# shroglck/open-pi-zero

Hardware: AMD Instinct MI355X
Metric: train samples/sec at gbsz 1024 (bf16 fwd+bwd+clip+AdamW) (higher is better)
Workload: dtype bf16; 1 GPU; Pi0 bridge training step: 256 img + 20 text + 1 proprio + 4 action tokens; model=pi0 (SigLIP-So400m/14 + Gemma-2B + 0.3B action expert), global_batch=1024, micro_batch=256, grad_accum=4, seq_len=281, parallelism=dp1

## Files before the change

include/pz_abi.h:

```cpp
#ifndef PZ_ABI_H
#define PZ_ABI_H

#include <stdint.h>

#ifdef __cplusplus
extern "C" {
#endif

#define PZ_ABI_VERSION 22

enum {
  PZ_OK = 0,
  PZ_ERR_INVALID_ARG = 1,
  PZ_ERR_LAUNCH = 2,
  PZ_ERR_UNSUPPORTED = 3,
};

enum {
  PZ_EPI_NONE = 0,
  PZ_EPI_GELU = 1,
  PZ_EPI_GEGLU = 2,
  PZ_EPI_SILU = 3,
  PZ_EPI_DGELU = 4,
  PZ_EPI_DSILU = 5,
// ... 13 lines not shown
  const void* bias;
  const void* resid; int64_t ld_resid;
  void* aux; int64_t ld_aux;
  int64_t geglu_inter;
  void* workspace; int64_t ws_bytes;
  const void* norm_w; float norm_eps;
  int32_t fp8_mode; const float* a_row_scale;
  const void* A2; int64_t lda2;
  const void* B2; int64_t ldb2;
  int64_t K2;
} pz_gemm_args;
int pz_gemm(const pz_gemm_args* args, void* stream);
#define PZ_ABSMAX_PARTS 1024
int pz_fp8_quant_vt(const void* v, int64_t ldv, int64_t v_bstride, int64_t Z, int64_t nk, void* vt, float* vs,
                    int64_t ldt, void* stream);
int pz_fp8_quant_attn(const void* q, int64_t nqr, const void* k, int64_t nkr, const void* v, int64_t ldv,
                      int64_t v_bstride, int64_t Z, int64_t nk, void* qc, float* qs, void* kc, float* ks, void* vt,
                      float* vs, int64_t ldt, void* stream);
int pz_rmsnorm_fwd_f8(const void* x, int64_t ldx, const void* w, void* q, int64_t ldq, float* qscale, int64_t R,
                      int64_t D, float eps, void* stream);
int pz_layernorm_fwd_f8(const void* x, int64_t ldx, const void* w, const void* b, void* q, int64_t ldq, float* qscale,
                        int64_t R, int64_t D, float eps, void* stream);
int pz_fp8_quant_rows(const void* x, int64_t ldx, void* q, int64_t ldq, float* row_scale, int64_t R, int64_t D,
                      void* stream);
int pz_fp8_quant_tensor(const void* x, int64_t n, void* q, float inv_scale, void* stream);
int pz_fp8_absmax(const void* x, int64_t n, float* parts, void* stream);
const char* pz_gemm_kernel_name(const pz_gemm_args* args);

typedef struct pz_small_gemm_args {
  int64_t M, N, K;
  const void* A; int64_t sAm, sAk;
  const void* B; int64_t sBk, sBn;
  void* C; int64_t ldc;
  const void* bias;
  float alpha;
  int32_t beta;
} pz_small_gemm_args;
int pz_gemm_small(const pz_small_gemm_args* args, void* stream);

int pz_rmsnorm_fwd(const void* x, int64_t ldx, const void* w, void* y, int64_t ldy, float* rstd,
                   int64_t R, int64_t D, float eps, void* stream);
int pz_rmsnorm_bwd(const void* dy, int64_t lddy, const void* x, int64_t ldx, const void* w,
                   const float* rstd, const void* dres, void* dx, int64_t lddx, float* dw_part,
                   int64_t R, int64_t D, void* stream);
int pz_layernorm_fwd(const void* x, int64_t ldx, const void* w, const void* b, void* y, int64_t ldy,
                     float* mean, float* rstd, int64_t R, int64_t D, float eps, void* stream);
int pz_layernorm_bwd(const void* dy, int64_t lddy, const void* x, int64_t ldx, const void* w,
                     const float* mean, const float* rstd, const void* dres, void* dx, int64_t lddx,
                     float* dw_part, float* db_part, int64_t R, int64_t D, float* dx_part, void* stream);
int64_t pz_norm_rows_per_part(void);
int pz_reduce_parts(const float* part, int64_t P, int64_t D, void* out, int32_t beta, void* stream);
typedef struct pz_reduce_seg {
  const float* part; int64_t P, D; void* out; int32_t beta;
} pz_reduce_seg;
int pz_reduce_parts_multi(const pz_reduce_seg* segs, int32_t nseg, void* stream);
int pz_act_bwd_colsum(const void* dh, int64_t lddh, const void* pre, int64_t ldpre, void* dpre, int64_t M, int64_t N,
                      int32_t act, float* ws, int64_t ws_rows, void* dbias, int32_t beta, void* stream);
int pz_colsum(const void* X, int64_t ld, int64_t M, int64_t N, void* out, int32_t beta, float* ws,
              void* stream);
int pz_batch_sum(const void* X, int64_t B, int64_t stride, int64_t n, void* out, int32_t beta, void* stream);

int pz_rope_table(float* cs, int64_t max_pos, int64_t head_dim, float theta, void* stream);
int pz_qkv_rope_split(const void* qkv, const int64_t* pos, const float* cs, void* q_out, void* k_out,
                      void* v_out, int64_t B, int64_t T, int64_t nh, int64_t nkv, int64_t hd,
                      int64_t Lq, int64_t qoff, int64_t Lk, int64_t koff, void* stream);
typedef struct pz_qkv_rope_args {
  const void* x; int64_t ldx;
  const void* W; int64_t ldw;
  int64_t M, N, K;
  const void* norm_w; float norm_eps;
  const int64_t* pos; const float* cs;
  void* q_out; void* k_out; void* v_out;
  int64_t T, nh, hd, Lq, qoff, Lk, koff;
  int32_t w_fp8; float w_scale;
  const void* x2; int64_t ldx2;
  const void* W2; int64_t ldw2;
  int64_t K2;
} pz_qkv_rope_args;
int pz_gemv_qkv_rope(const pz_qkv_rope_args* a, void* stream);
int pz_gemm_qkv_rope(const pz_qkv_rope_args* a, void* stream);
int pz_qkv_rope_split_bwd(const void* dq, const void* dk, const void* dv, const int64_t* pos,
                          const float* cs, void* dqkv, int64_t B, int64_t T, int64_t nh, int64_t nkv,
                          int64_t hd, int64_t Lq, int64_t qoff, int64_t Lk, int64_t koff, void* stream);

typedef struct pz_softmax_args {
  const float* S; int64_t lds;
  void* P; int64_t ldp;
  void* tcap;
  int64_t R, N;
  float scale, cap;
  int32_t mask_mode;
  int64_t rows_per_batch, heads, qoff;
  const int32_t* cnt; int64_t prefix, cond;
  const float* mask; int64_t ldm, mask_bstride;
} pz_softmax_args;
int pz_attn_softmax(const pz_softmax_args* a, void* stream);
int pz_attn_softmax_bwd(const void* P, const float* dP, int64_t lddp, const void* tcap, void* dS,
                        int64_t ldp, int64_t R, int64_t N, float scale, float cap, void* stream);

typedef struct pz_flash_args {
  int64_t Z, H, nq, nk, head_dim;
  const void* q; int64_t ldq, q_bstride, q_hstride;
  const void* k; int64_t ldk, k_bstride, k_hstride;
  const void* v; int64_t ldv, v_bstride, v_hstride;
  int32_t n_groups;
  int64_t g_row0[3];
  void* g_o[3];
  int64_t g_bstride[3], g_ld[3];
  int64_t o_hstride;
  float* lse;
  float scale, cap;
  int32_t mask_mode;
  const int32_t* cnt; int64_t prefix, cond, rows_per_token;
  const void* g_do[3];
  float* delta;
  void* dq; void* dk; void* dv;
  float* ws; int64_t ws_bytes;
  int64_t mask_row0;
} pz_flash_args;
int pz_flash_fwd(const pz_flash_args* a, void* stream);
int pz_flash_fwd_f8(const pz_flash_args* a, const void* qc, const float* qs, const void* kc, const float* ks,
                    int64_t krows, const void* vtc, const float* vs, int64_t ldvt, void* stream);
int pz_flash_fwd_probs(const pz_flash_args* a, void* P, void* tcap, int64_t ldp, void* stream);
int pz_flash_bwd_ds(const pz_flash_args* a, const void* P, const void* tcap, void* dS, int64_t ldp, void* stream);
int pz_flash_bwd_prep(const pz_flash_args* a, void* stream);
int pz_flash_bwd(const pz_flash_args* a, void* stream);

typedef struct pz_decode_attn_args {
  const void* q; int64_t ldq, Lq, qoff;
  const void* k; const void* v; int64_t k_bstride, v_bstride;
  void* o; int64_t ldo;
  int64_t B, nh, T, nk, head_dim;
  float scale, cap;
  const int32_t* cnt; int64_t prefix, cond, qtok0;
  float* ws; int64_t ws_bytes;
} pz_decode_attn_args;
int64_t pz_decode_attn_ws_bytes(int64_t B, int64_t rows, int64_t nk);
int pz_decode_attn(const pz_decode_attn_args* a, void* stream);

int pz_patchify(const void* pix, void* cols, int64_t B, int64_t H, int64_t W, int64_t ps, int64_t ldc,
                void* stream);
int pz_embed_merge(const int64_t* ids, const void* table, int64_t vocab, const void* img, void* out,
                   int64_t B, int64_t P, int64_t D, int64_t n_img, int64_t image_token, int64_t pad_token,
                   float emb_scale, float img_scale, void* stream);
int pz_embed_merge_bwd(const int64_t* ids, const void* dout, void* dimg, int64_t B, int64_t P,
                       int64_t D, int64_t n_img, int64_t image_token, float img_scale, void* stream);

int pz_time_embed(const float* t, void* out, int64_t B, int64_t D, float max_period, int32_t mode,
                  void* stream);
int pz_time_embed_rows(const float* t, void* out, int64_t ldo, int64_t B, int64_t H, int64_t D, float max_period,
                       int32_t mode, void* stream);
int pz_concat_time(const void* temb, const void* e1, void* out, int64_t B, int64_t H, int64_t D,
                   void* stream);
int pz_split_time_grad(const void* dcat, void* de1, int64_t rows, int64_t D, void* stream);
int pz_flow_psi(const float* x0, const float* x1, const float* t, void* psi, int64_t B, int64_t HA,
                float sig_min, void* stream);
int pz_flow_loss(const void* v, int64_t ldv, int64_t v_bstride, const float* x0, const float* x1, float* loss,
                 void* dv, const float* grad_scale, int64_t B, int64_t H, int64_t A, float sig_min, void* stream);
int pz_action_in(const float* action, int64_t A, const void* w1, const void* b1, const float* t, void* cat,
                 int64_t ldc, int64_t B, int64_t H, int64_t D, float max_period, int32_t mode, void* stream);
int pz_action_out(const void* x, int64_t ldx, const void* norm_w, float eps, const void* wd, const void* bd, int64_t D,
                  int64_t A, float* action, float* t, int64_t B, int64_t H, float dt, void* stream);
int pz_euler_step(float* action, const void* v, int64_t ldv, int64_t v_bstride, float* t, int64_t B, int64_t H,
                  int64_t A, float dt, void* stream);
int pz_clamp(float* x, int64_t n, float lo, float hi, void* stream);

int pz_geglu_bwd(const void* dh, int64_t lddh, const void* gu, int64_t ldgu, void* dgu, void* h_out,
                 int64_t ldh, int64_t M, int64_t I, void* stream);
int pz_act_bwd(const void* dh, int64_t lddh, const void* pre, int64_t ldpre, void* dpre, void* h_out,
               int64_t ldh, int64_t M, int64_t N, int32_t act ,
               void* stream);

int pz_adamw(void* p, const void* g, float* m, float* v, int64_t n, float lr, float beta1,
             float beta2, float eps, float wd, float bc1, float bc2, const float* gscale, void* stream);
#define PZ_SUMSQ_PARTS 2048
int pz_sumsq(const void* g, int64_t n, float* parts, void* stream);
int pz_clip_coef(const float* parts, int64_t nparts, float* coef, float* norm_out, float max_norm,
                 void* stream);

typedef struct pz_adamw8_args {
  void* p; const void* g;
  uint8_t* s1; uint8_t* s2;
  float* absmax1; float* absmax2;
  float* m32; float* v32;
  const int64_t* seg;
  int64_t nseg, nblocks;
  const float* qmap1; const float* qmap2;
  float beta1, beta2, omb1, omb2, step, epsc, decay;
  const float* gscale;
} pz_adamw8_args;
int pz_adamw8bit(const pz_adamw8_args* a, void* stream);

int pz_adamw8bit_r(const pz_adamw8_args* a, void* comp, int32_t mode, uint64_t rng_key, int64_t rng_base,
                   void* stream);
int pz_adamw_r(void* p, void* comp, const void* g, float* m, float* v, int64_t n, float lr, float beta1, float beta2,
               float eps, float wd, float bc1, float bc2, const float* gscale, int32_t mode, uint64_t rng_key,
               int64_t rng_base, void* stream);

int pz_fill_uniform(void* x, int32_t out_fp32, int64_t n, uint64_t seed, float off, float scale,
                    void* stream);
int pz_copy_rows(const void* src, int64_t sld, int64_t sbs, void* dst, int64_t dld, int64_t dbs, int64_t B,
                 int64_t rows, int64_t D, float scale, int32_t beta, void* stream);
int pz_cast_f32_bf16(const float* x, void* y, int64_t n, void* stream);
int pz_cast_bf16_f32(const void* x, float* y, int64_t n, void* stream);

int pz_adaln_fwd(const void* x, int64_t ldx, const void* y, int64_t ldy, const float* gate_pre,
                 const void* gate_bias, void* xm, int64_t ldxm, const float* gamma_pre, const void* gamma_bias,
                 const float* beta, void* h, int64_t ldh, float* rstd, int64_t ldmod, int64_t R, int64_t D,
                 int64_t rows_per_sample, float eps, void* stream);
int pz_adaln_norm_bwd(const void* dh, int64_t lddh, const void* x, int64_t ldx, const float* rstd,
                      const float* gamma_pre, const void* gamma_bias, const void* dres, void* dx, int64_t lddx,
                      float* dgamma_pre, float* dbeta, int64_t ldmod, int64_t R, int64_t D, int64_t rows_per_sample,
                      void* stream);
int pz_adaln_gate_bwd(const void* dout, int64_t lddo, const void* y, int64_t ldy, const float* gate_pre,
                      const void* gate_bias, void* dy, int64_t lddy, float* dgate_pre, int64_t ldmod, int64_t R,
                      int64_t D, int64_t rows_per_sample, void* stream);

int64_t pz_lora_wgrad_ws_bytes(int64_t M, int64_t D, int64_t R);
int pz_lora_wgrad(const void* Q, int64_t ldq, const void* P, int64_t ldp, void* out, int64_t ld_out, int64_t M,
                  int64_t D, int64_t R, int32_t transposed, float alpha, int32_t beta, void* ws, int64_t ws_bytes,
                  void* stream);

int pz_avg_lerp(void* avg, const void* p, int64_t n, float w, void* stream);
int pz_avg_swap(void* a, void* b, int64_t n, void* stream);

#define PZ_OBS_MAX_TAPS 64
#define PZ_OBS_MAX_EXTENT 16384
enum { PZ_OBS_NORM_BOUND = 0, PZ_OBS_NORM_GAUSSIAN = 1 };
int64_t pz_image_resize_scratch_bytes(int64_t n, int64_t H_in, int64_t S);
int pz_image_resize_norm(const void* frames, int32_t channels_last, int64_t n, int64_t H_in, int64_t W_in, int64_t S,
                         const void* h_first, const void* h_count, const void* h_w, int64_t h_taps,
                         const void* v_first, const void* v_count, const void* v_w, int64_t v_taps, const void* lut,
                         void* scratch, int64_t scratch_bytes, void* out, void* stream);
int pz_proprio_normalize(const void* x, void* y, int64_t rows, int64_t D, const void* a, const void* b, int32_t mode,
                         void* stream);
int pz_action_denormalize(const void* x, void* y, int64_t rows, int64_t D, int64_t n_pass, const void* a,
                          const void* b, int32_t mode, void* stream);

int pz_debug_poison_lds(uint32_t word, void* stream);
int pz_debug_spin(int64_t wgs, int64_t ticks, void* stream);

const char* pz_last_error(void);
int pz_abi_version(void);

#ifdef __cplusplus
}
#endif
#endif
```

open-pi-zero_amd/csrc/pz_attn.hip:

```cpp
#include "pz_common.h"

namespace {

__global__ void rope_table_kernel(float* cs, int64_t max_pos, int hd, float theta) {
  const int half = hd / 2;
  const int64_t idx = (int64_t)blockIdx.x * blockDim.x + threadIdx.x;
  if (idx >= (max_pos + 1) * half) return;
  const int64_t pos = idx / half;
  const int i = (int)(idx % half);
  const float expo = (float)(2 * i) / (float)hd;
  const float inv = 1.0f / powf(theta, expo);
  const float f = (float)pos * inv;
  cs[2 * idx] = cosf(f);
  cs[2 * idx + 1] = sinf(f);
}

__global__ void qkv_rope_split_kernel(const bf16_t* __restrict__ qkv, const int64_t* __restrict__ pos,
                                      const float* __restrict__ cs, bf16_t* q_out, bf16_t* k_out,
                                      bf16_t* v_out, int64_t T, int nh, int nkv, int hd, int64_t Lq,
                                      int64_t qoff, int64_t Lk, int64_t koff) {
  const int64_t t = blockIdx.x, b = blockIdx.y;
  const int64_t tok = b * T + t;
  const int half = hd / 2;
  const int width = (nh + 2 * nkv) * hd;
  const bf16_t* src = qkv + tok * width;
  const float* c = cs + pos[tok] * hd;
  if (q_out) {
    bf16_t* dq = q_out + (b * Lq + qoff + t) * (int64_t)(nh * hd);
    for (int e = threadIdx.x; e < nh * half; e += blockDim.x) {
      const int h = e / half, i = e % half;
      const float x1 = bf2f(src[h * hd + i]), x2 = bf2f(src[h * hd + i + half]);
      const float co = c[2 * i], si = c[2 * i + 1];
      float o1, o2;
      rope_pair(x1, x2, co, si, o1, o2);
      dq[h * hd + i] = f2bf(o1);
      dq[h * hd + i + half] = f2bf(o2);
    }
  }
  bf16_t* dk = k_out + (b * Lk + koff + t) * (int64_t)(nkv * hd);
  bf16_t* dv = v_out + (b * Lk + koff + t) * (int64_t)(nkv * hd);
  const bf16_t* sk = src + nh * hd;
  const bf16_t* sv = src + (nh + nkv) * hd;
  for (int e = threadIdx.x; e < nkv * half; e += blockDim.x) {
    const int h = e / half, i = e % half;
    const float x1 = bf2f(sk[h * hd + i]), x2 = bf2f(sk[h * hd + i + half]);
    const float co = c[2 * i], si = c[2 * i + 1];
    float o1, o2;
    rope_pair(x1, x2, co, si, o1, o2);
    dk[h * hd + i] = f2bf(o1);
    dk[h * hd + i + half] = f2bf(o2);
  }
  for (int e = threadIdx.x; e < nkv * hd; e += blockDim.x) dv[e] = sv[e];
}

__global__ void qkv_rope_split_bwd_kernel(const bf16_t* __restrict__ dq, const bf16_t* __restrict__ dk,
                                          const bf16_t* __restrict__ dv, const int64_t* __restrict__ pos,
                                          const float* __restrict__ cs, bf16_t* dqkv, int64_t T, int nh,
                                          int nkv, int hd, int64_t Lq, int64_t qoff, int64_t Lk,
                                          int64_t koff) {
  const int64_t t = blockIdx.x, b = blockIdx.y;
  const int64_t tok = b * T + t;
  const int half = hd / 2;
  const int width = (nh + 2 * nkv) * hd;
  bf16_t* dst = dqkv + tok * width;
  const float* c = cs + pos[tok] * hd;
  const bf16_t* sq = dq ? dq + (b * Lq + qoff + t) * (int64_t)(nh * hd) : nullptr;
  for (int e = threadIdx.x; e < nh * half; e += blockDim.x) {
    const int h = e / half, i = e % half;
    float o1 = 0.f, o2 = 0.f;
    if (sq) {
      const float y1 = bf2f(sq[h * hd + i]), y2 = bf2f(sq[h * hd + i + half]);
      const float co = c[2 * i], si = c[2 * i + 1];
      o1 = y1 * co + y2 * si;
      o2 = y2 * co - y1 * si;
    }
    dst[h * hd + i] = f2bf(o1);
    dst[h * hd + i + half] = f2bf(o2);
  }
  const bf16_t* sk = dk + (b * Lk + koff + t) * (int64_t)(nkv * hd);
  const bf16_t* sv = dv + (b * Lk + koff + t) * (int64_t)(nkv * hd);
  bf16_t* ok = dst + nh * hd;
  bf16_t* ov = dst + (nh + nkv) * hd;
  for (int e = threadIdx.x; e < nkv * half; e += blockDim.x) {
    const int h = e / half, i = e % half;
    const float y1 = bf2f(sk[h * hd + i]), y2 = bf2f(sk[h * hd + i + half]);
    const float co = c[2 * i], si = c[2 * i + 1];
    ok[h * hd + i] = f2bf(y1 * co + y2 * si);
    ok[h * hd + i + half] = f2bf(y2 * co - y1 * si);
  }
  for (int e = threadIdx.x; e < nkv * hd; e += blockDim.x) ov[e] = sv[e];
}

__device__ __forceinline__ bool block_allowed(int64_t i, int64_t j, int64_t cnt, int64_t P, int64_t C) {
  if (i < P) return i < cnt && j < cnt;
  if (i < P + C) return j < cnt || (j >= P && j < P + C);
  return j < cnt || j >= P;
}

template <int MAXE>
__global__ void __launch_bounds__(256) softmax_kernel(pz_softmax_args a) {
  const int lane = threadIdx.x & 63;
  const int64_t row = (int64_t)blockIdx.x * 4 + (threadIdx.x >> 6);
  if (row >= a.R) return;
  const float* s = a.S + row * a.lds;
  int64_t b = 0, qi = 0;
  if (a.mask_mode != 0) {
    b = row / a.rows_per_batch;
    qi = a.qoff + (row % a.rows_per_batch) / a.heads;
  }
  const int64_t cnt = a.mask_mode == 1 ? (int64_t)a.cnt[b] : 0;
  const float* mrow = a.mask_mode == 2 ? a.mask + b * a.mask_bstride + (qi - a.qoff) * a.ldm : nullptr;
  float x[MAXE];
  bool ok[MAXE];
  float mx = -INFINITY;
#pragma unroll
  for (int e = 0; e < MAXE; ++e) {
    const int64_t j = lane + 64 * e;
    ok[e] = false;
    x[e] = 0.f;
    if (j < a.N) {
      float v = s[j] * a.scale;
      if (a.cap > 0.f) v = a.cap * tanhf(v / a.cap);
      bool al = true;
      if (a.mask_mode == 1) al = block_allowed(qi, j, cnt, a.prefix, a.cond);
      else if (a.mask_mode == 2) {
        v += mrow[j];
        al = v > -INFINITY;
      }
      x[e] = v;
      ok[e] = al;
      if (al) mx = fmaxf(mx, v);
    }
  }
  mx = warp_max(mx);
  bf16_t* prow = (bf16_t*)a.P + row * a.ldp;
  bf16_t* trow = a.tcap ? (bf16_t*)a.tcap + row * a.ldp : nullptr;
  if (mx == -INFINITY) {
    const float u = 1.f / (float)a.N;
    for (int64_t j = lane; j < a.ldp; j += 64) {
      prow[j] = f2bf(j < a.N ? u : 0.f);
      if (trow) trow[j] = 0;
    }
    return;
  }
  float sum = 0.f;
#pragma unroll
  for (int e = 0; e < MAXE; ++e) {
    const float p = ok[e] ? __expf(x[e] - mx) : 0.f;
    x[e] = p;
    sum += p;
  }
  const float inv = 1.f / warp_sum(sum);
#pragma unroll
  for (int e = 0; e < MAXE; ++e) {
    const int64_t j = lane + 64 * e;
    if (j < a.N) {
      prow[j] = f2bf(x[e] * inv);
      if (trow) {
        float v = s[j] * a.scale;
        trow[j] = f2bf(a.cap > 0.f ? tanhf(v / a.cap) : 0.f);
      }
    }
  }
  for (int64_t j = a.N + lane; j < a.ldp; j += 64) {
    prow[j] = 0;
    if (trow) trow[j] = 0;
  }
}

__device__ __forceinline__ u32x2 pack4bf(const float (&v)[4]) { return u32x2{pack2bf(v[0], v[1]), pack2bf(v[2], v[3])}; }

template <int MAXV>
__global__ void __launch_bounds__(256) softmax4_kernel(pz_softmax_args a) {
// ... 115 lines not shown
      const float t[4] = {__uint_as_float(tw[0] << 16), __uint_as_float(tw[0] & 0xffff0000u),
                          __uint_as_float(tw[1] << 16), __uint_as_float(tw[1] & 0xffff0000u)};
#pragma unroll
      for (int i = 0; i < 4; ++i) {
        g[i] = j0 + i < N ? p[e][i] * (d[e][i] - dot) * scale : 0.f;
        if (cap > 0.f) g[i] *= (1.f - t[i] * t[i]);
      }
      *reinterpret_cast<u32x2*>(orow + j0) = pack4bf(g);
    }
  }
}

template <int MAXE>
__global__ void __launch_bounds__(256) softmax_bwd_kernel(const bf16_t* __restrict__ P,
                                                          const float* __restrict__ dP, int64_t lddp,
                                                          const bf16_t* __restrict__ tcap, bf16_t* dS,
                                                          int64_t ldp, int64_t R, int64_t N, float scale,
                                                          float cap) {
  const int lane = threadIdx.x & 63;
  const int64_t row = (int64_t)blockIdx.x * 4 + (threadIdx.x >> 6);
  if (row >= R) return;
  const bf16_t* prow = P + row * ldp;
  const float* drow = dP + row * lddp;
  float p[MAXE], d[MAXE];
  float dot = 0.f;
#pragma unroll
  for (int e = 0; e < MAXE; ++e) {
    const int64_t j = lane + 64 * e;
    p[e] = 0.f;
    d[e] = 0.f;
    if (j < N) {
      p[e] = bf2f(prow[j]);
      d[e] = drow[j];
      dot += p[e] * d[e];
    }
  }
  dot = warp_sum(dot);
  bf16_t* orow = dS + row * ldp;
#pragma unroll
  for (int e = 0; e < MAXE; ++e) {
    const int64_t j = lane + 64 * e;
    if (j < N) {
      float g = p[e] * (d[e] - dot) * scale;
      if (cap > 0.f) {
        const float t = bf2f(tcap[row * ldp + j]);
        g *= (1.f - t * t);
      }
      orow[j] = f2bf(g);
    }
  }
  for (int64_t j = N + lane; j < ldp; j += 64) orow[j] = 0;
}

}

extern "C" int pz_rope_table(float* cs, int64_t max_pos, int64_t head_dim, float theta, void* stream) {
  PZ_CHECK_ARG(cs && max_pos >= 0 && head_dim % 2 == 0, "rope_table: bad args");
  const int64_t n = (max_pos + 1) * (head_dim / 2);
  hipLaunchKernelGGL(rope_table_kernel, dim3((unsigned)((n + 255) / 256)), dim3(256), 0, (hipStream_t)stream, cs,
                     max_pos, (int)head_dim, theta);
  PZ_CHECK_LAUNCH();
  return PZ_OK;
}

extern "C" int pz_qkv_rope_split(const void* qkv, const int64_t* pos, const float* cs, void* q_out, void* k_out,
                                 void* v_out, int64_t B, int64_t T, int64_t nh, int64_t nkv, int64_t hd,
                                 int64_t Lq, int64_t qoff, int64_t Lk, int64_t koff, void* stream) {
  PZ_CHECK_ARG(qkv && pos && cs && k_out && v_out && B > 0 && T > 0 && hd % 2 == 0, "qkv_rope_split: bad args");
  PZ_CHECK_ARG(koff + T <= Lk && (!q_out || qoff + T <= Lq), "qkv_rope_split: token range");
  hipLaunchKernelGGL(qkv_rope_split_kernel, dim3((unsigned)T, (unsigned)B), dim3(256), 0, (hipStream_t)stream,
                     (const bf16_t*)qkv, pos, cs, (bf16_t*)q_out, (bf16_t*)k_out, (bf16_t*)v_out, T, (int)nh,
                     (int)nkv, (int)hd, Lq, qoff, Lk, koff);
  PZ_CHECK_LAUNCH();
  return PZ_OK;
}

extern "C" int pz_qkv_rope_split_bwd(const void* dq, const void* dk, const void* dv, const int64_t* pos,
                                     const float* cs, void* dqkv, int64_t B, int64_t T, int64_t nh, int64_t nkv,
                                     int64_t hd, int64_t Lq, int64_t qoff, int64_t Lk, int64_t koff, void* stream) {
  PZ_CHECK_ARG(dk && dv && pos && cs && dqkv && B > 0 && T > 0, "qkv_rope_split_bwd: bad args");
  hipLaunchKernelGGL(qkv_rope_split_bwd_kernel, dim3((unsigned)T, (unsigned)B), dim3(256), 0,
                     (hipStream_t)stream, (const bf16_t*)dq, (const bf16_t*)dk, (const bf16_t*)dv, pos, cs,
                     (bf16_t*)dqkv, T, (int)nh, (int)nkv, (int)hd, Lq, qoff, Lk, koff);
  PZ_CHECK_LAUNCH();
  return PZ_OK;
}

extern "C" int pz_attn_softmax(const pz_softmax_args* a, void* stream) {
  PZ_CHECK_ARG(a && a->S && a->P && a->R > 0 && a->N > 0 && a->ldp >= a->N && a->lds >= a->N,
               "attn_softmax: bad args");
  PZ_CHECK_ARG(a->N <= 1024, "attn_softmax: N=%lld > 1024 unsupported", (long long)a->N);
  if (a->mask_mode == 1) PZ_CHECK_ARG(a->cnt && a->rows_per_batch > 0 && a->heads > 0, "attn_softmax: block mask");
  if (a->mask_mode == 2) PZ_CHECK_ARG(a->mask && a->rows_per_batch > 0 && a->heads > 0, "attn_softmax: mask");
  dim3 grid((unsigned)((a->R + 3) / 4));
  hipStream_t st = (hipStream_t)stream;
  const bool vec = a->lds % 4 == 0 && a->ldp % 4 == 0 && PZ_ALIGNED(a->S, 16) && PZ_ALIGNED(a->P, 8) &&
                   (!a->tcap || PZ_ALIGNED(a->tcap, 8)) && a->R < (1LL << 31) && a->ldp <= 1024;
  if (vec) {
    if (a->ldp <= 512) hipLaunchKernelGGL(softmax4_kernel<2>, grid, dim3(256), 0, st, *a);
    else hipLaunchKernelGGL(softmax4_kernel<4>, grid, dim3(256), 0, st, *a);
    PZ_CHECK_LAUNCH();
    return PZ_OK;
  }
  if (a->N <= 256) hipLaunchKernelGGL(softmax_kernel<4>, grid, dim3(256), 0, st, *a);
  else if (a->N <= 512) hipLaunchKernelGGL(softmax_kernel<8>, grid, dim3(256), 0, st, *a);
  else hipLaunchKernelGGL(softmax_kernel<16>, grid, dim3(256), 0, st, *a);
  PZ_CHECK_LAUNCH();
  return PZ_OK;
}

extern "C" int pz_attn_softmax_bwd(const void* P, const float* dP, int64_t lddp, const void* tcap, void* dS,
                                   int64_t ldp, int64_t R, int64_t N, float scale, float cap, void* stream) {
  PZ_CHECK_ARG(P && dP && dS && R > 0 && N > 0 && N <= 1024 && (cap <= 0.f || tcap), "attn_softmax_bwd: bad args");
  dim3 grid((unsigned)((R + 3) / 4));
  hipStream_t st = (hipStream_t)stream;
  if (lddp % 4 == 0 && ldp % 4 == 0 && ldp <= 1024 && PZ_ALIGNED(dP, 16) && PZ_ALIGNED(P, 8) && PZ_ALIGNED(dS, 8) &&
      (cap <= 0.f || PZ_ALIGNED(tcap, 8))) {
    if (ldp <= 512)
      hipLaunchKernelGGL(softmax_bwd4_kernel<2>, grid, dim3(256), 0, st, (const bf16_t*)P, dP, lddp,
                         (const bf16_t*)tcap, (bf16_t*)dS, ldp, R, (int)N, scale, cap);
    else
      hipLaunchKernelGGL(softmax_bwd4_kernel<4>, grid, dim3(256), 0, st, (const bf16_t*)P, dP, lddp,
                         (const bf16_t*)tcap, (bf16_t*)dS, ldp, R, (int)N, scale, cap);
    PZ_CHECK_LAUNCH();
    return PZ_OK;
  }
  if (N <= 256)
    hipLaunchKernelGGL(softmax_bwd_kernel<4>, grid, dim3(256), 0, st, (const bf16_t*)P, dP, lddp,
                       (const bf16_t*)tcap, (bf16_t*)dS, ldp, R, N, scale, cap);
  else if (N <= 512)
    hipLaunchKernelGGL(softmax_bwd_kernel<8>, grid, dim3(256), 0, st, (const bf16_t*)P, dP, lddp,
                       (const bf16_t*)tcap, (bf16_t*)dS, ldp, R, N, scale, cap);
  else
    hipLaunchKernelGGL(softmax_bwd_kernel<16>, grid, dim3(256), 0, st, (const bf16_t*)P, dP, lddp,
                       (const bf16_t*)tcap, (bf16_t*)dS, ldp, R, N, scale, cap);
  PZ_CHECK_LAUNCH();
  return PZ_OK;
}
```

open-pi-zero_amd/csrc/pz_common.h:

```cpp
#pragma once

#include <hip/hip_runtime.h>
#include <stdint.h>
#include <stdlib.h>

#include "../../include/pz_abi.h"

typedef unsigned short bf16_t;
typedef __bf16 bf16x8 __attribute__((ext_vector_type(8)));
typedef float f32x4 __attribute__((ext_vector_type(4)));
typedef short s16x4 __attribute__((ext_vector_type(4)));
typedef short s16x8 __attribute__((ext_vector_type(8)));
typedef int i32x8 __attribute__((ext_vector_type(8)));
typedef unsigned int u32x4 __attribute__((ext_vector_type(4)));
typedef unsigned int u32x2 __attribute__((ext_vector_type(2)));

__device__ __forceinline__ float bf2f(bf16_t h) { return __uint_as_float(((unsigned)h) << 16); }
__device__ __forceinline__ bf16_t f2bf(float f) {
  __bf16 b = (__bf16)f;
  return __builtin_bit_cast(bf16_t, b);
}
typedef __bf16 bf16x2_t __attribute__((ext_vector_type(2)));
typedef float f32x2_t __attribute__((ext_vector_type(2)));
__device__ __forceinline__ unsigned pack2bf(float lo, float hi) {
  return __builtin_bit_cast(unsigned, __builtin_convertvector(f32x2_t{lo, hi}, bf16x2_t));
}

__device__ __forceinline__ uint64_t splitmix64(uint64_t z) {
  z += 0x9E3779B97F4A7C15ull;
  z = (z ^ (z >> 30)) * 0xBF58476D1CE4E5B9ull;
  z = (z ^ (z >> 27)) * 0x94D049BB133111EBull;
  return z ^ (z >> 31);
}

__device__ __forceinline__ float warp_sum(float v) {
#pragma unroll
  for (int o = 32; o > 0; o >>= 1) v += __shfl_xor(v, o, 64);
  return v;
}
__device__ __forceinline__ float warp_max(float v) {
#pragma unroll
  for (int o = 32; o > 0; o >>= 1) v = fmaxf(v, __shfl_xor(v, o, 64));
  return v;
}

template <int NW>
__device__ __forceinline__ float block_sum(float v, float* red) {
  v = warp_sum(v);
  const int w = threadIdx.x >> 6, l = threadIdx.x & 63;
  if (NW == 1) return v;
  if (l == 0) red[w] = v;
  __syncthreads();
  float t = 0.f;
#pragma unroll
  for (int i = 0; i < NW; ++i) t += red[i];
  __syncthreads();
  return t;
}

__device__ __forceinline__ float fast_rcp(float x) { return __builtin_amdgcn_rcpf(x); }
__device__ __forceinline__ float fast_exp(float u) { return __builtin_amdgcn_exp2f(u * 1.4426950408889634f); }

__device__ __forceinline__ float tanh_fast(float u) { return 1.f - 2.f * fast_rcp(fast_exp(2.f * u) + 1.f); }

__device__ __forceinline__ float gelu_tanh(float x) {
  constexpr float c0 = -2.f * 0.7978845608028654f * 1.4426950408889634f, c1 = c0 * 0.044715f;
  const float e = __builtin_amdgcn_exp2f(x * __builtin_fmaf(c1, x * x, c0));
  return x * fast_rcp(1.f + e);
}
__device__ __forceinline__ void gelu_tanh_both(float x, float& gl, float& gr) {
  constexpr float c0 = -2.f * 0.7978845608028654f * 1.4426950408889634f, c1 = c0 * 0.044715f;
  constexpr float k0 = 0.7978845608028654f, k3 = 3.f * 0.044715f * 0.7978845608028654f;
  const float x2 = x * x;
  const float s = fast_rcp(1.f + __builtin_amdgcn_exp2f(x * __builtin_fmaf(c1, x2, c0)));
  gl = x * s;
  gr = __builtin_fmaf(2.f * x * s * (1.f - s), __builtin_fmaf(k3, x2, k0), s);
}
__device__ __forceinline__ float gelu_tanh_grad(float x) {
  float gl, gr;
  gelu_tanh_both(x, gl, gr);
  return gr;
}

__device__ __forceinline__ float silu(float x) { return x * fast_rcp(1.f + fast_exp(-x)); }
__device__ __forceinline__ float silu_grad(float x) {
  const float s = fast_rcp(1.f + fast_exp(-x));
  return s * (1.f + x * (1.f - s));
}

bool pz_gemv_supported(const pz_gemm_args* a);
int pz_gemv_launch(const pz_gemm_args* a, hipStream_t st);

void pz_set_error(const char* fmt, ...);
#define PZ_CHECK_ARG(cond, ...)          \
  do {                                   \
    if (!(cond)) {                       \
      pz_set_error(__VA_ARGS__);         \
      return PZ_ERR_INVALID_ARG;         \
    }                                    \
  } while (0)
#define PZ_CHECK_LAUNCH()                                                   \
  do {                                                                      \
    hipError_t e_ = hipGetLastError();                                      \
    if (e_ != hipSuccess) {                                                 \
      pz_set_error("%s: launch failed: %s", __func__, hipGetErrorString(e_)); \
      return PZ_ERR_LAUNCH;                                                 \
    }                                                                       \
  } while (0)
#define PZ_ALIGNED(p, n) ((((uintptr_t)(p)) % (n)) == 0)

__device__ __forceinline__ void rope_pair(float x1, float x2, float co, float si, float& o1, float& o2) {
#pragma clang fp contract(off)
  o1 = x1 * co - x2 * si;
  o2 = x2 * co + x1 * si;
}
```

open-pi-zero_amd/csrc/pz_flash.hip:

```cpp
#include "pz_common.h"

#include <type_traits>

namespace {

constexpr int FA_KB = 64;
constexpr int FA_NW = 4;
constexpr int FA_QS = 32;

template <int HD>
struct FaDims {
  static constexpr int HDK = (HD + 31) / 32 * 32;
  static constexpr int HDV = (HD + 15) / 16 * 16;
  static constexpr int NKS = HDK / 32;
  static constexpr int NDB = HDV / 16;
  static constexpr int ROW = HD == 256 ? 272 : (HD == 72 ? 112 : HDK + 16);
  static constexpr int FNW = HD == 256 ? 8 : 4;
  static constexpr int FNQB = HD == 256 ? 1 : 2;
};

__device__ __forceinline__ bool fa_allowed(int64_t i, int64_t j, int64_t cnt, int64_t P, int64_t C) {
  if (i < P) return i < cnt && j < cnt;
  if (i < P + C) return j < cnt || (j >= P && j < P + C);
  return j < cnt || j >= P;
// ... 2104 lines not shown
    const bf16x8 dt = fs_cat(td[db][0], td[db][1]), qt = fs_cat(tq[db][0], tq[db][1]); \
    dv[db][0] = mfma(dt, pb0, dv[db][0]);                                        \
    dv[db][1] = mfma(dt, pb1, dv[db][1]);                                        \
    dk[db][0] = mfma(qt, sb0, dk[db][0]);                                        \
    dk[db][1] = mfma(qt, sb1, dk[db][1]);                                        \
  }
      FS_TR(0, 0); FS_TR(0, 1); FS_TR(1, 0); FS_TR(1, 1);
      asm volatile("s_waitcnt lgkmcnt(0)"
                   : "+v"(td[0][0]), "+v"(td[0][1]), "+v"(td[1][0]), "+v"(td[1][1]), "+v"(tq[0][0]), "+v"(tq[0][1]),
                     "+v"(tq[1][0]), "+v"(tq[1][1]));
      FS_TR(2, 0); FS_TR(2, 1); FS_TR(3, 0); FS_TR(3, 1);
      FS_MM(0) FS_MM(1)
      asm volatile("s_waitcnt lgkmcnt(0)"
                   : "+v"(td[2][0]), "+v"(td[2][1]), "+v"(td[3][0]), "+v"(td[3][1]), "+v"(tq[2][0]), "+v"(tq[2][1]),
                     "+v"(tq[3][0]), "+v"(tq[3][1]));
      FS_TR(4, 0); FS_TR(4, 1);
      FS_MM(2) FS_MM(3)
      asm volatile("s_waitcnt lgkmcnt(0)" : "+v"(td[4][0]), "+v"(td[4][1]), "+v"(tq[4][0]), "+v"(tq[4][1]));
      FS_MM(4)
#undef FS_MM
#undef FS_TR
    };
#pragma unroll 1
    for (int qs = 0; qs < FS_N / FA_QS - 1; ++qs) step(qs, false);
    step(FS_N / FA_QS - 1, true);
    FS_WAIT_VM(0);
#pragma unroll
    for (int kb2 = 0; kb2 < 2; ++kb2) {
      const int key = wave * 32 + kb2 * 16 + (lane & 15);
      bf16_t* dK = (bf16_t*)a.dk + b * a.k_bstride + h * a.k_hstride + (int64_t)key * a.ldk;
      bf16_t* dV = (bf16_t*)a.dv + b * a.v_bstride + h * a.v_hstride + (int64_t)key * a.ldv;
#pragma unroll
      for (int db = 0; db < 5; ++db) {
        const int d = db * 16 + 4 * g;
        if (d < 72) {
          *reinterpret_cast<u32x2*>(dK + d) = u32x2{pack2bf(dk[db][kb2][0] * a.scale, dk[db][kb2][1] * a.scale),
                                                    pack2bf(dk[db][kb2][2] * a.scale, dk[db][kb2][3] * a.scale)};
          *reinterpret_cast<u32x2*>(dV + d) =
              u32x2{pack2bf(dv[db][kb2][0], dv[db][kb2][1]), pack2bf(dv[db][kb2][2], dv[db][kb2][3])};
        }
      }
    }
    if (un < units && w0) tix.publish(tk, fa_smem + ((t + 1) & 1) * 2 * FS_IMG + FS_SLOT1);
    FS_BARRIER();
    u = un;
  }
}

constexpr int JD_SLOT = 64 * 512, JD_SMEM = 4 * JD_SLOT;

struct JdDma {
  int wave, lane;
  bool trs;
  __device__ __forceinline__ JdDma(int wave_, int lane_, bool trs_) : wave(wave_), lane(lane_), trs(trs_) {}
  __device__ __forceinline__ void issue(const bf16_t* X, int64_t ld, int kb, int nk, char* slot, int) const {
    int ln = lane;
    asm volatile("" : "+v"(ln));
#pragma unroll
    for (int s = 0; s < 4; ++s) {
      const int r = 2 * (wave * 4 + s) + (ln >> 5), pch = ln & 31;
      const int coff = 8 * (pch ^ (trs ? 2 * (r & 7) : (r & 15)));
      int key = kb * 64 + r;
      key = key < nk ? key : nk - 1;
      fs_glds16(X + (int64_t)key * ld + coff, slot + (wave * 4 + s) * 1024);
    }
  }
};

template <int K2, int DG>
__device__ __forceinline__ void jd_pv_group(f32x4 (&o)[16], const unsigned (&vs)[8], const bf16x8& pk) {
  s16x4 tv[4][2];
#define JD_TR(u, hf) tv[u][hf] = fs_tr<(K2 * 32 + 16 * (hf)) * 512 + ((DG * 4 + (u)) & 8) * 32>(vs[(DG * 4 + (u)) & 7])
  JD_TR(0, 0); JD_TR(0, 1); JD_TR(1, 0); JD_TR(1, 1); JD_TR(2, 0); JD_TR(2, 1); JD_TR(3, 0); JD_TR(3, 1);
#undef JD_TR
  asm volatile("s_waitcnt lgkmcnt(0)"
               : "+v"(tv[0][0]), "+v"(tv[0][1]), "+v"(tv[1][0]), "+v"(tv[1][1]), "+v"(tv[2][0]), "+v"(tv[2][1]),
                 "+v"(tv[3][0]), "+v"(tv[3][1]));
#pragma unroll
  for (int u = 0; u < 4; ++u) o[DG * 4 + u] = mfma(fs_cat(tv[u][0], tv[u][1]), pk, o[DG * 4 + u]);
}

template <bool CAP>
__global__ void __launch_bounds__(JP_NW * 64, 1) flash_fwd_probs_dma_kernel(pz_flash_args a, bf16_t* P, bf16_t* TC,
                                                                         int64_t ldp) {
  extern __shared__ __attribute__((aligned(16))) char fa_smem[];
  constexpr int RPW = JP_NW * 16;
  const int lane = threadIdx.x & 63, wave = threadIdx.x >> 6, g = lane >> 4, l15 = lane & 15;
  int64_t zh;
  int qblk;
  fa_unit_block((int)((a.nq + RPW - 1) / RPW), (int)(a.Z * a.H), zh, qblk);
  const int64_t b = zh / a.H, h = zh % a.H;
  const int64_t r = (int64_t)qblk * RPW + wave * 16 + l15;
  const bool live = r < a.nq;
  const bf16_t* Q = (const bf16_t*)a.q + b * a.q_bstride + h * a.q_hstride;
  const bf16_t* K = (const bf16_t*)a.k + b * a.k_bstride + h * a.k_hstride;
  const bf16_t* V = (const bf16_t*)a.v + b * a.v_bstride + h * a.v_hstride;
  const FaMask mk(a, b);
  const FaFast ff(a);
  const int nk = (int)a.nk;
  const JdDma dmk(wave, lane, false), dmv(wave, lane, true);
  bf16x8 qf[8];
  {
    const bf16_t* qrow = Q + (live ? r : 0) * a.ldq + 8 * g;
#define JD_QLD(ks) asm volatile("global_load_dwordx4 %0, %1, off offset:%2" : "=v"(qf[ks]) : "v"(qrow), "i"((ks) * 64) : "memory")
    JD_QLD(0); JD_QLD(1); JD_QLD(2); JD_QLD(3); JD_QLD(4); JD_QLD(5); JD_QLD(6); JD_QLD(7);
#undef JD_QLD
  }
  auto issue = [&](int s) {
    char* slot = fa_smem + (s % 4) * JD_SLOT;
    if (s < 5) dmk.issue(K, a.ldk, s, nk, slot, wave);
    else dmv.issue(V, a.ldv, s - 5, nk, slot, wave);
  };
  issue(0);
  issue(1);
  issue(2);
  const int t = mk.token((int)r);
  const bool dead = mk.dead(t);
  const int rb = fa_row_bits(mk, t), full_keys = fa_full_keys(mk);
  const bool clean = __ballot(dead || !live) == 0ull;
  f32x4 sc[JP_MAXKB][4];
  u32x2 tcv[JP_MAXKB][4];
  float mx = -INFINITY;
  auto logits_blk = [&](int kb) {
    auto logits = [&](auto FAST) {
#pragma unroll
      for (int i = 0; i < 4; ++i) {
        float tv[4];
#pragma unroll
        for (int e = 0; e < 4; ++e) {
          const float sv = sc[kb][i][e];
          float th = 0.f, x2;
          if constexpr (CAP) {
            th = fmaf(-2.f, __builtin_amdgcn_rcpf(__builtin_amdgcn_exp2f(sv * ff.k2) + 1.f), 1.f);
            x2 = th * ff.crow_live;
          } else {
            x2 = sv * ff.crow_live;
          }
          if constexpr (!decltype(FAST)::value) {
            const int j = kb * FA_KB + i * 16 + 4 * g + e;
            const bool ok = j < nk && (j < full_keys || ((rb >> fa_key_class(mk, j)) & 1));
            x2 = ok ? x2 : -INFINITY;
            th = (dead || j >= nk) ? 0.f : th;
          }
          sc[kb][i][e] = x2;
          mx = fmaxf(mx, x2);
          tv[e] = th;
        }
        tcv[kb][i] = u32x2{pack2bf(tv[0], tv[1]), pack2bf(tv[2], tv[3])};
      }
    };
    if (clean && (kb + 1) * 64 <= full_keys) logits(std::true_type{});
    else logits(std::false_type{});
  };
#pragma unroll
  for (int kb = 0; kb < JP_MAXKB; ++kb) {
    FS_WAIT_VM(8);
    FS_BARRIER();
    if (kb == 0)
      asm volatile("" : "+v"(qf[0]), "+v"(qf[1]), "+v"(qf[2]), "+v"(qf[3]), "+v"(qf[4]), "+v"(qf[5]), "+v"(qf[6]),
                   "+v"(qf[7]));
    issue(kb + 3);
    const char* slot = fa_smem + (kb % 4) * JD_SLOT + l15 * 512;
#pragma unroll
    for (int i = 0; i < 4; ++i) sc[kb][i] = f32x4{0.f, 0.f, 0.f, 0.f};
#pragma unroll
    for (int ks = 0; ks < 8; ++ks) {
      const char* kp = slot + 16 * ((4 * ks + g) ^ l15);
#pragma unroll
      for (int i = 0; i < 4; ++i) sc[kb][i] = mfma(*reinterpret_cast<const bf16x8*>(kp + i * 8192), qf[ks], sc[kb][i]);
    }
    if (kb >= 1) logits_blk(kb - 1);
  }
  logits_blk(JP_MAXKB - 1);
  FS_WAIT_VM(4);
  bf16_t* prow = P + (b * a.nq + (live ? r : 0)) * ldp;
  if (TC) {
    bf16_t* trow = TC + (b * a.nq + (live ? r : 0)) * ldp;
#pragma unroll
    for (int kb = 0; kb < JP_MAXKB; ++kb)
#pragma unroll
      for (int i = 0; i < 4; ++i) {
        const int j0 = kb * FA_KB + i * 16 + 4 * g;
        if (clean && (kb + 1) * 64 <= full_keys) *reinterpret_cast<u32x2*>(trow + j0) = tcv[kb][i];
        else if (live && j0 < ldp) *reinterpret_cast<u32x2*>(trow + j0) = tcv[kb][i];
      }
  }
  mx = fs_max4(mx);
  float sum = 0.f;
#pragma unroll
  for (int kb = 0; kb < JP_MAXKB; ++kb)
#pragma unroll
    for (int i = 0; i < 4; ++i)
#pragma unroll
      for (int e = 0; e < 4; ++e) {
        const float pv = __builtin_amdgcn_exp2f(sc[kb][i][e] - mx);
        sc[kb][i][e] = pv;
        sum += pv;
      }
  sum = fs_sum4(sum);
  const float inv = 1.f / sum, uni = 1.f / (float)nk;
  bf16x8 pf[JP_MAXKB][2];
#pragma unroll
  for (int kb = 0; kb < JP_MAXKB; ++kb) {
    unsigned pk[4][2];
    auto probs = [&](auto FAST) {
#pragma unroll
      for (int i = 0; i < 4; ++i) {
        if constexpr (decltype(FAST)::value) {
          pk[i][0] = pack2bf(sc[kb][i][0] * inv, sc[kb][i][1] * inv);
          pk[i][1] = pack2bf(sc[kb][i][2] * inv, sc[kb][i][3] * inv);
        } else {
          float pv[4];
#pragma unroll
          for (int e = 0; e < 4; ++e) {
            const int j = kb * FA_KB + i * 16 + 4 * g + e;
            pv[e] = dead ? (j < nk ? uni : 0.f) : sc[kb][i][e] * inv;
          }
          pk[i][0] = pack2bf(pv[0], pv[1]);
          pk[i][1] = pack2bf(pv[2], pv[3]);
        }
        const int j0 = kb * FA_KB + i * 16 + 4 * g;
        if (decltype(FAST)::value || (live && j0 < ldp)) *reinterpret_cast<u32x2*>(prow + j0) = u32x2{pk[i][0], pk[i][1]};
      }
    };
    if (clean && (kb + 1) * 64 <= full_keys) probs(std::true_type{});
    else probs(std::false_type{});
    pf[kb][0] = __builtin_bit_cast(bf16x8, u32x4{pk[0][0], pk[0][1], pk[1][0], pk[1][1]});
    pf[kb][1] = __builtin_bit_cast(bf16x8, u32x4{pk[2][0], pk[2][1], pk[3][0], pk[3][1]});
  }
  f32x4 o[16];
#pragma unroll
  for (int db = 0; db < 16; ++db) o[db] = f32x4{0.f, 0.f, 0.f, 0.f};
  const int q4 = l15 >> 2, p4 = lane & 3, w = 4 * (g & 1) + q4;
  unsigned va[8];
#pragma unroll
  for (int d7 = 0; d7 < 8; ++d7) va[d7] = fs_lds_addr(fa_smem + (4 * g + q4) * 512 + 32 * (d7 ^ w) + 8 * p4);
#pragma unroll
  for (int kb = 0; kb < JP_MAXKB; ++kb) {
    const int s = 5 + kb;
    if (s == 7) FS_WAIT_VM(8);
    if (s == 8) FS_WAIT_VM(4);
    if (s == 9) FS_WAIT_VM(0);
    FS_BARRIER();
    if (s + 3 <= 9) issue(s + 3);
    const unsigned sb = (unsigned)((s % 4) * JD_SLOT);
    unsigned vs[8];
#pragma unroll
    for (int d7 = 0; d7 < 8; ++d7) vs[d7] = va[d7] + sb;
    jd_pv_group<0, 0>(o, vs, pf[kb][0]);
    jd_pv_group<0, 1>(o, vs, pf[kb][0]);
    jd_pv_group<0, 2>(o, vs, pf[kb][0]);
    jd_pv_group<0, 3>(o, vs, pf[kb][0]);
    jd_pv_group<1, 0>(o, vs, pf[kb][1]);
    jd_pv_group<1, 1>(o, vs, pf[kb][1]);
    jd_pv_group<1, 2>(o, vs, pf[kb][1]);
    jd_pv_group<1, 3>(o, vs, pf[kb][1]);
  }
  if (!live) return;
  const FaRow fr{&a};
  const int gi = fr.grp(r);
  bf16_t* O = (bf16_t*)a.g_o[gi] + fr.off(b, h, r, gi);
#pragma unroll
  for (int db = 0; db < 16; ++db) {
    const int d = db * 16 + 4 * g;
    *reinterpret_cast<u32x2*>(O + d) = u32x2{pack2bf(o[db][0], o[db][1]), pack2bf(o[db][2], o[db][3])};
  }
}

__global__ void __launch_bounds__(JP_NW * 64, 1) flash_bwd_ds_dma_kernel(pz_flash_args a, const bf16_t* P,
                                                                      const bf16_t* TC, bf16_t* dS, int64_t ldp) {
  extern __shared__ __attribute__((aligned(16))) char fa_smem[];
  constexpr int RPW = JP_NW * 16;
  const int lane = threadIdx.x & 63, wave = threadIdx.x >> 6, g = lane >> 4, l15 = lane & 15;
  int64_t zh;
  int qblk;
  fa_unit_block((int)((a.nq + RPW - 1) / RPW), (int)(a.Z * a.H), zh, qblk);
  const int64_t b = zh / a.H, h = zh % a.H;
  const int64_t r = (int64_t)qblk * RPW + wave * 16 + l15;
  const bool live = r < a.nq;
  const bool want_dq = a.dq != nullptr;
  const bf16_t* V = (const bf16_t*)a.v + b * a.v_bstride + h * a.v_hstride;
  const bf16_t* K = want_dq ? (const bf16_t*)a.k + b * a.k_bstride + h * a.k_hstride : V;
  const int64_t ldk = want_dq ? a.ldk : a.ldv;
  const int nk = (int)a.nk;
  const JdDma dmv(wave, lane, false), dmk(wave, lane, true);
  auto issue = [&](int s) {
    char* slot = fa_smem + (s % 4) * JD_SLOT;
    if (s < 5) dmv.issue(V, a.ldv, s, nk, slot, wave);
    else dmk.issue(K, ldk, s - 5, nk, slot, wave);
  };
  bf16x8 df[8];
  bool has_do;
  {
    const FaRow fr{&a};
    const int gi = live ? fr.grp(r) : 0;
    has_do = live && a.g_do[gi];
    const bf16_t* dOr = has_do ? (const bf16_t*)a.g_do[gi] + fr.off(b, h, r, gi) + 8 * g : V;
#define JD_DLD(ks) asm volatile("global_load_dwordx4 %0, %1, off offset:%2" : "=v"(df[ks]) : "v"(dOr), "i"((ks) * 64) : "memory")
    JD_DLD(0); JD_DLD(1); JD_DLD(2); JD_DLD(3); JD_DLD(4); JD_DLD(5); JD_DLD(6); JD_DLD(7);
#undef JD_DLD
  }
  issue(0);
  issue(1);
  issue(2);
  const bf16_t* prow = P + (b * a.nq + (live ? r : 0)) * ldp;
  const bf16_t* trow = TC ? TC + (b * a.nq + (live ? r : 0)) * ldp : prow;
  const bool clean = __ballot(!live) == 0ull;
  f32x4 dp[JP_MAXKB][4];
  u32x2 pw[JP_MAXKB][4], tw[JP_MAXKB][4];
#pragma unroll
  for (int kb = 0; kb < JP_MAXKB; ++kb) {
    FS_WAIT_VM(8);
    FS_BARRIER();
    if (kb == 0) {
      asm volatile("" : "+v"(df[0]), "+v"(df[1]), "+v"(df[2]), "+v"(df[3]), "+v"(df[4]), "+v"(df[5]), "+v"(df[6]),
                   "+v"(df[7]));
      if (!has_do) {
#pragma unroll
        for (int ks = 0; ks < 8; ++ks) df[ks] = bf16x8{};
      }
    }
    issue(kb + 3);
    const char* slot = fa_smem + (kb % 4) * JD_SLOT + l15 * 512;
#pragma unroll
    for (int i = 0; i < 4; ++i) dp[kb][i] = f32x4{0.f, 0.f, 0.f, 0.f};
#pragma unroll
    for (int ks = 0; ks < 8; ++ks) {
      const char* vp = slot + 16 * ((4 * ks + g) ^ l15);
#pragma unroll
      for (int i = 0; i < 4; ++i) dp[kb][i] = mfma(*reinterpret_cast<const bf16x8*>(vp + i * 8192), df[ks], dp[kb][i]);
    }
  }
  int gl = g;
  asm volatile("" : "+v"(gl));
#pragma unroll
  for (int k2 = 0; k2 < JP_MAXKB; ++k2)
#pragma unroll
    for (int i = 0; i < 4; ++i) {
      const int j0 = k2 * FA_KB + i * 16 + 4 * gl;
      const int jc = j0 < ldp ? j0 : 0;
      asm volatile("global_load_dwordx2 %0, %1, off" : "=v"(pw[k2][i]) : "v"(prow + jc) : "memory");
    }
#pragma unroll
  for (int k2 = 0; k2 < JP_MAXKB; ++k2)
#pragma unroll
    for (int i = 0; i < 4; ++i) {
      const int j0 = k2 * FA_KB + i * 16 + 4 * gl;
      const int jc = j0 < ldp ? j0 : 0;
      asm volatile("global_load_dwordx2 %0, %1, off" : "=v"(tw[k2][i]) : "v"(trow + jc) : "memory");
    }
  FS_WAIT_VM(20);
  bf16_t* orow = dS + (b * a.nq + (live ? r : 0)) * ldp;
  const bool cap = a.cap > 0.f;
  float dot = 0.f;
#pragma unroll
  for (int kb = 0; kb < JP_MAXKB; ++kb)
#pragma unroll
    for (int i = 0; i < 4; ++i) {
      asm volatile("" : "+v"(pw[kb][i]));
      const int j0 = kb * FA_KB + i * 16 + 4 * g;
      if (!(live && j0 < nk)) pw[kb][i] = u32x2{0u, 0u};
      const float p0 = __uint_as_float(pw[kb][i][0] << 16), p1 = __uint_as_float(pw[kb][i][0] & 0xffff0000u);
      const float p2 = __uint_as_float(pw[kb][i][1] << 16), p3 = __uint_as_float(pw[kb][i][1] & 0xffff0000u);
      dot += p0 * dp[kb][i][0] + p1 * dp[kb][i][1] + p2 * dp[kb][i][2] + p3 * dp[kb][i][3];
    }
  dot += __shfl_xor(dot, 16, 64);
  dot += __shfl_xor(dot, 32, 64);
  FS_WAIT_VM(0);
#pragma unroll
  for (int kb = 0; kb < JP_MAXKB; ++kb)
#pragma unroll
    for (int i = 0; i < 4; ++i) asm volatile("" : "+v"(tw[kb][i]));
  bf16x8 dsf[JP_MAXKB][2];
#pragma unroll
  for (int kb = 0; kb < JP_MAXKB; ++kb) {
    unsigned pk[4][2];
#pragma unroll
    for (int i = 0; i < 4; ++i) {
      const int j0 = kb * FA_KB + i * 16 + 4 * g;
      const u32x2 tv2 = (cap && live && j0 < nk) ? tw[kb][i] : u32x2{0u, 0u};
      const float pv[4] = {__uint_as_float(pw[kb][i][0] << 16), __uint_as_float(pw[kb][i][0] & 0xffff0000u),
                           __uint_as_float(pw[kb][i][1] << 16), __uint_as_float(pw[kb][i][1] & 0xffff0000u)};
      const float tv[4] = {__uint_as_float(tv2[0] << 16), __uint_as_float(tv2[0] & 0xffff0000u),
                           __uint_as_float(tv2[1] << 16), __uint_as_float(tv2[1] & 0xffff0000u)};
      float x[4];
#pragma unroll
      for (int e = 0; e < 4; ++e) {
        x[e] = pv[e] * (dp[kb][i][e] - dot) * a.scale;
        if (cap) x[e] *= fmaf(-tv[e], tv[e], 1.f);
      }
      pk[i][0] = pack2bf(x[0], x[1]);
      pk[i][1] = pack2bf(x[2], x[3]);
      if (clean ? j0 < ldp : (live && j0 < ldp)) *reinterpret_cast<u32x2*>(orow + j0) = u32x2{pk[i][0], pk[i][1]};
    }
    dsf[kb][0] = __builtin_bit_cast(bf16x8, u32x4{pk[0][0], pk[0][1], pk[1][0], pk[1][1]});
    dsf[kb][1] = __builtin_bit_cast(bf16x8, u32x4{pk[2][0], pk[2][1], pk[3][0], pk[3][1]});
  }
  f32x4 dq[16];
#pragma unroll
  for (int db = 0; db < 16; ++db) dq[db] = f32x4{0.f, 0.f, 0.f, 0.f};
  const int q4 = l15 >> 2, p4 = lane & 3, w = 4 * (g & 1) + q4;
  unsigned ka[8];
#pragma unroll
  for (int d7 = 0; d7 < 8; ++d7) ka[d7] = fs_lds_addr(fa_smem + (4 * g + q4) * 512 + 32 * (d7 ^ w) + 8 * p4);
#pragma unroll
  for (int kb = 0; kb < JP_MAXKB; ++kb) {
    const int s = 5 + kb;
    if (s == 8) FS_WAIT_VM(4);
    if (s == 9) FS_WAIT_VM(0);
    FS_BARRIER();
    if (s + 3 <= 9) issue(s + 3);
    if (want_dq) {
      const unsigned sb = (unsigned)((s % 4) * JD_SLOT);
      unsigned ks_[8];
#pragma unroll
      for (int d7 = 0; d7 < 8; ++d7) ks_[d7] = ka[d7] + sb;
      jd_pv_group<0, 0>(dq, ks_, dsf[kb][0]);
      jd_pv_group<0, 1>(dq, ks_, dsf[kb][0]);
      jd_pv_group<0, 2>(dq, ks_, dsf[kb][0]);
      jd_pv_group<0, 3>(dq, ks_, dsf[kb][0]);
      jd_pv_group<1, 0>(dq, ks_, dsf[kb][1]);
      jd_pv_group<1, 1>(dq, ks_, dsf[kb][1]);
      jd_pv_group<1, 2>(dq, ks_, dsf[kb][1]);
      jd_pv_group<1, 3>(dq, ks_, dsf[kb][1]);
    }
  }
  if (!live || !want_dq) return;
  bf16_t* dQ = (bf16_t*)a.dq + b * a.q_bstride + h * a.q_hstride + r * a.ldq;
#pragma unroll
  for (int db = 0; db < 16; ++db) {
    const int d = db * 16 + 4 * g;
    *reinterpret_cast<u32x2*>(dQ + d) = u32x2{pack2bf(dq[db][0], dq[db][1]), pack2bf(dq[db][2], dq[db][3])};
  }
}

constexpr int F8_KB = 128, F8_KT = F8_KB * 256, F8_VT = 256 * F8_KB;
constexpr int F8_SMEM = 2 * (F8_KT + F8_VT) + 2 * F8_KB * 4;

__device__ __forceinline__ int f8_kswz(int r) { return (r & 3) | ((r >> 5) << 2); }
__device__ __forceinline__ int f8_vswz(int d) { return (d & 6) | ((d >> 3) & 1); }
__device__ __forceinline__ i32x8 f8_cat(const u32x4& lo, const u32x4& hi) {
  return i32x8{(int)lo[0], (int)lo[1], (int)lo[2], (int)lo[3], (int)hi[0], (int)hi[1], (int)hi[2], (int)hi[3]};
}
__device__ __forceinline__ unsigned f8_enc4(float a, float b, float c, float d) {
  int v = __builtin_amdgcn_cvt_pk_fp8_f32(a, b, 0, false);
  v = __builtin_amdgcn_cvt_pk_fp8_f32(c, d, v, true);
  return (unsigned)v;
}

__global__ void __launch_bounds__(512) flash_fwd_f8_kernel(pz_flash_args a, const uint8_t* __restrict__ qc,
                                                          const float* __restrict__ qs, const uint8_t* __restrict__ kc,
                                                          const float* __restrict__ ks, int64_t krows,
                                                          const uint8_t* __restrict__ vtc,
                                                          const float* __restrict__ vs, int64_t ldvt) {
  extern __shared__ __attribute__((aligned(16))) char fa_smem[];
  auto Kt = [&](int bi) { return fa_smem + bi * F8_KT; };
  auto Vt = [&](int bi) { return fa_smem + 2 * F8_KT + bi * F8_VT; };
  auto Sk = [&](int bi) { return reinterpret_cast<float*>(fa_smem + 2 * (F8_KT + F8_VT)) + bi * F8_KB; };
  const int t = threadIdx.x, lane = t & 63, wave = t >> 6, g = lane >> 4, l15 = lane & 15;
  const int64_t b = blockIdx.y;
  const int64_t q0 = (int64_t)blockIdx.x * 128 + wave * 16;
  const int64_t r = q0 + l15;
  const FaMask mk(a, b);
  const int nkb = (int)((a.nk + F8_KB - 1) / F8_KB);
  const int per = (nkb + (int)gridDim.z - 1) / (int)gridDim.z;
  const int kb_begin = (int)blockIdx.z * per, kb_end = min(nkb, kb_begin + per);
  u32x4 sk_[4], sv_[4];
  float sks = 0.f;
  auto load = [&](int kb) {
#pragma unroll
    for (int j = 0; j < 4; ++j) {
      const int c = t + 512 * j;
      const int64_t kr = min((int64_t)kb * F8_KB + (c >> 4), krows - 1);
      sk_[j] = *reinterpret_cast<const u32x4*>(kc + (b * krows + kr) * 256 + (c & 15) * 16);
      sv_[j] = *reinterpret_cast<const u32x4*>(vtc + (b * 256 + (c >> 3)) * ldvt + (int64_t)kb * F8_KB + (c & 7) * 16);
    }
    if (t < F8_KB) sks = ks[b * krows + min((int64_t)kb * F8_KB + t, krows - 1)];
  };
  auto store = [&](int bi) {
#pragma unroll
    for (int j = 0; j < 4; ++j) {
      const int c = t + 512 * j;
      const int kr = c >> 4, d = c >> 3;
      *reinterpret_cast<u32x4*>(Kt(bi) + kr * 256 + (((c & 15) ^ f8_kswz(kr)) << 4)) = sk_[j];
      *reinterpret_cast<u32x4*>(Vt(bi) + d * 128 + (((c & 7) ^ f8_vswz(d)) << 4)) = sv_[j];
    }
    if (t < F8_KB) Sk(bi)[t] = sks;
  };
  i32x8 qf[2];
  float sq = 0.f;
  {
    const bool ok = r < a.nq;
    const uint8_t* qr = qc + (b * a.nq + (ok ? r : 0)) * 256 + 32 * g;
#pragma unroll
    for (int k2 = 0; k2 < 2; ++k2) {
      const u32x4 lo = ok ? *reinterpret_cast<const u32x4*>(qr + 128 * k2) : u32x4{0u, 0u, 0u, 0u};
      const u32x4 hi = ok ? *reinterpret_cast<const u32x4*>(qr + 128 * k2 + 16) : u32x4{0u, 0u, 0u, 0u};
      qf[k2] = f8_cat(lo, hi);
    }
    if (ok) sq = qs[b * a.nq + r];
  }
  const int tq = mk.token((int)r);
  f32x4 o[16];
#pragma unroll
  for (int db = 0; db < 16; ++db) o[db] = f32x4{0.f, 0.f, 0.f, 0.f};
  float m = -INFINITY, l = 0.f;
  if (kb_begin < kb_end) {
    load(kb_begin);
    store(0);
  }
  __syncthreads();
// ... 167 lines not shown
               (long long)a->head_dim);
  PZ_CHECK_ARG(a->n_groups >= 1 && a->n_groups <= 3 && a->g_row0[0] == 0, "flash_fwd: output groups");
  for (int i = 0; i < a->n_groups; ++i) PZ_CHECK_ARG(a->g_o[i] && a->g_ld[i] % 4 == 0, "flash_fwd: group %d", i);
  PZ_CHECK_ARG(PZ_ALIGNED(a->q, 16) && PZ_ALIGNED(a->k, 16) && PZ_ALIGNED(a->v, 16) && a->ldq % 8 == 0 &&
                   a->ldk % 8 == 0 && a->ldv % 8 == 0 && a->q_hstride % 8 == 0 && a->k_hstride % 8 == 0 &&
                   a->v_hstride % 8 == 0 && a->q_bstride % 8 == 0 && a->k_bstride % 8 == 0 &&
                   a->v_bstride % 8 == 0 && a->o_hstride % 4 == 0,
               "flash_fwd: operands need 16-byte aligned rows");
  if (a->mask_mode == 1) PZ_CHECK_ARG(a->cnt && a->rows_per_token > 0, "flash_fwd: block mask needs cnt");
  PZ_CHECK_ARG(a->nq + a->mask_row0 < (1 << 22) && a->nk < (1 << 22) && a->mask_row0 >= 0, "flash_fwd: nq/nk too large");
  PZ_CHECK_ARG(a->Z * a->H < 65536, "flash_fwd: too many units");
  const int64_t qblk = (a->nq + 127) / 128, units = qblk * a->Z * a->H;
  const int64_t nkb = (a->nk + FA_KB - 1) / FA_KB;
  int64_t sp = 1;
  if (a->ws && units < 128 && nkb > 1 && a->head_dim % 4 == 0) {
    sp = (256 + units - 1) / units;
    sp = sp < nkb ? sp : nkb;
    sp = sp < 16 ? sp : 16;
    while (sp > 1 && sp * a->Z * a->H * a->nq * (a->head_dim + 2) * 4 > a->ws_bytes) --sp;
    const int64_t per = (nkb + sp - 1) / sp;
    sp = (nkb + per - 1) / per;
  }
  dim3 grid((unsigned)qblk, (unsigned)(a->Z * a->H), (unsigned)sp);
  hipStream_t st = (hipStream_t)stream;
  if (sp == 1 && fa_resident(a) && fa_unit(a)) {
    static bool attr = false;
    static bool attr2 = false;
    static bool attr3 = false;
    const dim3 gu((unsigned)(a->Z * a->H));
    if (fa_sig(a)) {
      const int G = fa_sig_grid(a);
      (void)attr3;
      {
        static bool attr4 = false;
        fa_smem_attr(flash_fwd_sig_kernel<1>, FS_SMEM, attr4);
        hipLaunchKernelGGL(flash_fwd_sig_kernel<1>, dim3((unsigned)G), dim3(16 * 64), FS_SMEM, st, *a, G);
      }
    } else if (fa_plain(a)) {
      fa_smem_attr(flash_fwd_unit_kernel<72, true>, FR_SMEM_KQ, attr);
      hipLaunchKernelGGL((flash_fwd_unit_kernel<72, true>), gu, dim3(FU_NW * 64), FR_SMEM_KQ, st, *a);
    } else {
      fa_smem_attr(flash_fwd_unit_kernel<72, false>, FR_SMEM_KQ, attr2);
      hipLaunchKernelGGL((flash_fwd_unit_kernel<72, false>), gu, dim3(FU_NW * 64), FR_SMEM_KQ, st, *a);
    }
    PZ_CHECK_LAUNCH();
    return PZ_OK;
  }
  if (sp == 1 && fa_resident(a)) {
    static bool attr = false;
    fa_smem_attr(flash_fwd_res_kernel<72>, FR_SMEM_KQ, attr);
    hipLaunchKernelGGL(flash_fwd_res_kernel<72>, dim3((unsigned)((a->nq + FR_NW * 16 - 1) / (FR_NW * 16) * a->Z * a->H)),
                       dim3(FR_NW * 64), FR_SMEM_KQ, st, *a);
    PZ_CHECK_LAUNCH();
    return PZ_OK;
  }
  FA_DISPATCH(a->head_dim, flash_fwd_kernel, grid, dim3((a->head_dim == 256 ? 8 : 4) * 64), 0, st, *a);
  PZ_CHECK_LAUNCH();
  if (sp > 1) {
    const int64_t n = a->Z * a->H * a->nq * (a->head_dim / 4);
    FA_DISPATCH(a->head_dim, flash_fwd_combine_kernel, dim3((unsigned)((n + 255) / 256)), dim3(256), 0, st, *a,
                (int)sp);
    PZ_CHECK_LAUNCH();
  }
  return PZ_OK;
}


extern "C" int pz_flash_fwd_probs(const pz_flash_args* a, void* P, void* tcap, int64_t ldp, void* stream) {
  PZ_CHECK_ARG(a && a->q && a->k && a->v && P && a->Z > 0 && a->H > 0 && a->nq > 0 && a->nk > 0,
               "flash_fwd_probs: bad args");
  PZ_CHECK_ARG(a->head_dim == 256, "flash_fwd_probs: head_dim %lld (256 only)", (long long)a->head_dim);
  PZ_CHECK_ARG(a->nk <= JP_MAXKB * FA_KB && ldp >= a->nk && ldp % 4 == 0, "flash_fwd_probs: nk %lld / ldp %lld",
               (long long)a->nk, (long long)ldp);
  PZ_CHECK_ARG(a->mask_mode == 0 || (a->mask_mode == 1 && a->cnt && a->rows_per_token > 0),
               "flash_fwd_probs: mask mode %d", a->mask_mode);
  PZ_CHECK_ARG(a->n_groups >= 1 && a->n_groups <= 3 && a->g_row0[0] == 0, "flash_fwd_probs: output groups");
  for (int i = 0; i < a->n_groups; ++i) PZ_CHECK_ARG(a->g_o[i] && a->g_ld[i] % 4 == 0, "flash_fwd_probs: group %d", i);
  PZ_CHECK_ARG(PZ_ALIGNED(a->q, 16) && PZ_ALIGNED(a->k, 16) && PZ_ALIGNED(a->v, 16) && PZ_ALIGNED(P, 8) &&
                   (!tcap || PZ_ALIGNED(tcap, 8)) && a->ldq % 8 == 0 && a->ldk % 8 == 0 && a->ldv % 8 == 0 &&
                   a->q_bstride % 8 == 0 && a->k_bstride % 8 == 0 && a->v_bstride % 8 == 0,
               "flash_fwd_probs: operands need 16-byte aligned rows");
  PZ_CHECK_ARG(a->nq + a->mask_row0 < (1 << 22) && a->Z * a->H < 65536, "flash_fwd_probs: nq / units too large");
  const int64_t units = a->Z * a->H, nqb = (a->nq + JP_NW * 16 - 1) / (JP_NW * 16);
  {
    static bool attr0 = false, attr1 = false;
    if (a->cap > 0.f) {
      fa_smem_attr(flash_fwd_probs_dma_kernel<true>, JD_SMEM, attr1);
      hipLaunchKernelGGL(flash_fwd_probs_dma_kernel<true>, dim3((unsigned)(nqb * units)), dim3(JP_NW * 64), JD_SMEM,
                         (hipStream_t)stream, *a, (bf16_t*)P, (bf16_t*)tcap, ldp);
    } else {
      fa_smem_attr(flash_fwd_probs_dma_kernel<false>, JD_SMEM, attr0);
      hipLaunchKernelGGL(flash_fwd_probs_dma_kernel<false>, dim3((unsigned)(nqb * units)), dim3(JP_NW * 64), JD_SMEM,
                         (hipStream_t)stream, *a, (bf16_t*)P, (bf16_t*)tcap, ldp);
    }
    PZ_CHECK_LAUNCH();
    return PZ_OK;
  }
}

extern "C" int pz_flash_bwd_ds(const pz_flash_args* a, const void* P, const void* tcap, void* dS, int64_t ldp,
                               void* stream) {
  PZ_CHECK_ARG(a && a->v && P && dS && a->Z > 0 && a->H > 0 && a->nq > 0 && a->nk > 0, "flash_bwd_ds: bad args");
  PZ_CHECK_ARG(a->head_dim == 256, "flash_bwd_ds: head_dim %lld (256 only)", (long long)a->head_dim);
  PZ_CHECK_ARG(a->nk <= JP_MAXKB * FA_KB && ldp >= a->nk && ldp % 4 == 0, "flash_bwd_ds: nk %lld / ldp %lld",
               (long long)a->nk, (long long)ldp);
  PZ_CHECK_ARG(a->cap <= 0.f || tcap, "flash_bwd_ds: soft-cap needs tcap");
  PZ_CHECK_ARG(a->n_groups >= 1 && a->n_groups <= 3 && a->g_row0[0] == 0, "flash_bwd_ds: output groups");
  for (int i = 0; i < a->n_groups; ++i) PZ_CHECK_ARG(!a->g_do[i] || a->g_ld[i] % 8 == 0, "flash_bwd_ds: dO group %d", i);
  PZ_CHECK_ARG(PZ_ALIGNED(a->v, 16) && a->ldv % 8 == 0 && a->v_bstride % 8 == 0 && PZ_ALIGNED(P, 8) &&
                   PZ_ALIGNED(dS, 8) && (!tcap || PZ_ALIGNED(tcap, 8)),
               "flash_bwd_ds: alignment");
  if (a->dq)
    PZ_CHECK_ARG(a->k && PZ_ALIGNED(a->k, 16) && a->ldk % 8 == 0 && a->k_bstride % 8 == 0 && PZ_ALIGNED(a->dq, 8) &&
                     a->ldq % 4 == 0 && a->q_bstride % 4 == 0,
                 "flash_bwd_ds: dQ needs K (16-byte rows) and an 8-byte aligned dQ");
  PZ_CHECK_ARG(a->Z * a->H < 65536, "flash_bwd_ds: too many units");
  const int64_t units = a->Z * a->H, nqb = (a->nq + JP_NW * 16 - 1) / (JP_NW * 16);
  static bool attr = false;
  fa_smem_attr(flash_bwd_ds_dma_kernel, JD_SMEM, attr);
  hipLaunchKernelGGL(flash_bwd_ds_dma_kernel, dim3((unsigned)(nqb * units)), dim3(JP_NW * 64), JD_SMEM,
                     (hipStream_t)stream, *a, (const bf16_t*)P, (const bf16_t*)tcap, (bf16_t*)dS, ldp);
  PZ_CHECK_LAUNCH();
  return PZ_OK;
}

extern "C" int pz_flash_bwd_prep(const pz_flash_args* a, void* stream) {
  PZ_CHECK_ARG(a && a->delta && a->n_groups >= 1 && a->n_groups <= 3, "flash_bwd_prep: bad args");
  for (int i = 0; i < a->n_groups; ++i) PZ_CHECK_ARG(a->g_o[i] && a->g_do[i], "flash_bwd_prep: group %d", i);
  const int64_t rows = a->Z * a->H * a->nq;
  PZ_CHECK_ARG(fa_hd_ok(a->head_dim), "flash_bwd_prep: head_dim");
  FA_DISPATCH(a->head_dim, flash_bwd_prep_kernel, dim3((unsigned)((rows + 3) / 4)), dim3(256), 0, (hipStream_t)stream,
              *a);
  PZ_CHECK_LAUNCH();
  return PZ_OK;
}

extern "C" int pz_flash_bwd(const pz_flash_args* a, void* stream) {
  PZ_CHECK_ARG(a && a->lse && a->delta && a->dq && a->dk && a->dv, "flash_bwd: bad args");
  PZ_CHECK_ARG(fa_hd_ok(a->head_dim), "flash_bwd: head_dim");
  PZ_CHECK_ARG(PZ_ALIGNED(a->dq, 16) && PZ_ALIGNED(a->dk, 16) && PZ_ALIGNED(a->dv, 16), "flash_bwd: alignment");
  for (int i = 0; i < a->n_groups; ++i) PZ_CHECK_ARG(a->g_do[i] && a->g_ld[i] % 8 == 0, "flash_bwd: dO group %d", i);
  hipStream_t st = (hipStream_t)stream;
  const int64_t nkb = (a->nk + FA_KB - 1) / FA_KB;
  int64_t splits = 1;
  if (a->ws && a->head_dim % 4 == 0) {
    splits = (1024 + nkb * a->Z * a->H - 1) / (nkb * a->Z * a->H);
    splits = splits < 8 ? splits : 8;
    while (splits > 1 && splits * 2 * a->Z * a->H * a->nk * a->head_dim * 4 > a->ws_bytes) --splits;
  }
  if (fa_resident(a) && fa_unit(a)) {
    static bool aq = false, akv = false, aq2 = false, akv2 = false, aq3 = false, akv3 = false;
    const dim3 gu((unsigned)(a->Z * a->H));
    if (fa_sig(a)) {
      const int G = fa_sig_grid(a);
      fa_smem_attr(flash_bwd_kv_sig_kernel, FS_SMEM, akv3);
      (void)aq3;
      {
        static bool aq4 = false;
        fa_smem_attr(flash_bwd_q_sig_kernel<true>, FS_SMEM, aq4);
        hipLaunchKernelGGL(flash_bwd_q_sig_kernel<true>, dim3((unsigned)G), dim3(FS_NW * 64), FS_SMEM, st, *a, G);
      }
      PZ_CHECK_LAUNCH();
      hipLaunchKernelGGL(flash_bwd_kv_sig_kernel, dim3((unsigned)G), dim3(FS_NW * 64), FS_SMEM, st, *a, G);
    } else if (fa_plain(a)) {
      fa_smem_attr(flash_bwd_q_unit_kernel<72, true>, FR_SMEM_KQ, aq);
      fa_smem_attr(flash_bwd_kv_unit_kernel<72, true>, FU_SMEM_KV, akv);
      hipLaunchKernelGGL((flash_bwd_q_unit_kernel<72, true>), gu, dim3(FU_NW * 64), FR_SMEM_KQ, st, *a);
      PZ_CHECK_LAUNCH();
      hipLaunchKernelGGL((flash_bwd_kv_unit_kernel<72, true>), gu, dim3(FU_NW * 64), FU_SMEM_KV, st, *a);
    } else {
      fa_smem_attr(flash_bwd_q_unit_kernel<72, false>, FR_SMEM_KQ, aq2);
      fa_smem_attr(flash_bwd_kv_unit_kernel<72, false>, FU_SMEM_KV, akv2);
      hipLaunchKernelGGL((flash_bwd_q_unit_kernel<72, false>), gu, dim3(FU_NW * 64), FR_SMEM_KQ, st, *a);
      PZ_CHECK_LAUNCH();
      hipLaunchKernelGGL((flash_bwd_kv_unit_kernel<72, false>), gu, dim3(FU_NW * 64), FU_SMEM_KV, st, *a);
    }
    PZ_CHECK_LAUNCH();
    return PZ_OK;
  }
  if (fa_resident(a)) {
    static bool aq = false, akv = false;
    fa_smem_attr(flash_bwd_q_res_kernel<72>, FR_SMEM_KQ, aq);
    fa_smem_attr(flash_bwd_kv_res_kernel<72>, FR_SMEM_KV, akv);
    hipLaunchKernelGGL(flash_bwd_q_res_kernel<72>, dim3((unsigned)((a->nq + FR_NW * 16 - 1) / (FR_NW * 16) * a->Z * a->H)),
                       dim3(FR_NW * 64), FR_SMEM_KQ, st, *a);
    PZ_CHECK_LAUNCH();
    hipLaunchKernelGGL(flash_bwd_kv_res_kernel<72>, dim3((unsigned)(nkb * a->Z * a->H)), dim3(FR_NW * 64),
                       FR_SMEM_KV, st, *a);
    PZ_CHECK_LAUNCH();
    return PZ_OK;
  }
  const int fm = fa_fast_bwd(a);
  {
    const int64_t units = a->Z * a->H, nqb = (a->nq + JQ_NW * 32 - 1) / (JQ_NW * 32);
    const dim3 gq2((unsigned)(nqb * units));
    if (fm == 2) {
      FA_DISPATCH(a->head_dim, FA_T2(flash_bwd_q2_kernel, true), gq2, dim3(JQ_NW * 64), 0, st, *a);
    } else {
      FA_DISPATCH(a->head_dim, FA_T2(flash_bwd_q2_kernel, false), gq2, dim3(JQ_NW * 64), 0, st, *a);
    }
  }
  PZ_CHECK_LAUNCH();
  const dim3 gkv1((unsigned)(nkb * a->Z * a->H * splits));
  if (fm == 2) {
    FA_DISPATCH(a->head_dim, FA_T2(flash_bwd_kv_kernel, 2), gkv1, dim3(FA_NW * 64), 0, st, *a, (int)splits);
  } else {
// ... 50 lines not shown
```

open-pi-zero_amd/csrc/pz_gemm.hip:

```cpp
#include <stdarg.h>
#include <stdio.h>
#include <stdlib.h>
#include <string.h>

#include <type_traits>

#include "pz_gemm_epi.h"

namespace {

constexpr int BM = 128, BN = 128, BK = 64, NT = 256;
constexpr int TILE_BYTES = 128 * 64 * 2;


__device__ __forceinline__ i32x8 cat_f8(const bf16x8& lo, const bf16x8& hi) {
  const u32x4 a = __builtin_bit_cast(u32x4, lo), b = __builtin_bit_cast(u32x4, hi);
  return i32x8{(int)a[0], (int)a[1], (int)a[2], (int)a[3], (int)b[0], (int)b[1], (int)b[2], (int)b[3]};
}

__device__ __forceinline__ int sw_tr(int k) { return ((k & 3) | (((k >> 3) & 1) << 2)) << 2; }

template <bool KC>
__device__ __forceinline__ void g2r(u32x4 (&r)[4], const bf16_t* __restrict__ base, int64_t ld,
                                    int64_t row0, int64_t R, int64_t k0, int64_t K,
// ... 560 lines not shown
          float gl_, gr_;
          gelu_tanh_both(x0[e], gl_, gr_);
          dg[e] = v[e] * x1[e] * gr_;
          du[e] = v[e] * gl_;
        }
        st16(Cp, pack8v(dg));
        st16(Cp + p.geglu_I, pack8v(du));
      } else if (FM == FM_DACT) {
#pragma unroll
        for (int e = 0; e < 8; ++e) v[e] *= gelu ? gelu_tanh_grad(x0[e]) : silu_grad(x0[e]);
        st16(Cp, pack8v(v));
      } else {
        if (act) {
          if (p.aux) st16(p.aux + (m0 + row) * p.ld_aux + n0 + col, iv[i]);
#pragma unroll
          for (int e = 0; e < 8; ++e) v[e] = gelu ? gelu_tanh(v[e]) : silu(v[e]);
        }
#pragma unroll
        for (int e = 0; e < 8; ++e) v[e] += x1[e] + x0[e];
        st16(Cp, pack8v(v));
      }
    }
  }
}

__device__ __forceinline__ void epi8p_rope(const GemmP& p, int64_t m0, int64_t n0, int wr, int wc, int lane,
                                           const f32x4 (&acc)[8][4], char* smem) {
  const int g4 = 4 * (lane >> 4), rl = lane & 15;
  char* img = smem + (wc >> 1) * 65536;
#pragma unroll
  for (int rb = 0; rb < 8; ++rb)
#pragma unroll
    for (int cb = 0; cb < 4; ++cb) {
      float v[4];
#pragma unroll
      for (int r = 0; r < 4; ++r) v[r] = acc[rb][cb][r] * p.alpha;
      img_put(img, wr * 128 + rb * 16 + rl, (wc & 1) * 64 + cb * 16 + g4, u32x2{pack2bf(v[0], v[1]), pack2bf(v[2], v[3])});
    }
  lds_sync();
  const int64_t h = n0 >> 8;
#pragma unroll 2
  for (int it = 0; it < 8; ++it) {
    const int c = threadIdx.x + it * NT2, row = c >> 4, ch = c & 15;
    const int64_t m = m0 + row;
    if (m >= p.M) continue;
    const int off = (ch ^ (row & 15)) << 4;
    const u32x4 w1 = *reinterpret_cast<const u32x4*>(smem + row * 256 + off);
    const u32x4 w2 = *reinterpret_cast<const u32x4*>(smem + 65536 + row * 256 + off);
    const int64_t b = m / p.rT, t = m - b * p.rT;
    if (h == p.rnh + 1) {
      bf16_t* dv = p.rv + (b * p.rLk + p.rkoff + t) * 256 + ch * 8;
      *reinterpret_cast<u32x4*>(dv) = w1;
      *reinterpret_cast<u32x4*>(dv + 128) = w2;
      continue;
    }
    float x1[8], x2[8], o1[8], o2[8];
    unpack8(w1, x1);
    unpack8(w2, x2);
    const float4* cs = reinterpret_cast<const float4*>(p.rcs + p.rpos[m] * 256 + 16 * ch);
#pragma unroll
    for (int q = 0; q < 4; ++q) {
      const float4 c2 = cs[q];
      const float co0 = c2.x, si0 = c2.y, co1 = c2.z, si1 = c2.w;
      rope_pair(x1[2 * q], x2[2 * q], co0, si0, o1[2 * q], o2[2 * q]);
      rope_pair(x1[2 * q + 1], x2[2 * q + 1], co1, si1, o1[2 * q + 1], o2[2 * q + 1]);
    }
    bf16_t* d = h < p.rnh ? p.rq + (b * p.rLq + p.rqoff + t) * (p.rnh * 256) + h * 256 + ch * 8
                          : p.rk + (b * p.rLk + p.rkoff + t) * 256 + ch * 8;
    *reinterpret_cast<u32x4*>(d) = pack8v(o1);
    *reinterpret_cast<u32x4*>(d + 128) = pack8v(o2);
  }
}

template <bool GEGLU>
__device__ __forceinline__ void epilogue8p(const GemmP& p, int64_t cofs, int64_t rofs, int64_t m0, int64_t n0,
                                           int wr, int wc, int lane, const f32x4 (&acc)[8][4], char* smem) {
  if (!GEGLU && p.rcs) {
    epi8p_rope(p, m0, n0, wr, wc, lane, acc, smem);
    return;
  }
  const int g4 = 4 * (lane >> 4), rl = lane & 15;
  if (GEGLU) {
    if (m0 + BT <= p.M && n0 + BT / 2 <= p.geglu_I && p.aux) {
#pragma unroll
      for (int rb = 0; rb < 8; ++rb) {
        const int64_t m = m0 + wr * 128 + rb * 16 + rl;
        bf16_t* Ur = p.aux + m * p.ld_aux + p.geglu_I + n0 + wc * 32 + g4;
#pragma unroll
        for (int j = 0; j < 2; ++j) {
          float gg[4], hh[4], uu[4];
#pragma unroll
          for (int r = 0; r < 4; ++r) {
            gg[r] = acc[rb][j][r] * p.alpha;
            uu[r] = acc[rb][2 + j][r] * p.alpha;
            hh[r] = gelu_tanh(gg[r]) * uu[r];
          }
          const int row = wr * 128 + rb * 16 + rl, col = wc * 32 + j * 16 + g4;
          img_put(smem, row, col, u32x2{pack2bf(hh[0], hh[1]), pack2bf(hh[2], hh[3])});
          img_put(smem + 65536, row, col, u32x2{pack2bf(gg[0], gg[1]), pack2bf(gg[2], gg[3])});
          *reinterpret_cast<u32x2*>(Ur + j * 16) = pk4(uu);
        }
      }
      lds_sync();
      img_flush(smem, reinterpret_cast<bf16_t*>(p.C) + cofs + m0 * p.ldc + n0, p.ldc);
      img_flush(smem + 65536, p.aux + m0 * p.ld_aux + n0, p.ld_aux);
      return;
    }
#pragma unroll
    for (int rb = 0; rb < 8; ++rb) {
      const int64_t m = m0 + wr * 128 + rb * 16 + rl;
#pragma unroll
      for (int j = 0; j < 2; ++j) store_geglu4(p, cofs, m, n0 + wc * 32 + j * 16 + g4, acc[rb][j], acc[rb][2 + j]);
    }
    return;
  }
  const int64_t m = m0 + wr * 128 + (lane & 15), nb = n0 + wc * 64 + 4 * (lane >> 4);
  if (m0 + BT <= p.M && n0 + BT <= p.N) {
    switch (fast_mode(p)) {
      case FM_STORE: {
        float bias[4][4];
#pragma unroll
        for (int cb = 0; cb < 4; ++cb) {
          if (p.bias) {
            unpack4(*reinterpret_cast<const u32x2*>(p.bias + nb + cb * 16), bias[cb]);
          } else {
#pragma unroll
            for (int r = 0; r < 4; ++r) bias[cb][r] = 0.f;
          }
        }
        char* img = smem + (wc >> 1) * 65536;
#pragma unroll
        for (int rb = 0; rb < 8; ++rb)
#pragma unroll
          for (int cb = 0; cb < 4; ++cb) {
            float v[4];
#pragma unroll
            for (int r = 0; r < 4; ++r) v[r] = acc[rb][cb][r] * p.alpha + bias[cb][r];
            img_put(img, wr * 128 + rb * 16 + rl, (wc & 1) * 64 + cb * 16 + g4, u32x2{pack2bf(v[0], v[1]), pack2bf(v[2], v[3])});
          }
        lds_sync();
        bf16_t* C = reinterpret_cast<bf16_t*>(p.C) + cofs + m0 * p.ldc + n0;
        img_flush(smem, C, p.ldc);
        img_flush(smem + 65536, C + 128, p.ldc);
        break;
      }
      case FM_F32: epi8p_fast<FM_F32>(p, cofs, rofs, m, nb, acc); break;
      case FM_DACT: epi8p_staged<FM_DACT>(p, cofs, rofs, m0, n0, wr, wc, lane, acc, smem); break;
      case FM_DGEGLU: epi8p_staged<FM_DGEGLU>(p, cofs, rofs, m0, n0, wr, wc, lane, acc, smem); break;
      default: epi8p_staged<FM_BF16>(p, cofs, rofs, m0, n0, wr, wc, lane, acc, smem); break;
    }
    return;
  }
  f32x4* park = reinterpret_cast<f32x4*>(smem) + (wr * 4 + wc) * 1024 + lane;
#pragma unroll
  for (int half = 0; half < 2; ++half) {
#pragma unroll
    for (int g = 0; g < 16; ++g) park[g * 64] = acc[half * 4 + (g >> 2)][g & 3];
#pragma unroll 1
    for (int g = 0; g < 16; ++g)
      store_out4_rt(p, cofs, rofs, m + (half * 4 + (g >> 2)) * 16, nb + (g & 3) * 16, park[g * 64]);
  }
}

template <bool AKC, bool BKC, bool GEGLU, bool KTAIL, bool F8, bool EXT = false>
__device__ __forceinline__ void gemm8p_body(const GemmP& p) {
  static_assert(!EXT || (KTAIL && !F8), "rank extension: bf16, tail-capable instantiation");
  static_assert(AKC, "a k-strided A takes gemm8k_kernel (use_khalf)");
  extern __shared__ __attribute__((aligned(16))) char smem[];
  const int nk1 = (int)((p.K + 63) / 64);
  const int nk_all = EXT ? nk1 + (int)((p.K2 + 63) / 64) : nk1;
  int lid = blockIdx.x, piece = -1, kt0 = 0, nk = nk_all;
  if (p.tail_s && lid >= p.dp_tiles) {
    const int u = lid - p.dp_tiles;
    piece = u;
    lid = p.dp_tiles + u / p.tail_s;
    kt0 = (u % p.tail_s) * p.tail_kt;
    nk = min(nk_all - kt0, p.tail_kt);
  }
  int tm, tn;
  tile_coords(lid, p.tiles_m * p.tiles_n, p.tiles_m, p.tiles_n, tm, tn, p.group);
  const int64_t m0 = (int64_t)tm * BT;
  const int64_t n0 = GEGLU ? (int64_t)tn * (BT / 2) : (int64_t)tn * BT;
  const int t = threadIdx.x, lane = t & 63;
// ... 556 lines not shown
      float* Cp = reinterpret_cast<float*>(p.C) + cofs + mm * p.ldc + nn;
      *Cp = p.beta ? *Cp + x : x;
    } else {
      bf16_t* Cp = reinterpret_cast<bf16_t*>(p.C) + cofs + mm * p.ldc + nn;
      *Cp = f2bf(p.beta ? bf2f(*Cp) + x : x);
    }
  }
}

__global__ void gemm_small_kernel(pz_small_gemm_args a) {
  const int64_t idx = (int64_t)blockIdx.x * blockDim.x + threadIdx.x;
  if (idx >= a.M * a.N) return;
  const int64_t m = idx / a.N, n = idx % a.N;
  const bf16_t* A = (const bf16_t*)a.A;
  const bf16_t* B = (const bf16_t*)a.B;
  float s = 0.f;
  for (int64_t k = 0; k < a.K; ++k)
    s += bf2f(A[m * a.sAm + k * a.sAk]) * bf2f(B[k * a.sBk + n * a.sBn]);
  s *= a.alpha;
  if (a.bias) s += bf2f(((const bf16_t*)a.bias)[n]);
  bf16_t* C = (bf16_t*)a.C + m * a.ldc + n;
  if (a.beta) s += bf2f(*C);
  *C = f2bf(s);
}

constexpr int SMALL_NMAX = 8;
__global__ void __launch_bounds__(256) gemm_small_rowwave_kernel(pz_small_gemm_args a) {
  const int lane = threadIdx.x & 63;
  const int64_t m = (int64_t)blockIdx.x * 4 + (threadIdx.x >> 6);
  if (m >= a.M) return;
  const bf16_t* A = (const bf16_t*)a.A + m * a.sAm;
  const bf16_t* B = (const bf16_t*)a.B;
  float s[SMALL_NMAX];
#pragma unroll
  for (int n = 0; n < SMALL_NMAX; ++n) s[n] = 0.f;
  for (int64_t k = 8 * lane; k < a.K; k += 512) {
    const u32x4 xa = *reinterpret_cast<const u32x4*>(A + k);
    float x[8];
#pragma unroll
    for (int e = 0; e < 4; ++e) {
      x[2 * e] = bf2f(xa[e] & 0xffff);
      x[2 * e + 1] = bf2f(xa[e] >> 16);
    }
#pragma unroll
    for (int n = 0; n < SMALL_NMAX; ++n) {
      if (n >= a.N) break;
      const u32x4 wb = *reinterpret_cast<const u32x4*>(B + n * a.sBn + k);
#pragma unroll
      for (int e = 0; e < 4; ++e) s[n] += x[2 * e] * bf2f(wb[e] & 0xffff) + x[2 * e + 1] * bf2f(wb[e] >> 16);
    }
  }
#pragma unroll
  for (int n = 0; n < SMALL_NMAX; ++n) {
#pragma unroll
    for (int off = 32; off > 0; off >>= 1) s[n] += __shfl_xor(s[n], off);
  }
  if (lane < a.N) {
    float v = 0.f;
#pragma unroll
    for (int n = 0; n < SMALL_NMAX; ++n)
      if (n == lane) v = s[n];
    v *= a.alpha;
    if (a.bias) v += bf2f(((const bf16_t*)a.bias)[lane]);
    bf16_t* C = (bf16_t*)a.C + m * a.ldc + lane;
    if (a.beta) v += bf2f(*C);
    *C = f2bf(v);
  }
}

}


static thread_local char g_err[512];
void pz_set_error(const char* fmt, ...) {
  va_list ap;
  va_start(ap, fmt);
  vsnprintf(g_err, sizeof(g_err), fmt, ap);
  va_end(ap);
}

extern "C" const char* pz_last_error(void) { return g_err; }

extern "C" int pz_abi_version(void) { return PZ_ABI_VERSION; }

template <bool AKC, bool BKC, int WM, int TAG = 0>
static int launch_tile(const GemmP& p, int64_t batch, hipStream_t st) {
  const int smem = 4 * TILE_BYTES;
  auto kern = gemm_kernel<AKC, BKC, WM, TAG>;
  static bool attr_set = false;
  if (!attr_set) {
    hipFuncSetAttribute((const void*)kern, hipFuncAttributeMaxDynamicSharedMemorySize, smem);
    attr_set = true;
  }
  static int xb = -1;
  if (xb < 0) {
    const char* e = getenv("PZ_GEMM_BATCH_XCD");
    xb = !(e && e[0] == '0');
  }
  if (xb && p.ksplit == 0 && batch >= 8 && batch % 8 == 0 && (int64_t)p.tiles_m * p.tiles_n * batch < (1LL << 31)) {
    GemmP q = p;
    q.batch_xcd = (int)batch;
    hipLaunchKernelGGL(kern, dim3((unsigned)(p.tiles_m * p.tiles_n * batch)), dim3(NT), smem, st, q);
    PZ_CHECK_LAUNCH();
    return PZ_OK;
  }
  dim3 grid(p.tiles_m * p.tiles_n, (unsigned)batch);
  hipLaunchKernelGGL(kern, grid, dim3(NT), smem, st, p);
  PZ_CHECK_LAUNCH();
  return PZ_OK;
}

template <bool AKC, bool BKC, int WM>
static int launch_tile_x(const GemmP& p, hipStream_t st) {
  const int smem = 4 * TILE_BYTES;
  auto kern = gemm_x_kernel<AKC, BKC, WM>;
  static bool attr_set = false;
  if (!attr_set) {
    hipFuncSetAttribute((const void*)kern, hipFuncAttributeMaxDynamicSharedMemorySize, smem);
    attr_set = true;
  }
  hipLaunchKernelGGL(kern, dim3(p.tiles_m * p.tiles_n, 1), dim3(NT), smem, st, p);
  PZ_CHECK_LAUNCH();
  return PZ_OK;
}

static bool use_khalf(bool akc, bool bkc, int64_t m, int64_t n, int64_t k);

namespace {
static bool sk64_two_launch() {
  const char* e = getenv("PZ_SK64_FUSED");
  return e && e[0] == '0';
}

enum PathKind { PATH_SKINNY, PATH_256, PATH_TILE, PATH_SPLIT, PATH_GEMV, PATH_SKINNY64, PATH_ROWS, PATH_TALL };
struct Plan {
  PathKind kind;
  bool akc, bkc, geglu;
  int wm, tag, skinny_w, skinny_nc, skinny_mb, splits;
  int64_t ksplit, ldw, tiles_m, tiles_n;
  int dp_tiles, tail_s, tail_kt;
  int rows_w, rows_tnb, rows_tmb;
  int rows_f8;
  int tall_mi;
};

int device_cus() {
  static int cache[64] = {0};
  int dev = 0;
  if (hipGetDevice(&dev) != hipSuccess || dev < 0 || dev >= 64) return 256;
  if (!cache[dev]) {
    int n = 0;
    if (hipDeviceGetAttribute(&n, hipDeviceAttributeMultiprocessorCount, dev) != hipSuccess || n <= 0) n = 256;
    cache[dev] = n;
  }
  return cache[dev];
}

void plan_tail(Plan& pl, const pz_gemm_args* a) {
  if (a->batch != 1 || !a->workspace || !PZ_ALIGNED(a->workspace, 16)) return;
  const char* e = getenv("PZ_GEMM_TAIL");
  if (e && e[0] == '0') return;
  const int64_t G = device_cus();
  const int64_t T = pl.tiles_m * pl.tiles_n;
  const int64_t q = T / G, r = T % G;
  const int64_t nk = (a->K + 63) / 64;
  if (r == 0 || (q > 0 && 2 * r >= G) || q > 8) return;
// ... 407 lines not shown
               "pz_gemm: batch strides must keep 16-byte alignment");
  if (a->a_kcontig) PZ_CHECK_ARG(a->K % 8 == 0, "pz_gemm: k-contiguous A needs K %% 8 == 0");
  else PZ_CHECK_ARG(a->M % 8 == 0, "pz_gemm: k-strided A needs M %% 8 == 0");
  if (a->b_kcontig) PZ_CHECK_ARG(a->K % 8 == 0, "pz_gemm: k-contiguous B needs K %% 8 == 0");
  else PZ_CHECK_ARG(a->N % 8 == 0, "pz_gemm: k-strided B needs N %% 8 == 0");
  const bool geglu = a->epilogue == PZ_EPI_GEGLU;
  if (geglu) {
    PZ_CHECK_ARG(a->b_kcontig && a->geglu_inter > 0 && a->N == 2 * a->geglu_inter && a->batch == 1 &&
                     !a->beta_accum && !a->resid && !a->bias && !a->c_fp32 && a->geglu_inter % 4 == 0,
                 "pz_gemm: GEGLU needs k-contiguous B = [gate; up] (N = 2I), no batch/bias/resid");
  }
  if (a->epilogue == PZ_EPI_GELU || a->epilogue == PZ_EPI_SILU)
    PZ_CHECK_ARG(a->batch == 1, "pz_gemm: activation epilogue is unbatched");
  PZ_CHECK_ARG(a->epilogue >= PZ_EPI_NONE && a->epilogue <= PZ_EPI_DGEGLU, "pz_gemm: unknown epilogue %d",
               (int)a->epilogue);
  PZ_CHECK_ARG(!(a->c_fp32 && a->beta_accum && a->resid), "pz_gemm: fp32 beta accumulation takes no resid");
  if (a->epilogue >= PZ_EPI_DGELU) {
    PZ_CHECK_ARG(a->batch == 1 && a->aux && !a->bias && !a->resid && !a->beta_accum && !a->c_fp32,
                 "pz_gemm: backward epilogues read aux, write bf16 C, unbatched, no bias/resid/beta");
    if (a->epilogue == PZ_EPI_DGEGLU)
      PZ_CHECK_ARG(a->geglu_inter == a->N && a->ldc >= 2 * a->N && a->ld_aux >= 2 * a->N,
                   "pz_gemm: DGEGLU needs N == geglu_inter and [*, 2I] aux / C rows");
  }
  if (a->aux) PZ_CHECK_ARG(a->ld_aux % 4 == 0 && PZ_ALIGNED(a->aux, 8), "pz_gemm: aux alignment");
  PZ_CHECK_ARG(a->ws_bytes >= 0, "pz_gemm: negative ws_bytes");
  PZ_CHECK_ARG(a->fp8_mode >= 0 && a->fp8_mode <= 2, "pz_gemm: fp8_mode %d", (int)a->fp8_mode);
  PZ_CHECK_ARG(a->K2 >= 0, "pz_gemm: negative K2");
  if (a->K2 > 0) {
    if (a->fp8_mode != 0) {
      pz_set_error("pz_gemm: the rank extension (K2 > 0) takes bf16 operands only");
      return PZ_ERR_UNSUPPORTED;
    }
    PZ_CHECK_ARG(a->K2 % 8 == 0 && a->K2 >= 8 && a->K2 <= 384, "pz_gemm: K2 = %lld must be a multiple of 8 in [8, 384]",
                 (long long)a->K2);
    PZ_CHECK_ARG(a->A2 && a->B2 && PZ_ALIGNED(a->A2, 16) && PZ_ALIGNED(a->B2, 16) && a->lda2 % 8 == 0 &&
                     a->ldb2 % 8 == 0,
                 "pz_gemm: A2 / B2 must be 16-byte aligned with lda2 / ldb2 %% 8 == 0");
    PZ_CHECK_ARG(a->batch == 1 && !a->norm_w, "pz_gemm: the rank extension is unbatched and takes no fused norm");
  }
  pz_gemm_args a8;
  if (a->fp8_mode == 1) {
    PZ_CHECK_ARG(a->a_kcontig && a->b_kcontig && a->batch == 1 && !a->norm_w && a->epilogue <= PZ_EPI_SILU &&
                     a->K % 16 == 0 && a->lda % 16 == 0 && a->ldb % 16 == 0,
                 "pz_gemm: fp8 W8A8 needs k-contiguous A [M][K] and B [N][K] codes, batch 1, K / lda / ldb "
                 "%% 16 == 0, a forward epilogue and no fused norm");
    a8 = *a;
    a8.K = a->K / 2;
    a8.lda = a->lda / 2;
    a8.ldb = a->ldb / 2;
    a = &a8;
  }
  if (a->fp8_mode == 2) {
    PZ_CHECK_ARG(a->a_kcontig && a->b_kcontig && a->batch == 1 && a->K % 64 == 0 && !a->c_fp32 &&
                     a->epilogue < PZ_EPI_DGELU && a->ldb % 16 == 0,
                 "pz_gemm: fp8 weights with bf16 rows (W8A16) need k-contiguous A and B, batch 1, "
                 "K %% 64 == 0, ldb %% 16 == 0, bf16 C and a forward epilogue");
    PZ_CHECK_ARG(a->M <= 64 || make_plan(a).kind == PATH_ROWS,
                 "pz_gemm: W8A16 above 64 rows needs a row-slab shape (M <= 1024, K <= 2048, <= 4096 columns)");
  }

  GemmP p;
  memset(&p, 0, sizeof(p));
  p.A = (const bf16_t*)a->A;
  p.B = (const bf16_t*)a->B;
  p.C = a->C;
  p.bias = (const bf16_t*)a->bias;
  p.resid = (const bf16_t*)a->resid;
  p.aux = (bf16_t*)a->aux;
  p.M = a->M; p.N = a->N; p.K = a->K;
  p.lda = a->lda; p.ldb = a->ldb; p.ldc = a->ldc;
  p.ld_resid = a->ld_resid; p.ld_aux = a->ld_aux; p.geglu_I = a->geglu_inter;
  p.batch_inner = a->batch_inner;
  p.sAo = a->sA_outer; p.sAi = a->sA_inner;
  p.sBo = a->sB_outer; p.sBi = a->sB_inner;
  p.sCo = a->sC_outer; p.sCi = a->sC_inner;
  p.sRo = a->sR_outer; p.sRi = a->sR_inner;
  p.epi = a->epilogue;
  p.c_fp32 = a->c_fp32;
  p.beta = a->beta_accum;
  p.alpha = a->alpha;
  p.nw = (const bf16_t*)a->norm_w;
  p.neps = a->norm_eps;
  p.rs = a->fp8_mode == 1 ? a->a_row_scale : nullptr;
  if (a->K2 > 0) {
    p.A2 = (const bf16_t*)a->A2;
    p.B2 = (const bf16_t*)a->B2;
    p.lda2 = a->lda2; p.ldb2 = a->ldb2; p.K2 = a->K2;
  }
  hipStream_t st = (hipStream_t)stream;

  const Plan pl = make_plan(a);
  {
    const char* e = getenv("PZ_GEMM_GROUP");
    if (e && atoi(e) >= 1 && atoi(e) <= 64) p.group = atoi(e);
    else p.group = (a->K >= 16384 && pl.tiles_n <= 8) || a->epilogue == PZ_EPI_DGEGLU ? 2 : 8;
  }
  if (pl.kind == PATH_GEMV) return pz_gemv_launch(a, st);
  if (a->norm_w)
    PZ_CHECK_ARG((pl.kind == PATH_SKINNY || pl.kind == PATH_SKINNY64) && PZ_ALIGNED(a->norm_w, 16),
                 "pz_gemm: fused RMSNorm needs the few-row paths (M <= 64, k-contiguous A/B, K %% 32 == 0 "
                 "(M <= 16) or K %% 64 == 0) and a 16-byte aligned weight");
  if (pl.kind == PATH_SKINNY64) {
    p.tiles_n = (int)pl.tiles_n;
    if (pl.ksplit > 0) {
      p.ws = (float*)a->workspace;
      p.ksplit = pl.ksplit;
      p.ldw = pl.ldw;
      p.sk_tk = sk64_fits(pl, a) ? 0 : -1;
    }
    return pz_sk64_launch(p, pl.skinny_w, pl.skinny_mb, a->fp8_mode == 2, pl.tiles_n, st);
  }
  if (a->fp8_mode == 1 && pl.kind == PATH_ROWS) {
    p.tiles_m = (int)pl.tiles_m;
    p.tiles_n = (int)pl.tiles_n;
    PZ_CHECK_ARG(PZ_ALIGNED(a->A, 16) && PZ_ALIGNED(a->B, 16), "pz_gemm: W8A8 rows need 16-byte aligned codes");
    return pz_rows_launch(p, pl.rows_w, pl.rows_tnb, false, 2, st);
  }
  if (a->fp8_mode == 1) {
    p.tiles_m = (int)pl.tiles_m;
    p.tiles_n = (int)pl.tiles_n;
    PZ_CHECK_ARG(pl.tiles_m * pl.tiles_n < (1LL << 31), "pz_gemm: grid too large");
    if (pl.tail_s) {
      p.ws = (float*)a->workspace;
      p.dp_tiles = pl.dp_tiles;
      p.tail_s = pl.tail_s;
      p.tail_kt = pl.tail_kt;
    }
    return geglu ? launch8p_f8<true>(p, st) : launch8p_f8<false>(p, st);
  }
  if (pl.kind == PATH_SKINNY) {
    PZ_CHECK_ARG(a->batch < 65536, "pz_gemm: batch too large");
    if (pl.skinny_w == 16) return launch_skinny<16>(p, pl.skinny_nc, pl.tiles_n, a->batch, st);
    if (pl.skinny_w == 8) return launch_skinny<8>(p, pl.skinny_nc, pl.tiles_n, a->batch, st);
    return launch_skinny<4>(p, pl.skinny_nc, pl.tiles_n, a->batch, st);
  }
  p.tiles_m = (int)pl.tiles_m;
  p.tiles_n = (int)pl.tiles_n;
  PZ_CHECK_ARG(pl.tiles_m * pl.tiles_n < (1LL << 31) && a->batch < 65536, "pz_gemm: grid too large");
  if (pl.kind == PATH_ROWS)
    return pz_rows_launch(p, pl.rows_w, pl.rows_tnb, pl.geglu, pl.rows_f8, st);
  if (pl.kind == PATH_TALL) {
    if (pl.splits > 1) {
      p.ws = (float*)a->workspace;
      p.ksplit = pl.ksplit;
      p.ldw = pl.ldw;
    }
    return pz_tall_launch(p, pl.tall_mi, pl.splits > 1 ? pl.splits : 1, st);
  }
  if (a->K2 > 0) {
    if (pl.kind == PATH_256) {
      if (geglu) return launch8p_x<true, true>(p, st);
      return a->b_kcontig ? launch8p_x<true, false>(p, st) : launch8p_x<false, false>(p, st);
    }
    if (geglu) return a->a_kcontig ? launch_tile_x<true, true, 4>(p, st) : launch_tile_x<false, true, 4>(p, st);
    if (a->a_kcontig && a->b_kcontig) return launch_tile_x<true, true, 2>(p, st);
    if (a->a_kcontig && !a->b_kcontig) return launch_tile_x<true, false, 2>(p, st);
    if (!a->a_kcontig && a->b_kcontig) return launch_tile_x<false, true, 2>(p, st);
    return launch_tile_x<false, false, 2>(p, st);
  }
  if (pl.kind == PATH_256) {
    if (pl.tail_s) {
      p.ws = (float*)a->workspace;
      p.dp_tiles = pl.dp_tiles;
      p.tail_s = pl.tail_s;
      p.tail_kt = pl.tail_kt;
    }
// ... 125 lines not shown
```

open-pi-zero_amd/csrc/pz_gemm_epi.h:

```cpp
#pragma once

#include <type_traits>

#include "pz_common.h"

struct GemmP {
  const bf16_t* A;
  const bf16_t* B;
  void* C;
  const bf16_t* bias;
  const bf16_t* resid;
  bf16_t* aux;
  int64_t M, N, K, lda, ldb, ldc, ld_resid, ld_aux, geglu_I;
  int64_t batch_inner, sAo, sAi, sBo, sBi, sCo, sCi, sRo, sRi;
  int tiles_m, tiles_n, epi, c_fp32, beta;
  float alpha;
  float* ws;
  int64_t ksplit, ldw;
  int sk_tk;
  int batch_xcd;
  int dp_tiles, tail_s, tail_kt;
  const bf16_t* nw;
  float neps;
  const float* rs;
  const int64_t* rpos;
  const float* rcs;
  bf16_t *rq, *rk, *rv;
  int64_t rT, rnh, rLq, rqoff, rLk, rkoff;
  int group;
  const bf16_t* A2;
  const bf16_t* B2;
  int64_t lda2, ldb2, K2;
};

namespace {

__device__ __forceinline__ void tile_coords(int bid, int nwg, int tiles_m, int tiles_n, int& tm, int& tn,
                                            int GROUP = 8) {
  const int xcd = bid & 7, local = bid >> 3;
  const int q = nwg >> 3, r = nwg & 7;
  const int wg = (xcd < r ? xcd * (q + 1) : r * (q + 1) + (xcd - r) * q) + local;
  GROUP = GROUP >= 1 ? GROUP : 8;
  const int per_group = GROUP * tiles_n;
  const int g = wg / per_group;
  const int first_m = g * GROUP;
  const int gsize = min(tiles_m - first_m, GROUP);
  const int in = wg - g * per_group;
  tm = first_m + in % gsize;
  tn = in / gsize;
}

struct Side {
  u32x4 w;
};

__device__ __forceinline__ u32x2 ld4bf(const bf16_t* X, bool full, int64_t n, int64_t N) {
  if (full) return *reinterpret_cast<const u32x2*>(X);
  unsigned h[4];
#pragma unroll
  for (int r = 0; r < 4; ++r) h[r] = n + r < N ? (unsigned)X[r] : 0u;
  return u32x2{h[0] | (h[1] << 16), h[2] | (h[3] << 16)};
}
__device__ __forceinline__ void unpack4(u32x2 w, float (&o)[4]) {
  o[0] = __uint_as_float(w[0] << 16); o[1] = __uint_as_float(w[0] & 0xffff0000u);
  o[2] = __uint_as_float(w[1] << 16); o[3] = __uint_as_float(w[1] & 0xffff0000u);
}
__device__ __forceinline__ void store4(bf16_t* X, bool full, int64_t n, int64_t N, const float (&v)[4]) {
  if (full) {
    *reinterpret_cast<u32x2*>(X) = u32x2{pack2bf(v[0], v[1]), pack2bf(v[2], v[3])};
  } else {
#pragma unroll
    for (int r = 0; r < 4; ++r)
      if (n + r < N) X[r] = f2bf(v[r]);
  }
}

__device__ __forceinline__ u32x2 epi_load_bias(const GemmP& p, int64_t n) {
  if (!p.bias || n >= p.N) return u32x2{0u, 0u};
  return ld4bf(p.bias + n, n + 4 <= p.N, n, p.N);
}

enum EpiMode { EM_BF16 = 0, EM_F32 = 1, EM_DACT = 2, EM_DGEGLU = 3 };

template <int EM>
__device__ __forceinline__ void epi_load4(const GemmP& p, int64_t cofs, int64_t rofs, int64_t m, int64_t n,
                                          Side& s) {
  s.w = u32x4{0u, 0u, 0u, 0u};
  if (m >= p.M || n >= p.N) return;
  const bool full = n + 4 <= p.N;
  if constexpr (EM == EM_DGEGLU) {
    const bf16_t* X = p.aux + m * p.ld_aux + n;
    const u32x2 g = ld4bf(X, full, n, p.N), u = ld4bf(X + p.geglu_I, full, n, p.N);
    s.w = u32x4{g[0], g[1], u[0], u[1]};
  } else if constexpr (EM == EM_DACT) {
    const u32x2 x = ld4bf(p.aux + m * p.ld_aux + n, full, n, p.N);
    s.w = u32x4{x[0], x[1], 0u, 0u};
  } else if constexpr (EM == EM_F32) {
    if (p.beta) {
      const float* Cp = reinterpret_cast<const float*>(p.C) + cofs + m * p.ldc + n;
      if (full) {
        s.w = *reinterpret_cast<const u32x4*>(Cp);
      } else {
#pragma unroll
        for (int r = 0; r < 4; ++r) s.w[r] = n + r < p.N ? __float_as_uint(Cp[r]) : 0u;
      }
    } else if (p.resid) {
      const u32x2 x = ld4bf(p.resid + rofs + m * p.ld_resid + n, full, n, p.N);
      s.w = u32x4{0u, 0u, x[0], x[1]};
    }
  } else {
    u32x2 x0{0u, 0u}, x1{0u, 0u};
    if (p.resid) x1 = ld4bf(p.resid + rofs + m * p.ld_resid + n, full, n, p.N);
    if (p.beta) x0 = ld4bf(reinterpret_cast<const bf16_t*>(p.C) + cofs + m * p.ldc + n, full, n, p.N);
    s.w = u32x4{x0[0], x0[1], x1[0], x1[1]};
  }
// ... 198 lines not shown
```

open-pi-zero_amd/pizero_native/_lib.py:

```python

from __future__ import annotations

import ctypes as C
import os

_HERE = os.path.dirname(os.path.dirname(os.path.abspath(__file__)))
LIB_PATH = os.path.join(_HERE, "libpizero_hip.so")
if os.environ.get("PZ_LIB_PATH"):
    LIB_PATH = os.path.join(_HERE, os.path.basename(os.environ["PZ_LIB_PATH"]))
    import sys as _sys

    print(f"[pizero_native] PZ_LIB_PATH override: loading {LIB_PATH} instead of the default libpizero_hip.so",
          file=_sys.stderr, flush=True)

ABI_VERSION = 22
PZ_EPI_NONE, PZ_EPI_GELU, PZ_EPI_GEGLU, PZ_EPI_SILU = 0, 1, 2, 3
PZ_EPI_DGELU, PZ_EPI_DSILU, PZ_EPI_DGEGLU = 4, 5, 6
PZ_SUMSQ_PARTS = 2048
PZ_OBS_MAX_TAPS, PZ_OBS_MAX_EXTENT = 64, 16384
PZ_OBS_NORM_BOUND, PZ_OBS_NORM_GAUSSIAN = 0, 1

i64, i32, f32, vp = C.c_int64, C.c_int32, C.c_float, C.c_void_p
fp = C.POINTER(C.c_float)

# ... 35 lines not shown
        ("mask", vp), ("ldm", i64), ("mask_bstride", i64),
    ]


class FlashArgs(C.Structure):
    _fields_ = [
        ("Z", i64), ("H", i64), ("nq", i64), ("nk", i64), ("head_dim", i64),
        ("q", vp), ("ldq", i64), ("q_bstride", i64), ("q_hstride", i64),
        ("k", vp), ("ldk", i64), ("k_bstride", i64), ("k_hstride", i64),
        ("v", vp), ("ldv", i64), ("v_bstride", i64), ("v_hstride", i64),
        ("n_groups", i32),
        ("g_row0", i64 * 3), ("g_o", vp * 3), ("g_bstride", i64 * 3), ("g_ld", i64 * 3),
        ("o_hstride", i64),
        ("lse", vp),
        ("scale", f32), ("cap", f32),
        ("mask_mode", i32),
        ("cnt", vp), ("prefix", i64), ("cond", i64), ("rows_per_token", i64),
        ("g_do", vp * 3),
        ("delta", vp),
        ("dq", vp), ("dk", vp), ("dv", vp),
        ("ws", vp), ("ws_bytes", i64),
        ("mask_row0", i64),
    ]


class AdamW8Args(C.Structure):
    _fields_ = [
        ("p", vp), ("g", vp), ("s1", vp), ("s2", vp), ("absmax1", vp), ("absmax2", vp),
        ("m32", vp), ("v32", vp), ("seg", vp), ("nseg", i64), ("nblocks", i64),
        ("qmap1", vp), ("qmap2", vp),
        ("beta1", f32), ("beta2", f32), ("omb1", f32), ("omb2", f32), ("step", f32), ("epsc", f32),
        ("decay", f32), ("gscale", vp),
    ]


class QkvRopeArgs(C.Structure):
    _fields_ = [
        ("x", vp), ("ldx", i64), ("W", vp), ("ldw", i64), ("M", i64), ("N", i64), ("K", i64),
        ("norm_w", vp), ("norm_eps", f32), ("pos", vp), ("cs", vp), ("q_out", vp), ("k_out", vp), ("v_out", vp),
        ("T", i64), ("nh", i64), ("hd", i64), ("Lq", i64), ("qoff", i64), ("Lk", i64), ("koff", i64),
        ("w_fp8", i32), ("w_scale", f32),
        ("x2", vp), ("ldx2", i64), ("W2", vp), ("ldw2", i64), ("K2", i64),
    ]


class ReduceSeg(C.Structure):
    _fields_ = [("part", vp), ("P", i64), ("D", i64), ("out", vp), ("beta", i32)]


class DecodeAttnArgs(C.Structure):
    _fields_ = [
        ("q", vp), ("ldq", i64), ("Lq", i64), ("qoff", i64), ("k", vp), ("v", vp), ("k_bstride", i64),
        ("v_bstride", i64), ("o", vp), ("ldo", i64), ("B", i64), ("nh", i64), ("T", i64), ("nk", i64),
        ("head_dim", i64), ("scale", f32), ("cap", f32), ("cnt", vp), ("prefix", i64), ("cond", i64),
        ("qtok0", i64), ("ws", vp), ("ws_bytes", i64),
    ]


SIGNATURES = {
    "pz_gemm": [C.POINTER(GemmArgs), vp],
    "pz_fp8_quant_rows": [vp, i64, vp, i64, vp, i64, i64, vp],
    "pz_fp8_quant_tensor": [vp, i64, vp, f32, vp],
    "pz_fp8_quant_vt": [vp, i64, i64, i64, i64, vp, vp, i64, vp],
    "pz_rmsnorm_fwd_f8": [vp, i64, vp, vp, i64, vp, i64, i64, f32, vp],
    "pz_layernorm_fwd_f8": [vp, i64, vp, vp, vp, i64, vp, i64, i64, f32, vp],
    "pz_fp8_quant_attn": [vp, i64, vp, i64, vp, i64, i64, i64, i64, vp, vp, vp, vp, vp, vp, i64, vp],
    "pz_flash_fwd_f8": [C.POINTER(FlashArgs), vp, vp, vp, vp, i64, vp, vp, i64, vp],
    "pz_fp8_absmax": [vp, i64, vp, vp],
    "pz_gemm_kernel_name": [C.POINTER(GemmArgs)],
    "pz_gemm_small": [C.POINTER(SmallGemmArgs), vp],
    "pz_rmsnorm_fwd": [vp, i64, vp, vp, i64, vp, i64, i64, f32, vp],
    "pz_rmsnorm_bwd": [vp, i64, vp, i64, vp, vp, vp, vp, i64, vp, i64, i64, vp],
    "pz_layernorm_fwd": [vp, i64, vp, vp, vp, i64, vp, vp, i64, i64, f32, vp],
    "pz_layernorm_bwd": [vp, i64, vp, i64, vp, vp, vp, vp, vp, i64, vp, vp, i64, i64, vp, vp],
    "pz_act_bwd_colsum": [vp, i64, vp, i64, vp, i64, i64, i32, vp, i64, vp, i32, vp],
    "pz_reduce_parts_multi": [vp, i32, vp],
    "pz_norm_rows_per_part": [],
    "pz_reduce_parts": [vp, i64, i64, vp, i32, vp],
    "pz_colsum": [vp, i64, i64, i64, vp, i32, vp, vp],
    "pz_batch_sum": [vp, i64, i64, i64, vp, i32, vp],
    "pz_rope_table": [vp, i64, i64, f32, vp],
    "pz_qkv_rope_split": [vp, vp, vp, vp, vp, vp, i64, i64, i64, i64, i64, i64, i64, i64, i64, vp],
    "pz_qkv_rope_split_bwd": [vp, vp, vp, vp, vp, vp, i64, i64, i64, i64, i64, i64, i64, i64, i64, vp],
    "pz_gemv_qkv_rope": [C.POINTER(QkvRopeArgs), vp],
    "pz_gemm_qkv_rope": [C.POINTER(QkvRopeArgs), vp],
    "pz_decode_attn": [C.POINTER(DecodeAttnArgs), vp],
    "pz_decode_attn_ws_bytes": [i64, i64, i64],
    "pz_attn_softmax": [C.POINTER(SoftmaxArgs), vp],
    "pz_attn_softmax_bwd": [vp, vp, i64, vp, vp, i64, i64, i64, f32, f32, vp],
    "pz_flash_fwd": [C.POINTER(FlashArgs), vp],
    "pz_flash_fwd_probs": [C.POINTER(FlashArgs), vp, vp, i64, vp],
    "pz_flash_bwd_ds": [C.POINTER(FlashArgs), vp, vp, vp, i64, vp],
    "pz_flash_bwd_prep": [C.POINTER(FlashArgs), vp],
    "pz_flash_bwd": [C.POINTER(FlashArgs), vp],
    "pz_patchify": [vp, vp, i64, i64, i64, i64, i64, vp],
    "pz_embed_merge": [vp, vp, i64, vp, vp, i64, i64, i64, i64, i64, i64, f32, f32, vp],
    "pz_embed_merge_bwd": [vp, vp, vp, i64, i64, i64, i64, i64, f32, vp],
    "pz_time_embed": [vp, vp, i64, i64, f32, i32, vp],
    "pz_concat_time": [vp, vp, vp, i64, i64, i64, vp],
    "pz_split_time_grad": [vp, vp, i64, i64, vp],
    "pz_flow_psi": [vp, vp, vp, vp, i64, i64, f32, vp],
    "pz_flow_loss": [vp, i64, i64, vp, vp, vp, vp, vp, i64, i64, i64, f32, vp],
    "pz_euler_step": [vp, vp, i64, i64, vp, i64, i64, i64, f32, vp],
    "pz_action_in": [vp, i64, vp, vp, vp, vp, i64, i64, i64, i64, f32, i32, vp],
    "pz_action_out": [vp, i64, vp, f32, vp, vp, i64, i64, vp, vp, i64, i64, f32, vp],
    "pz_copy_rows": [vp, i64, i64, vp, i64, i64, i64, i64, i64, f32, i32, vp],
    "pz_time_embed_rows": [vp, vp, i64, i64, i64, i64, f32, i32, vp],
    "pz_clamp": [vp, i64, f32, f32, vp],
    "pz_geglu_bwd": [vp, i64, vp, i64, vp, vp, i64, i64, i64, vp],
    "pz_act_bwd": [vp, i64, vp, i64, vp, vp, i64, i64, i64, i32, vp],
    "pz_adamw": [vp, vp, vp, vp, i64, f32, f32, f32, f32, f32, f32, f32, vp, vp],
    "pz_adamw8bit": [C.POINTER(AdamW8Args), vp],
    "pz_adamw8bit_r": [C.POINTER(AdamW8Args), vp, i32, C.c_uint64, i64, vp],
    "pz_adamw_r": [vp, vp, vp, vp, vp, i64, f32, f32, f32, f32, f32, f32, f32, vp, i32, C.c_uint64, i64, vp],
    "pz_sumsq": [vp, i64, vp, vp],
    "pz_clip_coef": [vp, i64, vp, vp, f32, vp],
    "pz_fill_uniform": [vp, i32, i64, C.c_uint64, f32, f32, vp],
    "pz_cast_f32_bf16": [vp, vp, i64, vp],
    "pz_cast_bf16_f32": [vp, vp, i64, vp],
    "pz_adaln_fwd": [vp, i64, vp, i64, vp, vp, vp, i64, vp, vp, vp, vp, i64, vp, i64, i64, i64, i64, f32, vp],
    "pz_adaln_norm_bwd": [vp, i64, vp, i64, vp, vp, vp, vp, vp, i64, vp, vp, i64, i64, i64, i64, vp],
    "pz_adaln_gate_bwd": [vp, i64, vp, i64, vp, vp, vp, i64, vp, i64, i64, i64, i64, vp],
    "pz_lora_wgrad_ws_bytes": [i64, i64, i64],
    "pz_lora_wgrad": [vp, i64, vp, i64, vp, i64, i64, i64, i64, i32, f32, i32, vp, i64, vp],
    "pz_avg_lerp": [vp, vp, i64, f32, vp],
    "pz_avg_swap": [vp, vp, i64, vp],
    "pz_image_resize_scratch_bytes": [i64, i64, i64],
    "pz_image_resize_norm": [vp, i32, i64, i64, i64, i64, vp, vp, vp, i64, vp, vp, vp, i64, vp, vp, i64, vp, vp],
    "pz_proprio_normalize": [vp, vp, i64, i64, vp, vp, i32, vp],
    "pz_action_denormalize": [vp, vp, i64, i64, i64, vp, vp, i32, vp],
    "pz_debug_poison_lds": [C.c_uint32, vp],
    "pz_debug_spin": [i64, i64, vp],
    "pz_last_error": [],
    "pz_abi_version": [],
}
_RESTYPE = {"pz_last_error": C.c_char_p, "pz_gemm_kernel_name": C.c_char_p, "pz_norm_rows_per_part": i64,
            "pz_decode_attn_ws_bytes": i64, "pz_lora_wgrad_ws_bytes": i64, "pz_image_resize_scratch_bytes": i64}

_lib = None


class NativeError(RuntimeError):
    pass


def lib():
    global _lib
    if _lib is None:
        if not os.path.exists(LIB_PATH):
            raise NativeError(
                f"{LIB_PATH} not found: build it with `python open-pi-zero_amd/build_native.py` "
                "(or __graft_entry__.build()); the Pi0 path has no CPU/eager fallback")
        L = C.CDLL(LIB_PATH)
        for name, argt in SIGNATURES.items():
            fn = getattr(L, name)
            fn.argtypes = argt
            fn.restype = _RESTYPE.get(name, C.c_int)
        if L.pz_abi_version() != ABI_VERSION:
            raise NativeError(f"{LIB_PATH}: ABI version {L.pz_abi_version()} != {ABI_VERSION}; rebuild it")
        _lib = L
    return _lib


_NO_LAUNCH = {"pz_last_error", "pz_abi_version", "pz_gemm_kernel_name", "pz_norm_rows_per_part",
              "pz_decode_attn_ws_bytes", "pz_lora_wgrad_ws_bytes", "pz_debug_poison_lds",
              "pz_image_resize_scratch_bytes"}
_POISON_LDS = [0xFFFFFFFF if os.environ.get("PZ_POISON_LDS", "0") == "1" else None]


_RECENT = [[] if os.environ.get("PZ_CHECK_FINITE", "0") == "1" else None]


def recent_launches(clear=True):
    r = _RECENT[0] or []
    if clear and _RECENT[0] is not None:
        _RECENT[0] = []
    return r


def set_poison_lds(word):
    _POISON_LDS[0] = None if word is None else int(word) & 0xFFFFFFFF


def call(name, *args):
    if _POISON_LDS[0] is not None and name not in _NO_LAUNCH:
        rc = lib().pz_debug_poison_lds(_POISON_LDS[0], args[-1])
        if rc != 0:
            raise NativeError(f"pz_debug_poison_lds failed (rc={rc}): {lib().pz_last_error().decode(errors='replace')}")
    if _RECENT[0] is not None:
        _RECENT[0].append(name)
    rc = getattr(lib(), name)(*args)
    if rc != 0:
        msg = lib().pz_last_error().decode(errors="replace")
        raise NativeError(f"{name} failed (rc={rc}): {msg}")
    return rc
```

open-pi-zero_amd/pizero_native/engine.py:

```python

from __future__ import annotations

import contextlib
import functools
import math
import os
import weakref
from dataclasses import dataclass

import torch

from . import ops
from .ops import PZ_EPI_DGEGLU, PZ_EPI_GEGLU, PZ_EPI_GELU, PZ_EPI_NONE, PZ_EPI_SILU

BF16 = torch.bfloat16
F32 = torch.float32


def _cfg(cfg, key, default=None):
    from src.utils.config import cfg_get

    return cfg_get(cfg, key, default)


# ... 181 lines not shown
        sl = eng.ar.slots
        self.r = sl[self.a[0]].shape[0]
        self.S = len(wnames)
        self.outs = [sl[n].shape[0] for n in self.b]
        self._b2 = None
        self._b2_ver = None

    def A(self):
        return self.eng.ar.span(self.a[0], self.a[-1])

    def B2(self):
        ar = self.eng.ar
        if self.S == 1:
            return ar.view(self.b[0])
        ver = self.eng.weights_version()
        if self._b2 is None or self._b2_ver != ver or self._b2.device != ar.data.device:
            if self._b2 is None or self._b2.device != ar.data.device:
                self._b2 = torch.zeros(sum(self.outs), self.S * self.r, device=ar.data.device, dtype=ar.data.dtype)
            r0 = 0
            for i, (n, o) in enumerate(zip(self.b, self.outs)):
                self._b2[r0:r0 + o, i * self.r:(i + 1) * self.r].copy_(ar.view(n))
                r0 += o
            self._b2_ver = ver
        return self._b2

    def fwd(self, x):
        u = torch.empty(x.shape[0], self.S * self.r, device=x.device, dtype=x.dtype)
        ops.linear(x, self.A(), u)
        return u, self.B2()

    def bwd(self, dy):
        v = torch.empty(dy.shape[0], self.S * self.r, device=dy.device, dtype=dy.dtype)
        ops.linear_dgrad(dy, self.B2(), v)
        return v, self.A()

    def grads(self, x, u, dy, v, beta):
        from src.model.lora import LORA_SCALING

        eng, r, c0 = self.eng, self.r, 0
        for i, o in enumerate(self.outs):
            if eng.rg(self.a[i]):
                ops.lora_wgrad(x, v[:, i * r:(i + 1) * r], eng.gw(self.a[i]), alpha=LORA_SCALING, beta=beta)
            if eng.rg(self.b[i]):
                ops.lora_wgrad(dy[:, c0:c0 + o], u[:, i * r:(i + 1) * r], eng.gw(self.b[i]), transposed=True,
                               alpha=LORA_SCALING, beta=beta)
            c0 += o


def _merged_weights(fn):

    @functools.wraps(fn)
    def wrap(self, *a, **k):
        if not self.m.has_lora:
            return fn(self, *a, **k)
        if not torch.cuda.is_current_stream_capturing():
            self.lora_refresh()
        prev, self._infer = self._infer, True
        try:
            return fn(self, *a, **k)
        finally:
            self._infer = prev

    return wrap


class Group:

    def __init__(self, name, prefix, mixtures, T, joint_off, hidden, inter, theta, skip_last, pos_key):
        self.name, self.prefix, self.mixtures = name, prefix, mixtures
        self.T, self.off, self.hid, self.inter, self.theta = T, joint_off, hidden, inter, theta
        self.skip_last = skip_last
        self.pos_key = pos_key


class Engine:
    def __init__(self, model):
        self.m = model
        self.d = Dims.from_cfg(model.cfg)
        self._tables = {}
        self._ws = {}
        self._jkv_holder = None
        self.joint_flash = False
        self.joint_probs = True
        self.infer_flash = True
        self.fuse_qkv_rope = self.d.hd == 256
        self.expert_stream = True
        self.expert_stream_fwd = False
        self.sig_pitch = (self.d.vI + 63) // 64 * 64
        self._side = {}
        self.check_finite = os.environ.get("PZ_CHECK_FINITE", "0") == "1"
        self.f8 = None
        self.f8_version = None
        self._lora_sites = {}
        self._lora_w = frozenset(n[: -len("lora_A")] + "weight" for n in self.ar.slots if n.endswith(".lora_A"))
        self._merged = None
        self._merged_ver = None
        self._infer = False
        if self.d.nkv != 1:
            raise NotImplementedError("joint attention kernel path assumes MQA (num_key_value_heads=1, bridge.yaml:176)")

    def ada_slots(self, prefix):
        key = ("ada_slots", prefix)
        sl = self._tables.get(key)
        if sl is None:
            from src.model.vla.pizero import adaln_slots

            sl = self._tables[key] = adaln_slots(prefix, self.d.nL, self.d.ada)
        return sl

    def _chk(self, where, **tensors):
        if not self.check_finite:
            return
        check_finite(where, **tensors)

    @property
    def ar(self):
        return self.m._arena

    def w(self, name):
        return self.ar.view(name, self._merged if self._infer and name in self._lora_w else None)

    def span(self, first, last):
        return self.ar.span(first, last, self._merged if self._infer and first in self._lora_w else None)

    def lora(self, *wnames):
        if wnames[0] not in self._lora_w:
            return None
        st = self._lora_sites.get(wnames)
        if st is None:
            st = self._lora_sites[wnames] = LoraSite(self, wnames)
        return st

    def lora_refresh(self):
        if not self._lora_w:
            return False
        ver = self.weights_version()
        if self._merged is not None and self._merged_ver == ver and self._merged.device == self.ar.data.device:
            return False
        from src.model.lora import LORA_SCALING

        if self._merged is None or self._merged.device != self.ar.data.device:
            self._merged = torch.empty_like(self.ar.data)
        for wn in sorted(self._lora_w):
            W = self.ar.view(wn)
            A = self.ar.view(wn[: -len("weight")] + "lora_A")
            Bm = self.ar.view(wn[: -len("weight")] + "lora_B")
            out, inn = W.shape
            ops.gemm(out, inn, A.shape[0], Bm, A.shape[0], True, A, inn, False, self.ar.view(wn, self._merged), inn,
                     alpha=LORA_SCALING, resid=W, ld_resid=inn)
        self._merged_ver = ver
        return True

    def gw(self, name):
        return self.ar.grad_view(name)

    def rg(self, name):
        return self.m._requires_grad(name)

    def qkv_w(self, p):
        return self.span(p + "self_attn.q_proj.weight", p + "self_attn.v_proj.weight")

    def gu_w(self, p):
        return self.span(p + "mlp.gate_proj.weight", p + "mlp.up_proj.weight")

    @_merged_weights
    def prepare_fp8(self):
# ... 628 lines not shown
                                 sA=(L * nh * Lp, 0), sB=(Lp * hd, 0), sC=(g.T * nh * hd, 0))
                st["O"] = Os
            if side is not None:
                side.wait_stream(main)
                for t in Os.values():
                    t.record_stream(side)
            for g in groups:
                gs = st["g"][g.name]
                if last and g.skip_last:
                    X[g.name] = None
                    gs["skip"] = True
                    continue
                with self._on(side, g):
                    if ada and g.name in ada:
                        self._post_attn_ada(ada[g.name], g, l, X, gs, Os, dev)
                    else:
                        self._post_attn_train(g, l, X, gs, Os, dev)
            layers.append(st)
            self._chk(f"joint fwd layer {l}", Q=Qj, K=Kj, V=Vj, O=Os, P=st.get("P"), tc=st.get("tc"), X=X)
        if side is not None:
            main.wait_stream(side)
            for t in X.values():
                if t is not None:
                    t.record_stream(main)
            for st in layers:
                for g in groups:
                    if g.name != "vlm":
                        for t in st["g"][g.name].values():
                            if isinstance(t, torch.Tensor):
                                t.record_stream(main)
        save["joint"] = layers
        return X

    def _mlp_oproj_backward(self, g, gs, p, dX, dO, dXm, beta, rpp, nh, hd, dev, A=None, l=None):
        dx = dres = dX[g.name]
        M = dx.shape[0]
        part = None if A is not None else torch.empty((M + rpp - 1) // rpp, g.hid, device=dev, dtype=F32)
        if A is not None and A.zero:
            dx = ops.adaln_gate_bwd(dres, gs["yd"], A.mod, A.biased(l, "final_z"), torch.empty_like(dres), A.dmod, g.T)
            gs["yd"] = None
        gu = gs["gu"]
        s_o = self.lora(p + "self_attn.o_proj.weight")
        s_gu = self.lora(p + "mlp.gate_proj.weight", p + "mlp.up_proj.weight")
        s_dn = self.lora(p + "mlp.down_proj.weight")
        lo = None
        if s_dn is not None:
            lo = s_dn.bwd(dx)
            s_dn.grads(gs["hm"], gs["u_dn"], dx, lo[0], beta)
        ops.linear_dgrad(dx, self.w(p + "mlp.down_proj.weight"), gu, epi=PZ_EPI_DGEGLU, aux=gu, lora=lo)
        if self.rg(p + "mlp.down_proj.weight"):
            ops.linear_wgrad(dx, gs["hm"], self.gw(p + "mlp.down_proj.weight"), beta=beta)
        gs["hm"] = None
        if self.rg(p + "mlp.gate_proj.weight") and self.rg(p + "mlp.up_proj.weight"):
            ops.linear_wgrad(gu, gs["h2"], self.ar.grad_span(p + "mlp.gate_proj.weight", p + "mlp.up_proj.weight"),
                             beta=beta)
        dh2 = torch.empty(M, g.hid, device=dev, dtype=BF16)
        lo = None
        if s_gu is not None:
            lo = s_gu.bwd(gu)
            s_gu.grads(gs["h2"], gs["u_gu"], gu, lo[0], beta)
        ops.linear_dgrad(gu, self.gu_w(p), dh2, lora=lo)
        dxm = torch.empty_like(dx)
        if A is not None:
            A.norm_bwd(dh2, gs["xm"], gs["r2"], l, "post_", g.T, dxm, dres=dres)
        else:
            ops.rmsnorm_bwd(dh2, gs["xm"], self.w(p + "post_attention_layernorm.weight"), gs["r2"], dxm, dres=dx,
                            dw_part=part)
            self._norm_grads(p + "post_attention_layernorm.", part, None, beta)
        dyo = dxm
        if A is not None and A.zero:
            dyo = ops.adaln_gate_bwd(dxm, gs["yo"], A.mod, A.biased(l, "post_z"), torch.empty_like(dxm), A.dmod, g.T)
            gs["yo"] = None
        if self.rg(p + "self_attn.o_proj.weight"):
            ops.linear_wgrad(dyo, gs["O"], self.gw(p + "self_attn.o_proj.weight"), beta=beta)
        o = torch.empty(M, nh * hd, device=dev, dtype=BF16)
        lo = None
        if s_o is not None:
            lo = s_o.bwd(dyo)
            s_o.grads(gs["O"], gs["u_o"], dyo, lo[0], beta)
        ops.linear_dgrad(dyo, self.w(p + "self_attn.o_proj.weight"), o, lora=lo)
        dO[g.name] = o
        dXm[g.name] = dxm

    def _qkv_backward(self, g, gs, p, dQ, dK, dV, dX, dXm, pos, B, L, Lp, beta, rpp, nh, hd, dev, A=None, l=None):
        x = gs["x"]
        M = x.shape[0]
        W = (nh + 2) * hd
        dqkv = torch.empty(M, W, device=dev, dtype=BF16)
        ops.qkv_rope_split_bwd(None if gs.get("skip") else dQ, dK, dV, pos[g.pos_key], self.rope(g.theta), dqkv,
                               B, g.T, nh, 1, hd, L, g.off, Lp, g.off)
        names = [p + f"self_attn.{k}_proj.weight" for k in "qkv"]
        rgs = [self.rg(n) for n in names]
        site = self.lora(*names)
        lo = None
        if site is not None:
            lo = site.bwd(dqkv)
            site.grads(gs["h"], gs["u_qkv"], dqkv, lo[0], beta)
        if gs.get("skip") and site is None:
            if rgs[0] and not beta:
                self.gw(names[0]).zero_()
            for n, rgk, c0, c1 in zip(names[1:], rgs[1:], (nh * hd, (nh + 1) * hd), ((nh + 1) * hd, W)):
                if rgk:
                    ops.linear_wgrad(dqkv[:, c0:c1], gs["h"], self.gw(n), beta=beta)
            dh = torch.empty(M, g.hid, device=dev, dtype=BF16)
            ops.linear_dgrad(dqkv[:, nh * hd:], self.span(names[1], names[2]), dh)
        else:
            if all(rgs):
                ops.linear_wgrad(dqkv, gs["h"], self.ar.grad_span(names[0], names[2]), beta=beta)
            elif rgs[0] and rgs[1]:
                ops.linear_wgrad(dqkv[:, : (nh + 1) * hd], gs["h"], self.ar.grad_span(names[0], names[1]),
                                 beta=beta)
            else:
                for n, rgk, c0, c1 in zip(names, rgs, (0, nh * hd, (nh + 1) * hd), (nh * hd, (nh + 1) * hd, W)):
                    if rgk:
                        ops.linear_wgrad(dqkv[:, c0:c1], gs["h"], self.gw(n), beta=beta)
            dh = torch.empty(M, g.hid, device=dev, dtype=BF16)
            ops.linear_dgrad(dqkv, self.qkv_w(p), dh, lora=lo)
        dxn = torch.empty(M, g.hid, device=dev, dtype=BF16)
        if A is not None:
            A.norm_bwd(dh, x, gs["r"], l, "in_", g.T, dxn, dres=dXm.get(g.name))
        else:
            part = torch.empty((M + rpp - 1) // rpp, g.hid, device=dev, dtype=F32)
            ops.rmsnorm_bwd(dh, x, self.w(p + "input_layernorm.weight"), gs["r"], dxn, dres=dXm.get(g.name),
                            dw_part=part)
            self._norm_grads(p + "input_layernorm.", part, None, beta)
        dX[g.name] = dxn

    def _joint_layers_backward(self, groups, dX, pos, cnt, B, sv, beta):
        d = self.d
        L, Lp, nh, hd = d.L, d.Lp, d.nh, d.hd
        dev = next(v for v in dX.values() if v is not None).device
        delta = dP = dS = None
        rpp = ops.rows_per_part()
        main = torch.cuda.current_stream(dev)
        side = None
        if self.expert_stream and len(groups) > 1 and dev.type == "cuda":
            side = self._side_stream(dev)
            side.wait_stream(main)
            for st in sv["joint"]:
                for g in groups:
                    if g.name != "vlm":
                        for t in st["g"][g.name].values():
                            if isinstance(t, torch.Tensor):
                                t.record_stream(side)
            for t in dX.values():
                if t is not None:
                    t.record_stream(side)
            for A in (sv.get("ada") or {}).values():
                A.mod.record_stream(side)
                A.dmod.record_stream(side)
        ada = sv.get("ada") or {}
        for l in reversed(range(d.nL)):
            st = sv["joint"][l]
            dQ = torch.empty(B, L, nh * hd, device=dev, dtype=BF16)
            dK = torch.empty(B, Lp, hd, device=dev, dtype=BF16)
            dV = torch.empty(B, Lp, hd, device=dev, dtype=BF16)
            dO = {}
            dXm = {}
            any_skip = False
            for g in groups:
                gs = st["g"][g.name]
                p = f"{g.prefix}{l}."
                if gs.get("skip"):
                    any_skip = True
                    continue
                with self._on(side, g):
                    self._mlp_oproj_backward(g, gs, p, dX, dO, dXm, beta, rpp, nh, hd, dev, ada.get(g.name), l)
                if side is not None and g.name != "vlm":
                    dO[g.name].record_stream(main)
            if side is not None:
                main.wait_stream(side)
            if "lse" in st:
                for g in groups:
                    if g.name not in dO:
                        dO[g.name] = torch.zeros(B * g.T, nh * hd, device=dev, dtype=BF16)
                if delta is None:
                    delta = torch.empty(B, L * nh, device=dev, dtype=F32)
                ops.flash_bwd(self._joint_flash(groups, st["Q"], st["K"], st["V"], st["O"], st["lse"], cnt, B, L,
                                                dO=dO, delta=delta, dq=dQ, dk=dK, dv=dV))
            else:
                Pm, tc, Qj, Kj, Vj = st["P"], st["tc"], st["Q"], st["K"], st["V"]
                dq_done = False
                if not isinstance(cnt, GeneralMask) and L <= 320 and hd == 256:
                    if dS is None:
                        dS = torch.empty(B, L * nh, Lp, device=dev, dtype=BF16)
                    ops.flash_bwd_ds(self._joint_flash(groups, Qj, Kj, Vj, st["O"], None, cnt, B, L, dO=dO,
                                                       dq=dQ), Pm, tc, dS, Lp)
                    dq_done = True
                else:
                    if dP is None:
                        dP = torch.empty(B, L * nh, Lp, device=dev, dtype=F32)
                    if dS is None:
                        dS = torch.empty(B, L * nh, Lp, device=dev, dtype=BF16)
                    if any_skip:
                        dP.zero_()
                    for g in groups:
                        if g.name not in dO:
                            continue
                        ops.gemm(g.T * nh, L, hd, dO[g.name], hd, True, Vj, hd, True, dP[:, g.off * nh:], Lp,
                                 batch=B, sA=(g.T * nh * hd, 0), sB=(Lp * hd, 0), sC=(L * nh * Lp, 0))
                    ops.attn_softmax_bwd(Pm, dP, Lp, tc, dS, Lp, B * L * nh, L, 1.0 / math.sqrt(hd), 50.0)
                if not dq_done:
                    ops.gemm(L * nh, hd, Lp, dS, Lp, True, Kj, hd, False, dQ, hd, batch=B, sA=(L * nh * Lp, 0),
                             sB=(Lp * hd, 0), sC=(L * nh * hd, 0))
                ops.gemm(Lp, hd, L * nh, dS, Lp, False, Qj, hd, False, dK, hd, batch=B, sA=(L * nh * Lp, 0),
                         sB=(L * nh * hd, 0), sC=(Lp * hd, 0))
                first = True
                for g in sorted(groups, key=lambda g: g.T):
                    if g.name not in dO:
                        continue
                    ops.gemm(Lp, hd, g.T * nh, Pm[:, g.off * nh:], Lp, False, dO[g.name], hd, False, dV, hd, batch=B,
                             sA=(L * nh * Lp, 0), sB=(g.T * nh * hd, 0), sC=(Lp * hd, 0), beta=not first)
                    first = False
                if first:
                    dV.zero_()
            if side is not None:
                side.wait_stream(main)
                for t in (dQ, dK, dV):
                    t.record_stream(side)
            for g in groups:
                with self._on(side, g):
                    self._qkv_backward(g, st["g"][g.name], f"{g.prefix}{l}.", dQ, dK, dV, dX, dXm, pos, B, L, Lp, beta,
                                       rpp, nh, hd, dev, ada.get(g.name), l)
            self._chk(f"joint bwd layer {l}", dO=dO, dS=dS, dQ=dQ, dK=dK, dV=dV, dX=dX)
            self._notify("joint", l, (side,) if side is not None else ())
        if side is not None:
            main.wait_stream(side)
            for t in dX.values():
                if t is not None:
                    t.record_stream(main)
        sv.pop("_jkv_token", None)
        return dX

    def train_forward(self, ids, pix, cnt, pos, proprios, actions, t, x0, save):
        d = self.d
        dev = pix.device
        B = ids.shape[0]
        tied = self.m._tied
        sv_v = {}
        img = self.siglip_forward(pix, sv_v)
        Xv = self.embed_prefix(ids, img)
        prop = proprios.reshape(B * d.C, d.Pd).to(BF16)
        pe = torch.empty(B * d.C, d.aH, device=dev, dtype=BF16)
        ops.small_linear(prop, self.w("proprio_encoder.weight"), pe, bias=self.w("proprio_encoder.bias"))
        psi = torch.empty(B * d.H, d.A, device=dev, dtype=BF16)
        ops.flow_psi(x0, actions, t, psi, d.sig_min)
        e3 = self.action_embed(psi, t, save)
        sa = math.sqrt(d.aH)
        if tied:
            Xe = torch.empty(B * (d.C + d.H), d.aH, device=dev, dtype=BF16)
            T = d.C + d.H
            ops.copy_rows(pe, d.aH, d.C * d.aH, Xe, d.aH, T * d.aH, B, d.C, d.aH, scale=sa)
            ops.copy_rows(e3, d.aH, d.H * d.aH, Xe[d.C:], d.aH, T * d.aH, B, d.H, d.aH, scale=sa)
            X = {"vlm": Xv, "expert": Xe}
        else:
            Xp = torch.empty(B * d.C, d.aH, device=dev, dtype=BF16)
            Xa = torch.empty(B * d.H, d.aH, device=dev, dtype=BF16)
            ops.copy_rows(pe, d.aH, 0, Xp, d.aH, 0, 1, B * d.C, d.aH, scale=sa)
            ops.copy_rows(e3, d.aH, 0, Xa, d.aH, 0, 1, B * d.H, d.aH, scale=sa)
            X = {"vlm": Xv, "proprio": Xp, "action": Xa}
        groups = self.groups(tied)
        if d.ada:
            cond = torch.empty(B, d.tH, device=dev, dtype=BF16)
            ops.time_embed(t, cond, d.tmax, ref_bf16=d.time_bf16)
            save["cond"] = cond
            save["ada"] = {g.name: Ada(self, g, cond) for g in groups if g.name != "vlm"}
        X = self._joint_layers_train(groups, X, pos, cnt, B, save)
        ag = "expert" if tied else "action"
        aoff = d.C if tied else 0
        Tg = d.C + d.H if tied else d.H
        Xl = X[ag]
        ya = torch.empty_like(Xl)
        ra = torch.empty(Xl.shape[0], device=dev, dtype=F32)
        if d.ada:
            save["ada"][ag].norm_fwd(Xl, "norm", "", Tg, ya, ra)
        else:
            ops.rmsnorm(Xl, self.w("joint_model.mixtures.action.norm.weight"), ya, ra, d.rms_eps)
        v = torch.empty(B * Tg, 8, device=dev, dtype=BF16)
        ops.small_linear(ya, self.w("action_decoder.weight"), v, bias=self.w("action_decoder.bias"))
        loss = torch.empty(1, device=dev, dtype=F32)
        ops.flow_loss(v[aoff:], 8, Tg * 8, x0, actions, loss, None, None, B, d.H, d.A, d.sig_min)
        save.update(sv_v=sv_v, ids=ids, cnt=cnt, pos=pos, B=B, prop=prop, pe=pe, tied=tied, Xl=Xl, ya=ya, ra=ra,
                    x0=x0, x1=actions, v=v, ag=ag, aoff=aoff, Tg=Tg, groups=groups)
        self._chk("train fwd head (action norm, decoder, flow loss)", embed=Xv, ya=ya, v=v, loss=loss)
        return loss

    def train_backward(self, sv, grad_loss, beta):
        d = self.d
        B = sv["B"]
        dev = sv["v"].device
        Tg, aoff = sv["Tg"], sv["aoff"]
        ws = self.colsum_ws(2 * d.aH)
        rpp = ops.rows_per_part()
        dv = torch.zeros(B * Tg, 8, device=dev, dtype=BF16)
        tmp = torch.empty(1, device=dev, dtype=F32)
        ops.flow_loss(sv["v"][aoff:], 8, Tg * 8, sv["x0"], sv["x1"], tmp, dv[aoff:], grad_loss, B, d.H, d.A, d.sig_min)
        R = B * Tg
        if self.rg("action_decoder.weight"):
            ops.small_gemm(d.A, d.aH, R, dv, 1, 8, sv["ya"], d.aH, 1, self.gw("action_decoder.weight"), d.aH, beta=beta)
        if self.rg("action_decoder.bias"):
            ops.colsum(dv[:, : d.A], self.gw("action_decoder.bias"), ws, beta=beta)
        dya = torch.empty(R, d.aH, device=dev, dtype=BF16)
        ops.small_gemm(R, d.aH, d.A, dv, 8, 1, self.w("action_decoder.weight"), d.aH, 1, dya, d.aH)
        dXl = torch.empty_like(dya)
        ada = sv.get("ada")
        if ada:
# ... 519 lines not shown
```

open-pi-zero_amd/pizero_native/ops.py:

```python

from __future__ import annotations

import ctypes as C

import torch

from ._lib import (
    PZ_EPI_DGEGLU,
    PZ_EPI_DGELU,
    PZ_EPI_DSILU,
    PZ_EPI_GEGLU,
    PZ_EPI_GELU,
    PZ_EPI_NONE,
    PZ_EPI_SILU,
    PZ_OBS_MAX_EXTENT,
    PZ_OBS_MAX_TAPS,
    PZ_OBS_NORM_BOUND,
    PZ_OBS_NORM_GAUSSIAN,
    PZ_SUMSQ_PARTS,
    AdamW8Args,
    QkvRopeArgs,
    DecodeAttnArgs,
    FlashArgs,
    GemmArgs,
# ... 427 lines not shown
    need = lib().pz_decode_attn_ws_bytes(B, T * nh, nk)
    ws = workspace(o.device)
    if ws.numel() * 4 < need:
        raise ValueError(f"decode_attn: {B} samples x {nk} keys need {need} B of workspace (> {ws.numel() * 4})")
    a.ws, a.ws_bytes = _p(ws), ws.numel() * 4
    call("pz_decode_attn", C.byref(a), _st())


def attn_softmax(S, lds, P, ldp, R, N, scale, cap=0.0, tcap=None, mask_mode=0, rows_per_batch=1, heads=1,
                 qoff=0, cnt=None, prefix=0, cond=0, mask=None, ldm=0, mask_bstride=0):
    a = SoftmaxArgs()
    a.S, a.lds, a.P, a.ldp, a.tcap = _p(S), lds, _p(P), ldp, _p(tcap)
    a.R, a.N, a.scale, a.cap, a.mask_mode = R, N, float(scale), float(cap), mask_mode
    a.rows_per_batch, a.heads, a.qoff = rows_per_batch, heads, qoff
    a.cnt, a.prefix, a.cond = _p(cnt), prefix, cond
    a.mask, a.ldm, a.mask_bstride = _p(mask), ldm, mask_bstride
    call("pz_attn_softmax", C.byref(a), _st())


def attn_softmax_bwd(P, dP, lddp, tcap, dS, ldp, R, N, scale, cap):
    call("pz_attn_softmax_bwd", _p(P), _p(dP), lddp, _p(tcap), _p(dS), ldp, R, N, float(scale), float(cap),
         _st())


def flash_args(Z, H, nq, nk, hd, q, q_strides, k, k_strides, v, v_strides, groups, o_hstride, lse, scale,
               cap=0.0, mask_mode=0, cnt=None, prefix=0, cond=0, rows_per_token=1, dgroups=None, delta=None,
               dq=None, dk=None, dv=None, mask_row0=0, key_split=False):
    a = FlashArgs()
    a.Z, a.H, a.nq, a.nk, a.head_dim = int(Z), int(H), int(nq), int(nk), int(hd)
    a.q, (a.ldq, a.q_bstride, a.q_hstride) = _p(q), tuple(int(x) for x in q_strides)
    a.k, (a.ldk, a.k_bstride, a.k_hstride) = _p(k), tuple(int(x) for x in k_strides)
    a.v, (a.ldv, a.v_bstride, a.v_hstride) = _p(v), tuple(int(x) for x in v_strides)
    a.n_groups = len(groups)
    for i, (r0, o, bs, ld) in enumerate(groups):
        a.g_row0[i], a.g_o[i], a.g_bstride[i], a.g_ld[i] = int(r0), _p(o), int(bs), int(ld)
        if dgroups is not None:
            a.g_do[i] = _p(dgroups[i])
    a.o_hstride = int(o_hstride)
    a.lse = _p(lse)
    a.scale, a.cap, a.mask_mode = float(scale), float(cap), int(mask_mode)
    a.cnt, a.prefix, a.cond, a.rows_per_token = _p(cnt), int(prefix), int(cond), int(rows_per_token)
    a.mask_row0 = int(mask_row0)
    a.delta, a.dq, a.dk, a.dv = _p(delta), _p(dq), _p(dk), _p(dv)
    if dq is not None or key_split:
        ws = flash_workspace(q.device)
        a.ws, a.ws_bytes = ws.data_ptr(), ws.numel() * ws.element_size()
    return a


_FLASH_WS_BYTES = 320 << 20
_FLASH_WS = {}


def flash_workspace(device):
    dev = torch.device(device)
    ws = _FLASH_WS.get(dev)
    if ws is None:
        ws = torch.empty(_FLASH_WS_BYTES // 4, dtype=torch.float32, device=dev)
        _FLASH_WS[dev] = ws
    return ws


def flash_fwd(a):
    call("pz_flash_fwd", C.byref(a), _st())


def fp8_quant_vt(v, Z, nk, vt, vs):
    call("pz_fp8_quant_vt", _p(v), v.stride(1), v.stride(0), Z, nk, _p(vt), _p(vs), vt.shape[2], _st())


def fp8_quant_attn(q, k, v, Z, nk, qc, qs, kc, ks, vt, vs):
    call("pz_fp8_quant_attn", _p(q), q.shape[0], _p(k), k.shape[0], _p(v), v.stride(1), v.stride(0), Z, nk, _p(qc),
         _p(qs), _p(kc), _p(ks), _p(vt), _p(vs), vt.shape[2], _st())


def flash_fwd_f8(a, qc, qs, kc, ks, krows, vt, vs):
    call("pz_flash_fwd_f8", C.byref(a), _p(qc), _p(qs), _p(kc), _p(ks), int(krows), _p(vt), _p(vs), vt.shape[2], _st())


def flash_bwd_ds(a, P, tcap, dS, ldp):
    call("pz_flash_bwd_ds", C.byref(a), _p(P), _p(tcap), _p(dS), int(ldp), _st())


def flash_fwd_probs(a, P, tcap, ldp):
    call("pz_flash_fwd_probs", C.byref(a), _p(P), _p(tcap), int(ldp), _st())


def flash_bwd(a):
    call("pz_flash_bwd", C.byref(a), _st())


def flash_bwd_prep(a):
    call("pz_flash_bwd_prep", C.byref(a), _st())


def siglip_flash_args(qkv, O, lse, B, nh, hd, N, dO=None, delta=None, dqkv=None):
    W = qkv.stride(0)
    H = nh * hd
    strides = (W, N * W, hd)
    return flash_args(B, nh, N, N, hd, qkv, strides, qkv[:, H:], strides, qkv[:, 2 * H:], strides,
                      [(0, O, N * O.stride(0), O.stride(0))], hd, lse, hd ** -0.5,
                      dgroups=None if dO is None else [dO], delta=delta,
                      dq=dqkv, dk=None if dqkv is None else dqkv[:, H:], dv=None if dqkv is None else dqkv[:, 2 * H:])


def patchify(pix, cols, ps):
    B, _, H, W = pix.shape
    call("pz_patchify", _p(pix), _p(cols), B, H, W, ps, cols.stride(0), _st())


def embed_merge(ids, table, img, out, n_img, image_token, pad_token, emb_scale, img_scale):
    B, P = ids.shape
    D = table.shape[1]
    call("pz_embed_merge", _p(ids), _p(table), table.shape[0], _p(img), _p(out), B, P, D, n_img, image_token,
         pad_token,
         float(emb_scale), float(img_scale), _st())


def embed_merge_bwd(ids, dout, dimg, n_img, image_token, img_scale):
    B, P = ids.shape
    D = dout.shape[-1]
    call("pz_embed_merge_bwd", _p(ids), _p(dout), _p(dimg), B, P, D, n_img, image_token, float(img_scale),
         _st())


def time_embed(t, out, max_period, ref_bf16=False):
    B, D = out.shape
    call("pz_time_embed", _p(t), _p(out), B, D, float(max_period), int(bool(ref_bf16)), _st())


def time_embed_rows(t, out, H, max_period, ref_bf16=False):
    rows, D = out.shape
    call("pz_time_embed_rows", _p(t), _p(out), out.stride(0), rows // H, H, D, float(max_period), int(bool(ref_bf16)),
         _st())


def concat_time(temb, e1, out, B, H, D):
    call("pz_concat_time", _p(temb), _p(e1), _p(out), B, H, D, _st())


def split_time_grad(dcat, de1, rows, D):
    call("pz_split_time_grad", _p(dcat), _p(de1), rows, D, _st())


def flow_psi(x0, x1, t, psi, sig_min):
    B = x0.shape[0]
    call("pz_flow_psi", _p(x0), _p(x1), _p(t), _p(psi), B, x0[0].numel(), float(sig_min), _st())


def flow_loss(v, ldv, vbs, x0, x1, loss, dv, grad_scale, B, H, A, sig_min):
    call("pz_flow_loss", _p(v), ldv, vbs, _p(x0), _p(x1), _p(loss), _p(dv), _p(grad_scale), B, H, A,
         float(sig_min), _st())


def action_in(action, W1, b1, t, cat, B, H, D, max_period, ref_bf16=False):
    A = action.shape[-1]
    call("pz_action_in", _p(action), A, _p(W1), _p(b1), _p(t), _p(cat), cat.stride(0), B, H, D, float(max_period),
         int(bool(ref_bf16)), _st())


def action_out(x, norm_w, eps, Wd, bd, action, t, B, H, dt):
    D = x.shape[1]
    call("pz_action_out", _p(x), x.stride(0), _p(norm_w), float(eps), _p(Wd), _p(bd), D, Wd.shape[0], _p(action),
         _p(t), B, H, float(dt), _st())


def euler_step(action, v, ldv, vbs, t, B, H, A, dt):
    call("pz_euler_step", _p(action), _p(v), ldv, vbs, _p(t), B, H, A, float(dt), _st())
# ... 219 lines not shown
```

Before: 277.2 samples/s.

## Fuse dQ RoPE-backward into flash dS kernel and widen attention stores

The joint-attention backward dS kernel now applies the inverse RoPE to dQ and writes it straight into each group's packed dqkv buffer. This removes the separate dQ tensor and its re-read in the split kernel, and a new vectorized kernel fills only the dK/dV part of dqkv. The probs, tcap, O and dQ stores in the flash kernels are widened to 16-byte writes using permlane16 swaps, with a debug switch to fall back to the old narrow stores. The cost is more code paths, and the fused path hardcodes hd=256 and assumes the expected alignment.

```diff
diff --git a/include/pz_abi.h b/include/pz_abi.h
--- a/include/pz_abi.h
+++ b/include/pz_abi.h
@@ -119,6 +119,8 @@
 int pz_qkv_rope_split_bwd(const void* dq, const void* dk, const void* dv, const int64_t* pos,
                           const float* cs, void* dqkv, int64_t B, int64_t T, int64_t nh, int64_t nkv,
                           int64_t hd, int64_t Lq, int64_t qoff, int64_t Lk, int64_t koff, void* stream);
+int pz_qkv_rope_split_bwd_kv(const void* dk, const void* dv, const int64_t* pos, const float* cs, void* dqkv, int64_t B,
+                             int64_t T, int64_t nh, int64_t nkv, int64_t hd, int64_t Lk, int64_t koff, void* stream);
 
 typedef struct pz_softmax_args {
   const float* S; int64_t lds;
@@ -160,6 +162,9 @@
                     int64_t krows, const void* vtc, const float* vs, int64_t ldvt, void* stream);
 int pz_flash_fwd_probs(const pz_flash_args* a, void* P, void* tcap, int64_t ldp, void* stream);
 int pz_flash_bwd_ds(const pz_flash_args* a, const void* P, const void* tcap, void* dS, int64_t ldp, void* stream);
+int pz_flash_bwd_ds_rope(const pz_flash_args* a, const void* P, const void* tcap, void* dS, int64_t ldp,
+                         void* const* dqkv, const int64_t* ld_dqkv, const int64_t* const* pos, const float* const* cs,
+                         void* stream);
 int pz_flash_bwd_prep(const pz_flash_args* a, void* stream);
 int pz_flash_bwd(const pz_flash_args* a, void* stream);
 
@@ -276,6 +281,7 @@
 
 int pz_debug_poison_lds(uint32_t word, void* stream);
 int pz_debug_spin(int64_t wgs, int64_t ticks, void* stream);
+int pz_debug_narrow_stores(int32_t on);
 
 const char* pz_last_error(void);
 int pz_abi_version(void);
diff --git a/open-pi-zero_amd/csrc/pz_attn.hip b/open-pi-zero_amd/csrc/pz_attn.hip
--- a/open-pi-zero_amd/csrc/pz_attn.hip
+++ b/open-pi-zero_amd/csrc/pz_attn.hip
@@ -71,8 +71,7 @@
     if (sq) {
       const float y1 = bf2f(sq[h * hd + i]), y2 = bf2f(sq[h * hd + i + half]);
       const float co = c[2 * i], si = c[2 * i + 1];
-      o1 = y1 * co + y2 * si;
-      o2 = y2 * co - y1 * si;
+      rope_pair_bwd<true>(y1, y2, co, si, o1, o2);
     }
     dst[h * hd + i] = f2bf(o1);
     dst[h * hd + i + half] = f2bf(o2);
@@ -85,10 +84,58 @@
     const int h = e / half, i = e % half;
     const float y1 = bf2f(sk[h * hd + i]), y2 = bf2f(sk[h * hd + i + half]);
     const float co = c[2 * i], si = c[2 * i + 1];
-    ok[h * hd + i] = f2bf(y1 * co + y2 * si);
-    ok[h * hd + i + half] = f2bf(y2 * co - y1 * si);
+    float o1, o2;
+    rope_pair_bwd<false>(y1, y2, co, si, o1, o2);
+    ok[h * hd + i] = f2bf(o1);
+    ok[h * hd + i + half] = f2bf(o2);
   }
   for (int e = threadIdx.x; e < nkv * hd; e += blockDim.x) ov[e] = sv[e];
+}
+
+__device__ __forceinline__ void unpack8bf(const u32x4& w, float (&v)[8]) {
+#pragma unroll
+  for (int j = 0; j < 4; ++j) {
+    v[2 * j] = __uint_as_float(w[j] << 16);
+    v[2 * j + 1] = __uint_as_float(w[j] & 0xffff0000u);
+  }
+}
+
+__global__ void __launch_bounds__(256) qkv_rope_split_bwd_kv_kernel(const bf16_t* __restrict__ dk,
+                                                                    const bf16_t* __restrict__ dv,
+                                                                    const int64_t* __restrict__ pos,
+                                                                    const float* __restrict__ cs, bf16_t* dqkv,
+                                                                    int64_t toks, int64_t T, int nh, int nkv, int hd,
+                                                                    int64_t Lk, int64_t koff) {
+  const int half = hd / 2, kun = nkv * half / 8, per = kun + nkv * hd / 8;
+  const int64_t id = (int64_t)blockIdx.x * blockDim.x + threadIdx.x;
+  const int64_t tok = id / per;
+  if (tok >= toks) return;
+  const int u = (int)(id - tok * per);
+  const int64_t b = tok / T, t = tok - b * T;
+  const int64_t src = (b * Lk + koff + t) * (int64_t)(nkv * hd);
+  bf16_t* dst = dqkv + tok * (int64_t)((nh + 2 * nkv) * hd) + nh * hd;
+  if (u >= kun) {
+    const int e = (u - kun) * 8;
+    *reinterpret_cast<u32x4*>(dst + nkv * hd + e) = *reinterpret_cast<const u32x4*>(dv + src + e);
+    return;
+  }
+  const int h = u / (half / 8), i = (u % (half / 8)) * 8;
+  const u32x4 w1 = *reinterpret_cast<const u32x4*>(dk + src + h * hd + i);
+  const u32x4 w2 = *reinterpret_cast<const u32x4*>(dk + src + h * hd + i + half);
+  const float4* c = reinterpret_cast<const float4*>(cs + pos[tok] * hd + 2 * i);
+  float y1[8], y2[8], o1[8], o2[8];
+  unpack8bf(w1, y1);
+  unpack8bf(w2, y2);
+#pragma unroll
+  for (int q = 0; q < 4; ++q) {
+    const float4 c2 = c[q];
+    rope_pair_bwd<false>(y1[2 * q], y2[2 * q], c2.x, c2.y, o1[2 * q], o2[2 * q]);
+    rope_pair_bwd<false>(y1[2 * q + 1], y2[2 * q + 1], c2.z, c2.w, o1[2 * q + 1], o2[2 * q + 1]);
+  }
+  *reinterpret_cast<u32x4*>(dst + h * hd + i) =
+      u32x4{pack2bf(o1[0], o1[1]), pack2bf(o1[2], o1[3]), pack2bf(o1[4], o1[5]), pack2bf(o1[6], o1[7])};
+  *reinterpret_cast<u32x4*>(dst + h * hd + i + half) =
+      u32x4{pack2bf(o2[0], o2[1]), pack2bf(o2[2], o2[3]), pack2bf(o2[4], o2[5]), pack2bf(o2[6], o2[7])};
 }
 
 __device__ __forceinline__ bool block_allowed(int64_t i, int64_t j, int64_t cnt, int64_t P, int64_t C) {
@@ -370,6 +417,23 @@
   hipLaunchKernelGGL(qkv_rope_split_bwd_kernel, dim3((unsigned)T, (unsigned)B), dim3(256), 0,
                      (hipStream_t)stream, (const bf16_t*)dq, (const bf16_t*)dk, (const bf16_t*)dv, pos, cs,
                      (bf16_t*)dqkv, T, (int)nh, (int)nkv, (int)hd, Lq, qoff, Lk, koff);
+  PZ_CHECK_LAUNCH();
+  return PZ_OK;
+}
+
+extern "C" int pz_qkv_rope_split_bwd_kv(const void* dk, const void* dv, const int64_t* pos, const float* cs, void* dqkv,
+                                        int64_t B, int64_t T, int64_t nh, int64_t nkv, int64_t hd, int64_t Lk,
+                                        int64_t koff, void* stream) {
+  PZ_CHECK_ARG(dk && dv && pos && cs && dqkv && B > 0 && T > 0 && nh >= 0 && nkv > 0 && hd > 0,
+               "qkv_rope_split_bwd_kv: bad args");
+  PZ_CHECK_ARG(koff >= 0 && koff + T <= Lk, "qkv_rope_split_bwd_kv: token range");
+  PZ_CHECK_ARG(hd % 16 == 0 && PZ_ALIGNED(dk, 16) && PZ_ALIGNED(dv, 16) && PZ_ALIGNED(dqkv, 16) && PZ_ALIGNED(cs, 16),
+               "qkv_rope_split_bwd_kv: needs hd %% 16 == 0 and 16-byte aligned dK / dV / dqkv / cs");
+  const int64_t per = nkv * hd / 16 + nkv * hd / 8, n = B * T * per;
+  PZ_CHECK_ARG((n + 255) / 256 < (1LL << 31), "qkv_rope_split_bwd_kv: too many tokens");
+  hipLaunchKernelGGL(qkv_rope_split_bwd_kv_kernel, dim3((unsigned)((n + 255) / 256)), dim3(256), 0,
+                     (hipStream_t)stream, (const bf16_t*)dk, (const bf16_t*)dv, pos, cs, (bf16_t*)dqkv, B * T, T,
+                     (int)nh, (int)nkv, (int)hd, Lk, koff);
   PZ_CHECK_LAUNCH();
   return PZ_OK;
 }
diff --git a/open-pi-zero_amd/csrc/pz_common.h b/open-pi-zero_amd/csrc/pz_common.h
--- a/open-pi-zero_amd/csrc/pz_common.h
+++ b/open-pi-zero_amd/csrc/pz_common.h
@@ -25,6 +25,13 @@
 __device__ __forceinline__ unsigned pack2bf(float lo, float hi) {
   return __builtin_bit_cast(unsigned, __builtin_convertvector(f32x2_t{lo, hi}, bf16x2_t));
 }
+
+__device__ __forceinline__ u32x4 pair16(u32x2 a, u32x2 b) {
+  const auto r0 = __builtin_amdgcn_permlane16_swap(a[0], b[0], false, false);
+  const auto r1 = __builtin_amdgcn_permlane16_swap(a[1], b[1], false, false);
+  return u32x4{r0[0], r1[0], r0[1], r1[1]};
+}
+__device__ __forceinline__ int pair16_col(int g) { return (g & 1) * 16 + 4 * (g & 2); }
 
 __device__ __forceinline__ uint64_t splitmix64(uint64_t z) {
   z += 0x9E3779B97F4A7C15ull;
@@ -92,6 +99,7 @@
 int pz_gemv_launch(const pz_gemm_args* a, hipStream_t st);
 
 void pz_set_error(const char* fmt, ...);
+extern int g_pz_narrow_stores;
 #define PZ_CHECK_ARG(cond, ...)          \
   do {                                   \
     if (!(cond)) {                       \
@@ -114,3 +122,9 @@
   o1 = x1 * co - x2 * si;
   o2 = x2 * co + x1 * si;
 }
+template <bool Q>
+__device__ __forceinline__ void rope_pair_bwd(float y1, float y2, float co, float si, float& o1, float& o2) {
+#pragma clang fp contract(off)
+  o1 = Q ? __builtin_fmaf(y2, si, y1 * co) : __builtin_fmaf(y1, co, y2 * si);
+  o2 = __builtin_fmaf(y2, co, -(y1 * si));
+}
diff --git a/open-pi-zero_amd/csrc/pz_flash.hip b/open-pi-zero_amd/csrc/pz_flash.hip
--- a/open-pi-zero_amd/csrc/pz_flash.hip
+++ b/open-pi-zero_amd/csrc/pz_flash.hip
@@ -2210,7 +2210,7 @@
 
 template <bool CAP>
 __global__ void __launch_bounds__(JP_NW * 64, 1) flash_fwd_probs_dma_kernel(pz_flash_args a, bf16_t* P, bf16_t* TC,
-                                                                         int64_t ldp) {
+                                                                         int64_t ldp, int wide) {
   extern __shared__ __attribute__((aligned(16))) char fa_smem[];
   constexpr int RPW = JP_NW * 16;
   const int lane = threadIdx.x & 63, wave = threadIdx.x >> 6, g = lane >> 4, l15 = lane & 15;
@@ -2301,17 +2301,29 @@
   }
   logits_blk(JP_MAXKB - 1);
   FS_WAIT_VM(4);
+  const bool wide_p = wide & 1;
+  const int pc = pair16_col(g);
   bf16_t* prow = P + (b * a.nq + (live ? r : 0)) * ldp;
   if (TC) {
     bf16_t* trow = TC + (b * a.nq + (live ? r : 0)) * ldp;
 #pragma unroll
-    for (int kb = 0; kb < JP_MAXKB; ++kb)
-#pragma unroll
-      for (int i = 0; i < 4; ++i) {
-        const int j0 = kb * FA_KB + i * 16 + 4 * g;
-        if (clean && (kb + 1) * 64 <= full_keys) *reinterpret_cast<u32x2*>(trow + j0) = tcv[kb][i];
-        else if (live && j0 < ldp) *reinterpret_cast<u32x2*>(trow + j0) = tcv[kb][i];
-      }
+    for (int kb = 0; kb < JP_MAXKB; ++kb) {
+      const bool fast = clean && (kb + 1) * 64 <= full_keys;
+      if (wide_p) {
+#pragma unroll
+        for (int i = 0; i < 4; i += 2) {
+          const u32x4 v = pair16(tcv[kb][i], tcv[kb][i + 1]);
+          const int j0 = kb * FA_KB + i * 16 + pc;
+          if (fast || (live && j0 < ldp)) *reinterpret_cast<u32x4*>(trow + j0) = v;
+        }
+      } else {
+#pragma unroll
+        for (int i = 0; i < 4; ++i) {
+          const int j0 = kb * FA_KB + i * 16 + 4 * g;
+          if (fast || (live && j0 < ldp)) *reinterpret_cast<u32x2*>(trow + j0) = tcv[kb][i];
+        }
+      }
+    }
   }
   mx = fs_max4(mx);
   float sum = 0.f;
@@ -2348,7 +2360,16 @@
           pk[i][1] = pack2bf(pv[2], pv[3]);
         }
         const int j0 = kb * FA_KB + i * 16 + 4 * g;
-        if (decltype(FAST)::value || (live && j0 < ldp)) *reinterpret_cast<u32x2*>(prow + j0) = u32x2{pk[i][0], pk[i][1]};
+        if (!wide_p && (decltype(FAST)::value || (live && j0 < ldp)))
+          *reinterpret_cast<u32x2*>(prow + j0) = u32x2{pk[i][0], pk[i][1]};
+      }
+      if (wide_p) {
+#pragma unroll
+        for (int i = 0; i < 4; i += 2) {
+          const u32x4 v = pair16(u32x2{pk[i][0], pk[i][1]}, u32x2{pk[i + 1][0], pk[i + 1][1]});
+          const int j0 = kb * FA_KB + i * 16 + pc;
+          if (decltype(FAST)::value || (live && j0 < ldp)) *reinterpret_cast<u32x4*>(prow + j0) = v;
+        }
       }
     };
     if (clean && (kb + 1) * 64 <= full_keys) probs(std::true_type{});
@@ -2388,6 +2409,14 @@
   const FaRow fr{&a};
   const int gi = fr.grp(r);
   bf16_t* O = (bf16_t*)a.g_o[gi] + fr.off(b, h, r, gi);
+  if (wide & 2) {
+#pragma unroll
+    for (int db = 0; db < 16; db += 2)
+      *reinterpret_cast<u32x4*>(O + db * 16 + pc) =
+          pair16(u32x2{pack2bf(o[db][0], o[db][1]), pack2bf(o[db][2], o[db][3])},
+                 u32x2{pack2bf(o[db + 1][0], o[db + 1][1]), pack2bf(o[db + 1][2], o[db + 1][3])});
+    return;
+  }
 #pragma unroll
   for (int db = 0; db < 16; ++db) {
     const int d = db * 16 + 4 * g;
@@ -2395,8 +2424,17 @@
   }
 }
 
+struct JdRope {
+  bf16_t* dqkv[3];
+  int64_t ld[3], T[3];
+  const int64_t* pos[3];
+  const float* cs[3];
+};
+
+template <bool ROPE>
 __global__ void __launch_bounds__(JP_NW * 64, 1) flash_bwd_ds_dma_kernel(pz_flash_args a, const bf16_t* P,
-                                                                      const bf16_t* TC, bf16_t* dS, int64_t ldp) {
+                                                                      const bf16_t* TC, bf16_t* dS, int64_t ldp,
+                                                                      int wide, JdRope rp) {
   extern __shared__ __attribute__((aligned(16))) char fa_smem[];
   constexpr int RPW = JP_NW * 16;
   const int lane = threadIdx.x & 63, wave = threadIdx.x >> 6, g = lane >> 4, l15 = lane & 15;
@@ -2406,7 +2444,7 @@
   const int64_t b = zh / a.H, h = zh % a.H;
   const int64_t r = (int64_t)qblk * RPW + wave * 16 + l15;
   const bool live = r < a.nq;
-  const bool want_dq = a.dq != nullptr;
+  const bool want_dq = ROPE || a.dq != nullptr;
   const bf16_t* V = (const bf16_t*)a.v + b * a.v_bstride + h * a.v_hstride;
   const bf16_t* K = want_dq ? (const bf16_t*)a.k + b * a.k_bstride + h * a.k_hstride : V;
   const int64_t ldk = want_dq ? a.ldk : a.ldv;
@@ -2519,7 +2557,16 @@
       }
       pk[i][0] = pack2bf(x[0], x[1]);
       pk[i][1] = pack2bf(x[2], x[3]);
-      if (clean ? j0 < ldp : (live && j0 < ldp)) *reinterpret_cast<u32x2*>(orow + j0) = u32x2{pk[i][0], pk[i][1]};
+      if (!(wide & 1) && (clean ? j0 < ldp : (live && j0 < ldp)))
+        *reinterpret_cast<u32x2*>(orow + j0) = u32x2{pk[i][0], pk[i][1]};
+    }
+    if (wide & 1) {
+#pragma unroll
+      for (int i = 0; i < 4; i += 2) {
+        const u32x4 v = pair16(u32x2{pk[i][0], pk[i][1]}, u32x2{pk[i + 1][0], pk[i + 1][1]});
+        const int j0 = kb * FA_KB + i * 16 + pair16_col(g);
+        if (clean ? j0 < ldp : (live && j0 < ldp)) *reinterpret_cast<u32x4*>(orow + j0) = v;
+      }
     }
     dsf[kb][0] = __builtin_bit_cast(bf16x8, u32x4{pk[0][0], pk[0][1], pk[1][0], pk[1][1]});
     dsf[kb][1] = __builtin_bit_cast(bf16x8, u32x4{pk[2][0], pk[2][1], pk[3][0], pk[3][1]});
@@ -2554,7 +2601,48 @@
     }
   }
   if (!live || !want_dq) return;
+  if constexpr (ROPE) {
+    const FaRow fr{&a};
+    const int gi = fr.grp(r);
+    const int64_t rr = r - a.g_row0[gi];
+    const int64_t tg = rr / a.rows_per_token, hh = rr - tg * a.rows_per_token;
+    const int64_t tok = b * rp.T[gi] + tg;
+    const float* c = rp.cs[gi] + rp.pos[gi][tok] * 256 + 8 * g;
+    bf16_t* dst = rp.dqkv[gi] + tok * rp.ld[gi] + hh * 256 + pair16_col(g);
+    u32x2 lo[8], hi[8];
+#pragma unroll
+    for (int db = 0; db < 8; ++db) {
+      const float4 c0 = *reinterpret_cast<const float4*>(c + 32 * db);
+      const float4 c1 = *reinterpret_cast<const float4*>(c + 32 * db + 4);
+      const float co[4] = {c0.x, c0.z, c1.x, c1.z}, si[4] = {c0.y, c0.w, c1.y, c1.w};
+      const u32x2 w1{pack2bf(dq[db][0], dq[db][1]), pack2bf(dq[db][2], dq[db][3])};
+      const u32x2 w2{pack2bf(dq[db + 8][0], dq[db + 8][1]), pack2bf(dq[db + 8][2], dq[db + 8][3])};
+      const float y1[4] = {__uint_as_float(w1[0] << 16), __uint_as_float(w1[0] & 0xffff0000u),
+                           __uint_as_float(w1[1] << 16), __uint_as_float(w1[1] & 0xffff0000u)};
+      const float y2[4] = {__uint_as_float(w2[0] << 16), __uint_as_float(w2[0] & 0xffff0000u),
+                           __uint_as_float(w2[1] << 16), __uint_as_float(w2[1] & 0xffff0000u)};
+      float o1[4], o2[4];
+#pragma unroll
+      for (int e = 0; e < 4; ++e) rope_pair_bwd<true>(y1[e], y2[e], co[e], si[e], o1[e], o2[e]);
+      lo[db] = u32x2{pack2bf(o1[0], o1[1]), pack2bf(o1[2], o1[3])};
+      hi[db] = u32x2{pack2bf(o2[0], o2[1]), pack2bf(o2[2], o2[3])};
+    }
+#pragma unroll
+    for (int db = 0; db < 8; db += 2) {
+      *reinterpret_cast<u32x4*>(dst + db * 16) = pair16(lo[db], lo[db + 1]);
+      *reinterpret_cast<u32x4*>(dst + 128 + db * 16) = pair16(hi[db], hi[db + 1]);
+    }
+    return;
+  }
   bf16_t* dQ = (bf16_t*)a.dq + b * a.q_bstride + h * a.q_hstride + r * a.ldq;
+  if (wide & 2) {
+#pragma unroll
+    for (int db = 0; db < 16; db += 2)
+      *reinterpret_cast<u32x4*>(dQ + db * 16 + pair16_col(g)) =
+          pair16(u32x2{pack2bf(dq[db][0], dq[db][1]), pack2bf(dq[db][2], dq[db][3])},
+                 u32x2{pack2bf(dq[db + 1][0], dq[db + 1][1]), pack2bf(dq[db + 1][2], dq[db + 1][3])});
+    return;
+  }
 #pragma unroll
   for (int db = 0; db < 16; ++db) {
     const int d = db * 16 + 4 * g;
@@ -2888,24 +2976,32 @@
                "flash_fwd_probs: operands need 16-byte aligned rows");
   PZ_CHECK_ARG(a->nq + a->mask_row0 < (1 << 22) && a->Z * a->H < 65536, "flash_fwd_probs: nq / units too large");
   const int64_t units = a->Z * a->H, nqb = (a->nq + JP_NW * 16 - 1) / (JP_NW * 16);
+  int wide = 0;
+  if (!g_pz_narrow_stores) {
+    if (ldp % 32 == 0 && PZ_ALIGNED(P, 16) && (!tcap || PZ_ALIGNED(tcap, 16))) wide |= 1;
+    bool o16 = a->o_hstride % 8 == 0;
+    for (int i = 0; i < a->n_groups; ++i)
+      o16 = o16 && PZ_ALIGNED(a->g_o[i], 16) && a->g_ld[i] % 8 == 0 && a->g_bstride[i] % 8 == 0;
+    if (o16) wide |= 2;
+  }
   {
     static bool attr0 = false, attr1 = false;
     if (a->cap > 0.f) {
       fa_smem_attr(flash_fwd_probs_dma_kernel<true>, JD_SMEM, attr1);
       hipLaunchKernelGGL(flash_fwd_probs_dma_kernel<true>, dim3((unsigned)(nqb * units)), dim3(JP_NW * 64), JD_SMEM,
-                         (hipStream_t)stream, *a, (bf16_t*)P, (bf16_t*)tcap, ldp);
+                         (hipStream_t)stream, *a, (bf16_t*)P, (bf16_t*)tcap, ldp, wide);
     } else {
       fa_smem_attr(flash_fwd_probs_dma_kernel<false>, JD_SMEM, attr0);
       hipLaunchKernelGGL(flash_fwd_probs_dma_kernel<false>, dim3((unsigned)(nqb * units)), dim3(JP_NW * 64), JD_SMEM,
-                         (hipStream_t)stream, *a, (bf16_t*)P, (bf16_t*)tcap, ldp);
+                         (hipStream_t)stream, *a, (bf16_t*)P, (bf16_t*)tcap, ldp, wide);
     }
     PZ_CHECK_LAUNCH();
     return PZ_OK;
   }
 }
 
-extern "C" int pz_flash_bwd_ds(const pz_flash_args* a, const void* P, const void* tcap, void* dS, int64_t ldp,
-                               void* stream) {
+static int fa_bwd_ds(const pz_flash_args* a, const void* P, const void* tcap, void* dS, int64_t ldp, const JdRope* rope,
+                     void* stream) {
   PZ_CHECK_ARG(a && a->v && P && dS && a->Z > 0 && a->H > 0 && a->nq > 0 && a->nk > 0, "flash_bwd_ds: bad args");
   PZ_CHECK_ARG(a->head_dim == 256, "flash_bwd_ds: head_dim %lld (256 only)", (long long)a->head_dim);
   PZ_CHECK_ARG(a->nk <= JP_MAXKB * FA_KB && ldp >= a->nk && ldp % 4 == 0, "flash_bwd_ds: nk %lld / ldp %lld",
@@ -2920,14 +3016,59 @@
     PZ_CHECK_ARG(a->k && PZ_ALIGNED(a->k, 16) && a->ldk % 8 == 0 && a->k_bstride % 8 == 0 && PZ_ALIGNED(a->dq, 8) &&
                      a->ldq % 4 == 0 && a->q_bstride % 4 == 0,
                  "flash_bwd_ds: dQ needs K (16-byte rows) and an 8-byte aligned dQ");
+  if (rope)
+    PZ_CHECK_ARG(a->k && PZ_ALIGNED(a->k, 16) && a->ldk % 8 == 0 && a->k_bstride % 8 == 0 && a->H == 1 &&
+                     a->rows_per_token > 0,
+                 "flash_bwd_ds_rope: needs K (16-byte rows), H == 1 (heads stacked as rows) and rows_per_token");
   PZ_CHECK_ARG(a->Z * a->H < 65536, "flash_bwd_ds: too many units");
   const int64_t units = a->Z * a->H, nqb = (a->nq + JP_NW * 16 - 1) / (JP_NW * 16);
-  static bool attr = false;
-  fa_smem_attr(flash_bwd_ds_dma_kernel, JD_SMEM, attr);
-  hipLaunchKernelGGL(flash_bwd_ds_dma_kernel, dim3((unsigned)(nqb * units)), dim3(JP_NW * 64), JD_SMEM,
-                     (hipStream_t)stream, *a, (const bf16_t*)P, (const bf16_t*)tcap, (bf16_t*)dS, ldp);
+  int wide = 0;
+  if (!g_pz_narrow_stores) {
+    if (ldp % 32 == 0 && PZ_ALIGNED(dS, 16)) wide |= 1;
+    if (a->dq && PZ_ALIGNED(a->dq, 16) && a->ldq % 8 == 0 && a->q_bstride % 8 == 0 && a->q_hstride % 8 == 0) wide |= 2;
+  }
+  static bool attr = false, attr_r = false;
+  if (rope) {
+    fa_smem_attr(flash_bwd_ds_dma_kernel<true>, JD_SMEM, attr_r);
+    hipLaunchKernelGGL(flash_bwd_ds_dma_kernel<true>, dim3((unsigned)(nqb * units)), dim3(JP_NW * 64), JD_SMEM,
+                       (hipStream_t)stream, *a, (const bf16_t*)P, (const bf16_t*)tcap, (bf16_t*)dS, ldp, wide, *rope);
+  } else {
+    fa_smem_attr(flash_bwd_ds_dma_kernel<false>, JD_SMEM, attr);
+    hipLaunchKernelGGL(flash_bwd_ds_dma_kernel<false>, dim3((unsigned)(nqb * units)), dim3(JP_NW * 64), JD_SMEM,
+                       (hipStream_t)stream, *a, (const bf16_t*)P, (const bf16_t*)tcap, (bf16_t*)dS, ldp, wide, JdRope{});
+  }
   PZ_CHECK_LAUNCH();
   return PZ_OK;
+}
+
+extern "C" int pz_flash_bwd_ds(const pz_flash_args* a, const void* P, const void* tcap, void* dS, int64_t ldp,
+                               void* stream) {
+  return fa_bwd_ds(a, P, tcap, dS, ldp, nullptr, stream);
+}
+
+extern "C" int pz_flash_bwd_ds_rope(const pz_flash_args* a, const void* P, const void* tcap, void* dS, int64_t ldp,
+                                    void* const* dqkv, const int64_t* ld_dqkv, const int64_t* const* pos,
+                                    const float* const* cs, void* stream) {
+  PZ_CHECK_ARG(a && dqkv && ld_dqkv && pos && cs && a->n_groups >= 1 && a->n_groups <= 3,
+               "flash_bwd_ds_rope: bad args");
+  PZ_CHECK_ARG(!a->dq, "flash_bwd_ds_rope: dQ leaves through dqkv (a->dq must be NULL)");
+  JdRope rp{};
+  const int64_t nh = a->rows_per_token;
+  PZ_CHECK_ARG(nh > 0 && a->nq % nh == 0, "flash_bwd_ds_rope: nq must be whole tokens of rows_per_token rows");
+  for (int i = 0; i < a->n_groups; ++i) {
+    const int64_t r0 = a->g_row0[i], r1 = i + 1 < a->n_groups ? a->g_row0[i + 1] : a->nq;
+    PZ_CHECK_ARG(r0 % nh == 0 && r1 > r0 && r1 % nh == 0, "flash_bwd_ds_rope: group %d rows [%lld, %lld)", i,
+                 (long long)r0, (long long)r1);
+    PZ_CHECK_ARG(dqkv[i] && pos[i] && cs[i] && PZ_ALIGNED(dqkv[i], 16) && PZ_ALIGNED(cs[i], 16) &&
+                     ld_dqkv[i] % 8 == 0 && ld_dqkv[i] >= nh * 256,
+                 "flash_bwd_ds_rope: group %d needs dqkv (16-byte rows of >= nh * 256 columns), pos and cs", i);
+    rp.dqkv[i] = (bf16_t*)dqkv[i];
+    rp.ld[i] = ld_dqkv[i];
+    rp.T[i] = (r1 - r0) / nh;
+    rp.pos[i] = pos[i];
+    rp.cs[i] = cs[i];
+  }
+  return fa_bwd_ds(a, P, tcap, dS, ldp, &rp, stream);
 }
 
 extern "C" int pz_flash_bwd_prep(const pz_flash_args* a, void* stream) {
diff --git a/open-pi-zero_amd/csrc/pz_gemm.hip b/open-pi-zero_amd/csrc/pz_gemm.hip
--- a/open-pi-zero_amd/csrc/pz_gemm.hip
+++ b/open-pi-zero_amd/csrc/pz_gemm.hip
@@ -666,10 +666,12 @@
   const int g4 = 4 * (lane >> 4), rl = lane & 15;
   if (GEGLU) {
     if (m0 + BT <= p.M && n0 + BT / 2 <= p.geglu_I && p.aux) {
+      const int ucol = wc * 32 + pair16_col(lane >> 4);
 #pragma unroll
       for (int rb = 0; rb < 8; ++rb) {
         const int64_t m = m0 + wr * 128 + rb * 16 + rl;
-        bf16_t* Ur = p.aux + m * p.ld_aux + p.geglu_I + n0 + wc * 32 + g4;
+        bf16_t* Ur = p.aux + m * p.ld_aux + p.geglu_I + n0;
+        u32x2 uq[2];
 #pragma unroll
         for (int j = 0; j < 2; ++j) {
           float gg[4], hh[4], uu[4];
@@ -682,7 +684,13 @@
           const int row = wr * 128 + rb * 16 + rl, col = wc * 32 + j * 16 + g4;
           img_put(smem, row, col, u32x2{pack2bf(hh[0], hh[1]), pack2bf(hh[2], hh[3])});
           img_put(smem + 65536, row, col, u32x2{pack2bf(gg[0], gg[1]), pack2bf(gg[2], gg[3])});
-          *reinterpret_cast<u32x2*>(Ur + j * 16) = pk4(uu);
+          uq[j] = pk4(uu);
+        }
+        if (p.wide_u) {
+          *reinterpret_cast<u32x4*>(Ur + ucol) = pair16(uq[0], uq[1]);
+        } else {
+          *reinterpret_cast<u32x2*>(Ur + wc * 32 + g4) = uq[0];
+          *reinterpret_cast<u32x2*>(Ur + wc * 32 + g4 + 16) = uq[1];
         }
       }
       lds_sync();
@@ -1405,6 +1413,12 @@
 extern "C" const char* pz_last_error(void) { return g_err; }
 
 extern "C" int pz_abi_version(void) { return PZ_ABI_VERSION; }
+
+int g_pz_narrow_stores = 0;
+extern "C" int pz_debug_narrow_stores(int32_t on) {
+  g_pz_narrow_stores = on != 0;
+  return PZ_OK;
+}
 
 template <bool AKC, bool BKC, int WM, int TAG = 0>
 static int launch_tile(const GemmP& p, int64_t batch, hipStream_t st) {
@@ -1978,6 +1992,7 @@
   p.nw = (const bf16_t*)a->norm_w;
   p.neps = a->norm_eps;
   p.rs = a->fp8_mode == 1 ? a->a_row_scale : nullptr;
+  p.wide_u = !g_pz_narrow_stores && PZ_ALIGNED(a->aux, 16) && a->ld_aux % 8 == 0 && a->geglu_inter % 8 == 0;
   if (a->K2 > 0) {
     p.A2 = (const bf16_t*)a->A2;
     p.B2 = (const bf16_t*)a->B2;
diff --git a/open-pi-zero_amd/csrc/pz_gemm_epi.h b/open-pi-zero_amd/csrc/pz_gemm_epi.h
--- a/open-pi-zero_amd/csrc/pz_gemm_epi.h
+++ b/open-pi-zero_amd/csrc/pz_gemm_epi.h
@@ -31,6 +31,7 @@
   const bf16_t* A2;
   const bf16_t* B2;
   int64_t lda2, ldb2, K2;
+  int wide_u;
 };
 
 namespace {
diff --git a/open-pi-zero_amd/pizero_native/_lib.py b/open-pi-zero_amd/pizero_native/_lib.py
--- a/open-pi-zero_amd/pizero_native/_lib.py
+++ b/open-pi-zero_amd/pizero_native/_lib.py
@@ -141,6 +141,7 @@
     "pz_rope_table": [vp, i64, i64, f32, vp],
     "pz_qkv_rope_split": [vp, vp, vp, vp, vp, vp, i64, i64, i64, i64, i64, i64, i64, i64, i64, vp],
     "pz_qkv_rope_split_bwd": [vp, vp, vp, vp, vp, vp, i64, i64, i64, i64, i64, i64, i64, i64, i64, vp],
+    "pz_qkv_rope_split_bwd_kv": [vp, vp, vp, vp, vp, i64, i64, i64, i64, i64, i64, i64, vp],
     "pz_gemv_qkv_rope": [C.POINTER(QkvRopeArgs), vp],
     "pz_gemm_qkv_rope": [C.POINTER(QkvRopeArgs), vp],
     "pz_decode_attn": [C.POINTER(DecodeAttnArgs), vp],
@@ -150,6 +151,8 @@
     "pz_flash_fwd": [C.POINTER(FlashArgs), vp],
     "pz_flash_fwd_probs": [C.POINTER(FlashArgs), vp, vp, i64, vp],
     "pz_flash_bwd_ds": [C.POINTER(FlashArgs), vp, vp, vp, i64, vp],
+    "pz_flash_bwd_ds_rope": [C.POINTER(FlashArgs), vp, vp, vp, i64, C.POINTER(vp), C.POINTER(i64), C.POINTER(vp),
+                             C.POINTER(vp), vp],
     "pz_flash_bwd_prep": [C.POINTER(FlashArgs), vp],
     "pz_flash_bwd": [C.POINTER(FlashArgs), vp],
     "pz_patchify": [vp, vp, i64, i64, i64, i64, i64, vp],
@@ -190,6 +193,7 @@
     "pz_action_denormalize": [vp, vp, i64, i64, i64, vp, vp, i32, vp],
     "pz_debug_poison_lds": [C.c_uint32, vp],
     "pz_debug_spin": [i64, i64, vp],
+    "pz_debug_narrow_stores": [i32],
     "pz_last_error": [],
     "pz_abi_version": [],
 }
@@ -223,7 +227,7 @@
 
 _NO_LAUNCH = {"pz_last_error", "pz_abi_version", "pz_gemm_kernel_name", "pz_norm_rows_per_part",
               "pz_decode_attn_ws_bytes", "pz_lora_wgrad_ws_bytes", "pz_debug_poison_lds",
-              "pz_image_resize_scratch_bytes"}
+              "pz_image_resize_scratch_bytes", "pz_debug_narrow_stores"}
 _POISON_LDS = [0xFFFFFFFF if os.environ.get("PZ_POISON_LDS", "0") == "1" else None]
 
 
diff --git a/open-pi-zero_amd/pizero_native/engine.py b/open-pi-zero_amd/pizero_native/engine.py
--- a/open-pi-zero_amd/pizero_native/engine.py
+++ b/open-pi-zero_amd/pizero_native/engine.py
@@ -287,6 +287,7 @@
         self._jkv_holder = None
         self.joint_flash = False
         self.joint_probs = True
+        self.joint_dq_rope = True
         self.infer_flash = True
         self.fuse_qkv_rope = self.d.hd == 256
         self.expert_stream = True
@@ -1081,13 +1082,17 @@
         dO[g.name] = o
         dXm[g.name] = dxm
 
-    def _qkv_backward(self, g, gs, p, dQ, dK, dV, dX, dXm, pos, B, L, Lp, beta, rpp, nh, hd, dev, A=None, l=None):
+    def _qkv_backward(self, g, gs, p, dQ, dK, dV, dX, dXm, pos, B, L, Lp, beta, rpp, nh, hd, dev, A=None, l=None,
+                      dqkv=None):
         x = gs["x"]
         M = x.shape[0]
         W = (nh + 2) * hd
-        dqkv = torch.empty(M, W, device=dev, dtype=BF16)
-        ops.qkv_rope_split_bwd(None if gs.get("skip") else dQ, dK, dV, pos[g.pos_key], self.rope(g.theta), dqkv,
-                               B, g.T, nh, 1, hd, L, g.off, Lp, g.off)
+        if dqkv is not None:
+            ops.qkv_rope_split_bwd_kv(dK, dV, pos[g.pos_key], self.rope(g.theta), dqkv, B, g.T, nh, 1, hd, Lp, g.off)
+        else:
+            dqkv = torch.empty(M, W, device=dev, dtype=BF16)
+            ops.qkv_rope_split_bwd(None if gs.get("skip") else dQ, dK, dV, pos[g.pos_key], self.rope(g.theta), dqkv,
+                                   B, g.T, nh, 1, hd, L, g.off, Lp, g.off)
         names = [p + f"self_attn.{k}_proj.weight" for k in "qkv"]
         rgs = [self.rg(n) for n in names]
         site = self.lora(*names)
@@ -1151,11 +1156,12 @@
         ada = sv.get("ada") or {}
         for l in reversed(range(d.nL)):
             st = sv["joint"][l]
-            dQ = torch.empty(B, L, nh * hd, device=dev, dtype=BF16)
+            dQ = None
             dK = torch.empty(B, Lp, hd, device=dev, dtype=BF16)
             dV = torch.empty(B, Lp, hd, device=dev, dtype=BF16)
             dO = {}
             dXm = {}
+            dqkvs = None
             any_skip = False
             for g in groups:
                 gs = st["g"][g.name]
@@ -1175,14 +1181,26 @@
                         dO[g.name] = torch.zeros(B * g.T, nh * hd, device=dev, dtype=BF16)
                 if delta is None:
                     delta = torch.empty(B, L * nh, device=dev, dtype=F32)
+                dQ = torch.empty(B, L, nh * hd, device=dev, dtype=BF16)
                 ops.flash_bwd(self._joint_flash(groups, st["Q"], st["K"], st["V"], st["O"], st["lse"], cnt, B, L,
                                                 dO=dO, delta=delta, dq=dQ, dk=dK, dv=dV))
             else:
                 Pm, tc, Qj, Kj, Vj = st["P"], st["tc"], st["Q"], st["K"], st["V"]
                 dq_done = False
-                if not isinstance(cnt, GeneralMask) and L <= 320 and hd == 256:
+                fused = not isinstance(cnt, GeneralMask) and L <= 320 and hd == 256
+                if fused and self.joint_dq_rope and not any_skip:
                     if dS is None:
                         dS = torch.empty(B, L * nh, Lp, device=dev, dtype=BF16)
+                    gsort = sorted(groups, key=lambda g: g.off)
+                    dqkvs = {g.name: torch.empty(B * g.T, (nh + 2) * hd, device=dev, dtype=BF16) for g in groups}
+                    ops.flash_bwd_ds_rope(self._joint_flash(groups, Qj, Kj, Vj, st["O"], None, cnt, B, L, dO=dO), Pm, tc,
+                                          dS, Lp, [dqkvs[g.name] for g in gsort], [pos[g.pos_key] for g in gsort],
+                                          [self.rope(g.theta) for g in gsort])
+                    dq_done = True
+                elif fused:
+                    if dS is None:
+                        dS = torch.empty(B, L * nh, Lp, device=dev, dtype=BF16)
+                    dQ = torch.empty(B, L, nh * hd, device=dev, dtype=BF16)
                     ops.flash_bwd_ds(self._joint_flash(groups, Qj, Kj, Vj, st["O"], None, cnt, B, L, dO=dO,
                                                        dq=dQ), Pm, tc, dS, Lp)
                     dq_done = True
@@ -1200,6 +1218,7 @@
                                  batch=B, sA=(g.T * nh * hd, 0), sB=(Lp * hd, 0), sC=(L * nh * Lp, 0))
                     ops.attn_softmax_bwd(Pm, dP, Lp, tc, dS, Lp, B * L * nh, L, 1.0 / math.sqrt(hd), 50.0)
                 if not dq_done:
+                    dQ = torch.empty(B, L, nh * hd, device=dev, dtype=BF16)
                     ops.gemm(L * nh, hd, Lp, dS, Lp, True, Kj, hd, False, dQ, hd, batch=B, sA=(L * nh * Lp, 0),
                              sB=(Lp * hd, 0), sC=(L * nh * hd, 0))
                 ops.gemm(Lp, hd, L * nh, dS, Lp, False, Qj, hd, False, dK, hd, batch=B, sA=(L * nh * Lp, 0),
@@ -1215,12 +1234,14 @@
                     dV.zero_()
             if side is not None:
                 side.wait_stream(main)
-                for t in (dQ, dK, dV):
-                    t.record_stream(side)
+                for t in (dQ, dK, dV, *(dqkvs or {}).values()):
+                    if t is not None:
+                        t.record_stream(side)
             for g in groups:
                 with self._on(side, g):
                     self._qkv_backward(g, st["g"][g.name], f"{g.prefix}{l}.", dQ, dK, dV, dX, dXm, pos, B, L, Lp, beta,
-                                       rpp, nh, hd, dev, ada.get(g.name), l)
+                                       rpp, nh, hd, dev, ada.get(g.name), l,
+                                       dqkv=None if dqkvs is None else dqkvs[g.name])
             self._chk(f"joint bwd layer {l}", dO=dO, dS=dS, dQ=dQ, dK=dK, dV=dV, dX=dX)
             self._notify("joint", l, (side,) if side is not None else ())
         if side is not None:
diff --git a/open-pi-zero_amd/pizero_native/ops.py b/open-pi-zero_amd/pizero_native/ops.py
--- a/open-pi-zero_amd/pizero_native/ops.py
+++ b/open-pi-zero_amd/pizero_native/ops.py
@@ -533,8 +533,31 @@
     call("pz_flash_bwd_ds", C.byref(a), _p(P), _p(tcap), _p(dS), int(ldp), _st())
 
 
+def flash_bwd_ds_rope(a, P, tcap, dS, ldp, dqkv, pos, cs):
+    n = len(dqkv)
+    assert n == a.n_groups == len(pos) == len(cs)
+    pd = (C.c_void_p * n)(*[_p(t) for t in dqkv])
+    ld = (C.c_int64 * n)(*[int(t.stride(0)) for t in dqkv])
+    pp = (C.c_void_p * n)(*[_p(t) for t in pos])
+    pc = (C.c_void_p * n)(*[_p(t) for t in cs])
+    call("pz_flash_bwd_ds_rope", C.byref(a), _p(P), _p(tcap), _p(dS), int(ldp), pd, ld, pp, pc, _st())
+
+
+def qkv_rope_split_bwd_kv(dk, dv, pos, cs, dqkv, B, T, nh, nkv, hd, Lk, koff):
+    call("pz_qkv_rope_split_bwd_kv", _p(dk), _p(dv), _p(pos), _p(cs), _p(dqkv), B, T, nh, nkv, hd, Lk, koff, _st())
+
+
 def flash_fwd_probs(a, P, tcap, ldp):
     call("pz_flash_fwd_probs", C.byref(a), _p(P), _p(tcap), int(ldp), _st())
+
+
+class narrow_stores:
+
+    def __enter__(self):
+        call("pz_debug_narrow_stores", 1)
+
+    def __exit__(self, *exc):
+        call("pz_debug_narrow_stores", 0)
 
 
 def flash_bwd(a):
```

Measured after the change: 278.6 samples/s, median of 6. No clear change (+0.5%).
